# millecker/hadoop-1.0.3-gpu

Measured on AMD Instinct MI355X. Metric: K-Means job makespan + map-tasks/sec (whole node) at 1/2/4/8 MI355X, higher is better.
Workload: dtype fp32

## Files before the change

hbmr/models/kmeans.py:

```python
from __future__ import annotations

import base64
import logging
import math
import os
import threading
import time

import numpy as np
import torch

from ..gpu.splitjob import SplitJob, SplitSpec
from ..mapred import counters as C

log = logging.getLogger("hbmr.kmeans")

K_KEY = "hbmr.kmeans.k"
D_KEY = "hbmr.kmeans.dims"
INPUT_KEY = "hbmr.kmeans.input"
SPLIT_PTS_KEY = "hbmr.split.points"
CIN_KEY = "hbmr.kmeans.centroids.in"
COUT_KEY = "hbmr.kmeans.centroids.out"
INIT_KEY = "hbmr.kmeans.centroids.init"
NCENTERS_KEY = "hbmr.kmeans.synthetic.centers"
RETURN_KEY = "hbmr.kmeans.return.centroids"
CDIR_KEY = "hbmr.kmeans.centroids.dir"
EXACT_KEY = "hbmr.kmeans.exact"
EXACT_MFMA_KEY = "hbmr.kmeans.exact.mfma"
COMBINER_KEY = "hbmr.kmeans.combiner"
BOUNDS_KEY = "hbmr.kmeans.exact.bounds"

_M32 = 0xFFFFFFFF


def _mix32(x: torch.Tensor) -> torch.Tensor:
    x = x & _M32
    x = ((x ^ (x >> 16)) * 0x45D9F3B) & _M32
    x = ((x ^ (x >> 16)) * 0x45D9F3B) & _M32
    return x ^ (x >> 16)


def _uniform(c: torch.Tensor) -> torch.Tensor:
    return (_mix32(c).to(torch.float64) + 0.5) * (1.0 / 4294967296.0)


def _gauss(c1: torch.Tensor, c2: torch.Tensor) -> torch.Tensor:
    u1 = _uniform(c1)
    u2 = _uniform(c2)
    return torch.sqrt(-2.0 * torch.log(u1)) * torch.cos(2.0 * math.pi * u2)


def synthetic_points(seed: int, start: int, n: int, d: int, centers: int, device,
                     chunk: int = 1 << 18) -> torch.Tensor:
    dev = torch.device(device)
    out = torch.empty(n, d, dtype=torch.float32, device=dev)
    j = torch.arange(d, dtype=torch.int64, device=dev)
    cidx = torch.arange(centers, dtype=torch.int64, device=dev)
    s = (seed * 0x9E3779B1) & _M32
    cc = (cidx[:, None] * 131071 + j[None, :] + s * 7) & _M32
    cen = 10.0 * _gauss(cc * 2 + 1, cc * 2 + 2)
    for a in range(0, n, chunk):
        b = min(n, a + chunk)
        p = torch.arange(start + a, start + b, dtype=torch.int64, device=dev)
        lab = _mix32(p * 3 + s) % centers
        base = ((p[:, None] & 0xFFFFFF) * 1024 + j[None, :] + (s << 7)) & _M32
        noise = _gauss(base * 2 + 11, base * 2 + 12 + (p[:, None] >> 24))
        out[a:b] = (cen[lab] + noise).to(torch.float32)
    return out


def encode_centroids(c: torch.Tensor) -> str:
    a = c.detach().to("cpu", torch.float32).contiguous().numpy()
    return f"{a.shape[0]}x{a.shape[1]}:" + base64.b64encode(a.tobytes()).decode()


def decode_centroids(s: str) -> torch.Tensor:
    shp, b = s.split(":", 1)
    k, d = map(int, shp.split("x"))
    return torch.from_numpy(np.frombuffer(base64.b64decode(b), dtype=np.float32).copy()
                            ).reshape(k, d)


class CentroidStore:

    def __init__(self):
        self.lock = threading.Lock()
        self.host: dict[str, torch.Tensor] = {}
        self.images: dict[tuple, object] = {}
        self.order: list[str] = []
        self.keep = 4

    def put_host(self, key, cen):
        with self.lock:
            self.host[key] = cen
            for k in [k for k in self.images if k[0] == key]:
                self.images.pop(k)
            self._touch(key)

    def put_image(self, key, device, img):
        with self.lock:
            self.host.pop(key, None)
            self.images[(key, str(device))] = img
            self._touch(key)

    def _touch(self, key):
        if key in self.order:
            self.order.remove(key)
        self.order.append(key)
        while len(self.order) > self.keep:
            old = self.order.pop(0)
            self.host.pop(old, None)
            for k in [k for k in self.images if k[0] == old]:
                self.images.pop(k)

    def host_centroids(self, key):
        with self.lock:
            c = self.host.get(key)
            if c is not None:
                return c
            for (k, _dev), img in self.images.items():
                if k == key:
                    ready = getattr(img, "ready", None)
                    if ready is not None:
                        ready.synchronize()
                    c = img.cen.detach().to("cpu")
                    self.host[key] = c
                    return c
        return None

    def image(self, key, device):
        from ..ops import kmeans as km
        with self.lock:
            img = self.images.get((key, str(device)))
        if img is not None:
            return img
        cen = self.host_centroids(key)
        if cen is None:
            raise KeyError(f"centroids {key!r} not resident on this tracker")
        img = km.CentroidImage(cen, device)
        if img.cen.is_cuda:
            img.ready = torch.cuda.Event()
            img.ready.record()
        self.put_image(key, device, img)
        return img


STORE = CentroidStore()


def _centroid_file(cdir, key):
    return os.path.join(cdir, key.replace("/", "_").replace(":", "_") + ".npy")


def _save_centroids(cdir, key, cen):
    host = cen.detach().to("cpu", torch.float32).numpy()
    os.makedirs(cdir, exist_ok=True)
    path = _centroid_file(cdir, key)
    tmp = path + ".tmp.npy"
    np.save(tmp, host)
    os.replace(tmp, path)
    old = _SAVED.setdefault(cdir, [])
    old.append(path)
    while len(old) > 3:
        try:
            os.remove(old.pop(0))
        except OSError:
            pass


_SAVED: dict = {}
_PINNED_INFLIGHT: list = []


def _sum_slabs(outs):
    groups: dict = {}
    loose = []
    for s, c in outs:
        bs, bc = s._base, c._base
        if bs is not None and bc is not None and bs.dim() == 3 and bc.dim() == 2 and \
                tuple(s.shape) == tuple(bs.shape[1:]) and tuple(c.shape) == tuple(bc.shape[1:]):
            g = groups.setdefault(id(bs), [bs, bc, 0, []])
            g[2] += 1
            g[3].append((s, c))
        else:
            loose.append((s, c))
    parts_s, parts_c = [], []
    for bs, bc, n, members in groups.values():
        if n == bs.shape[0] and len({m[0].data_ptr() for m in members}) == n:
            parts_s.append(bs.sum(0))
            parts_c.append(bc.sum(0))
        else:
            loose.extend(members)
    if loose:
        parts_s.append(torch.stack([s for s, _ in loose]).sum(0))
        parts_c.append(torch.stack([c for _, c in loose]).sum(0))
    sums, counts = parts_s[0], parts_c[0]
    for s, c in zip(parts_s[1:], parts_c[1:]):
        sums = sums + s
        counts = counts + c
    return sums, counts


_EXACT_STATS: dict = {}
_EXACT_SKIPPED: dict = {}
_EXACT_LOCK = threading.Lock()

_BASELINES: "dict" = {}
_BASE_LOCK = threading.Lock()
_BASE_MAX = 4096


def _baseline_plan(ctxs, datas, k, dp, fx, exact, enabled):
    have, new, plain = [], [], []
    bases, keys = [], []
    seen = set()
    dev = str(ctxs[0].device)
    with _BASE_LOCK:
        for i, (c, d) in enumerate(zip(ctxs, datas)):
            sp = c.spec.split
            sk = sp.get("key") if enabled and isinstance(sp, dict) else None
            key = None if sk is None else (sk, dev, k, dp, fx, exact)
            keys.append(key)
            if key is None or key in seen:
                plain.append(i)
                bases.append(None)
                continue
            seen.add(key)
            b = _BASELINES.get(key)
            x = d.xb if exact else d
            if b is not None and b.data_ptr == x.data_ptr() and b.n == x.shape[0]:
                have.append(i)
                bases.append(b)
            else:
                new.append(i)
                bases.append(None)
    return have, new, plain, bases, keys


def _baseline_bytes(b) -> int:
    return sum(t.numel() * t.element_size() for t in (b.g, b.S0, b.N0, getattr(b, "gap", None))
               if t is not None)


def _drop_baselines(split_key, device):
    dev = f"cuda:{device}" if isinstance(device, int) else str(device)
    with _BASE_LOCK:
        for key in [kk for kk in _BASELINES if kk[0] == split_key and kk[1] == dev]:
            _BASELINES.pop(key)


def _install_baselines(entries, stream, cache=None, grown=None):
    ev = torch.cuda.Event()
    ev.record(stream)
    charge = []
    with _BASE_LOCK:
        for key, b in entries:
            b.event, b.stream = ev, stream
            old = _BASELINES.pop(key, None)
            _BASELINES[key] = b
            if old is not b:
                charge.append((key, b, _baseline_bytes(b)))
            elif grown and grown.get(id(b)):
                charge.append((key, b, grown[id(b)]))
        while len(_BASELINES) > _BASE_MAX:
            _BASELINES.pop(next(iter(_BASELINES)))
    if cache is not None and charge:
        cache.add_listener(_drop_baselines)
        idx = stream.device.index if stream is not None else 0
        for key, b, nbytes in charge:
            if not cache.charge(key[0], idx, nbytes):
                with _BASE_LOCK:
                    if _BASELINES.get(key) is b:
                        _BASELINES.pop(key)


def _exact_stats(cin, device):
    key = (cin, str(device))
    with _EXACT_LOCK:
        t = _EXACT_STATS.get(key)
        if t is None:
            t = _EXACT_STATS[key] = torch.zeros(3, dtype=torch.int64, device=device)
        return t


def _exact_skipped(cin, device):
    key = (cin, str(device))
    with _EXACT_LOCK:
        t = _EXACT_SKIPPED.get(key)
        if t is None:
            t = _EXACT_SKIPPED[key] = torch.zeros(1, dtype=torch.int64, device=device)
        return t


class KMeansSplitJob(SplitJob):
    collective_reduce = True
    needs_reduce = True

    def configure(self, conf):
        self.conf = conf
        self.k = conf.get_int(K_KEY, 64)
        self.d = conf.get_int(D_KEY, 128)
        self.input = conf.get(INPUT_KEY, "synthetic:100000:1")
        self.split_points = conf.get_int(SPLIT_PTS_KEY, 500_000)
        self.cin = conf.get(CIN_KEY)
        self.cout = conf.get(COUT_KEY)
        self.centers = conf.get_int(NCENTERS_KEY, self.k)
        self.fx_shift = conf.get_int("hbmr.kmeans.fx.shift", 24)
        self.cdir = conf.get(CDIR_KEY)
        self.exact = conf.get_boolean(EXACT_KEY, False)
        self.exact_dtype = torch.bfloat16 if (conf.get(EXACT_MFMA_KEY) or "f16").lower() in (
            "bf16", "bfloat16") else torch.float16
        self.bounds = conf.get_boolean(BOUNDS_KEY, True)
        self.combiner = (conf.get(COMBINER_KEY) or "delta").lower()
        if self.combiner not in ("delta", "sorted"):
            raise ValueError(f"{COMBINER_KEY} must be delta or sorted, not {self.combiner!r}")
        init = conf.get(INIT_KEY)
        if init and self.cin and STORE.host_centroids(self.cin) is None:
            STORE.put_host(self.cin, decode_centroids(init))
        if self.cin and self.cdir and STORE.host_centroids(self.cin) is None:
            path = _centroid_file(self.cdir, self.cin)
            if os.path.exists(path):
                STORE.put_host(self.cin, torch.from_numpy(np.load(path)))

    _split_memo: dict = {}

    def get_splits(self, conf, trackers):
        if self.input.startswith("synthetic:"):
            mk = (self.input, self.split_points, self.d, self.centers, tuple(trackers),
                  self.exact)
            got = KMeansSplitJob._split_memo.get(mk)
            if got is not None:
                return got
            if len(KMeansSplitJob._split_memo) > 16:
                KMeansSplitJob._split_memo.clear()
            out = KMeansSplitJob._split_memo[mk] = self._synthetic_splits(trackers)
            return out
        return self._file_splits(conf, trackers)

    def _synthetic_splits(self, trackers):
        _, n, seed = self.input.split(":")
        n, seed = int(n), int(seed)
        per = self.split_points
        nsplits = max(1, math.ceil(n / per))
        out = []
        for i in range(nsplits):
            a = i * per
            m = min(per, n - a)
            key = f"kmeans-syn:{seed}:{self.d}:{self.centers}:{a}:{m}" + \
                (":exact" if self.exact else "")
            loc = [trackers[i * len(trackers) // nsplits]] if trackers else []
            out.append(SplitSpec(i, key, "synthetic",
                                 {"seed": seed, "start": a, "n": m}, loc, m * self.d * 2))
        return out

    def _file_splits(self, conf, trackers):
        from ..mapred.formats import FileInputFormat, SequenceFileInputFormat
        from ..mapred.jobconf import JobConf
        jc = JobConf(conf)
        FileInputFormat.setInputPaths(jc, self.input)
        fmt = SequenceFileInputFormat()
        nmaps = max(1, conf.get_int("mapred.map.tasks", 1))
        if conf.get_long("mapred.min.split.size", 0) <= 1 and "://" not in self.input:
            total = sum(f.length for f in fmt.list_status(jc))
            jc.set_long("mapred.min.split.size", max(1, -(-total // nmaps)))
        splits = fmt.getSplits(jc, nmaps)
        out = []
        for i, s in enumerate(splits):
            key = f"kmeans-file:{s.path}:{s.start}:{s.length}" + (":exact" if self.exact else "")
            loc = [trackers[i % len(trackers)]] if trackers else []
            out.append(SplitSpec(i, key, "file", {"path": s.path, "start": s.start,
                                                  "length": s.length}, loc, s.length))
        return out

    def _load_raw(self, spec: SplitSpec, device):
        if spec.kind == "synthetic":
            p = spec.params
            return synthetic_points(p["seed"], p["start"], p["n"], self.d, self.centers, device)
        return self._load_file_split(spec.params, device)

    def _load_fp32(self, spec: SplitSpec, device):
        return self._load_raw(spec, device).to(torch.bfloat16)

    def split_nbytes(self, data) -> int:
        nb = getattr(data, "nbytes", None)
        if callable(nb):
            return int(nb())
        return super().split_nbytes(data)

    def load_split_host(self, spec: SplitSpec):
        if spec.kind != "file":
            return None
        from ..io import nativeio
        p = spec.params
        n = p["length"] // (20 + 4 * self.d) + 2
        host = torch.empty(n, self.d, dtype=torch.float32,
                           pin_memory=torch.cuda.is_available())
        got = nativeio.read_points_into(p["path"], p["start"], p["length"], host.data_ptr(),
                                        self.d, n)
        return host[:got]

    def load_split_from_host(self, spec: SplitSpec, host, device):
        from ..ops import kmeans as km
        x = host.to(device, non_blocking=True)
        ev = torch.cuda.Event()
        ev.record()
        _PINNED_INFLIGHT.append((ev, host))
        while _PINNED_INFLIGHT and _PINNED_INFLIGHT[0][0].query():
            _PINNED_INFLIGHT.pop(0)
        if self.exact:
            return km.ExactSplit(x, km.padded_dim(self.d), self.exact_dtype)
        xb = x.to(torch.bfloat16)
        dp = km.padded_dim(self.d)
        if dp == self.d:
            return xb.contiguous()
        out = torch.zeros(xb.shape[0], dp, dtype=torch.bfloat16, device=device)
        out[:, :self.d] = xb
        return out

    def _load_file_split(self, p, device):
        from ..io import nativeio
        n = p["length"] // (20 + 4 * self.d) + 2
        dev = torch.device(device)
        host = torch.empty(n, self.d, dtype=torch.float32, pin_memory=dev.type == "cuda")
        got = nativeio.read_points_into(p["path"], p["start"], p["length"], host.data_ptr(),
                                        self.d, n)
        host = host[:got]
        if dev.type != "cuda":
            return host
        x = host.to(dev, non_blocking=True)
        ev = torch.cuda.Event()
        ev.record()
        _PINNED_INFLIGHT.append((ev, host))
        while _PINNED_INFLIGHT and _PINNED_INFLIGHT[0][0].query():
            _PINNED_INFLIGHT.pop(0)
        return x

    def load_split_sample(self, spec: SplitSpec, device, fraction: float):
        if spec.kind == "synthetic":
            p = dict(spec.params)
            p["n"] = max(1, int(p["n"] * fraction))
            spec = SplitSpec(spec.index, spec.key + f":sample{fraction}", spec.kind, p,
                             spec.locations, spec.length)
            return self.load_split(spec, device)
        return super().load_split_sample(spec, device, fraction)

    def load_split(self, spec: SplitSpec, device):
        from ..ops import kmeans as km
        if self.exact:
            x = self._load_raw(spec, device)
            if str(device) == "cpu":
                return x.contiguous()
            return km.ExactSplit(x, km.padded_dim(self.d), self.exact_dtype)
        xb = self._load_fp32(spec, device)
        if str(device) == "cpu":
            return xb.to(torch.float32)
        dp = km.padded_dim(self.d)
        if dp == self.d:
            return xb.contiguous()
        out = torch.zeros(xb.shape[0], dp, dtype=torch.bfloat16, device=device)
        out[:, :self.d] = xb
        return out

    @staticmethod
    def _scratch(ctx, ns, k):
        from ..ops import kmeans as km
        key = ("kmeans-scratch", str(ctx.device), id(ctx.stream))
        store = ctx.tracker.__dict__.setdefault("_scratch", {})
        ws, labels = store.get(key, (None, None))
        need_lab, need_ws = km.batch_scratch_sizes(ns, k)
        need_ws = max(need_ws, km.delta_workspace_bytes(int(sum(ns)), len(ns), k))
        if ws is None or ws.numel() < need_ws:
            ws = torch.empty(max(need_ws, 1 << 20), dtype=torch.uint8, device=ctx.device)
        if labels is None or labels.numel() < need_lab:
            labels = torch.empty(max(need_lab, 1), dtype=torch.int32, device=ctx.device)
        store[key] = (ws, labels)
        return ws, labels

    def map_gpu(self, ctx, points):
        return self.map_gpu_batch([ctx], [points])[0]

    def map_gpu_batch(self, ctxs, datas):
        st = ctxs[0].stream
        if st is None:
            return self._map_gpu_batch(ctxs, datas)
        with torch.cuda.stream(st):
            return self._map_gpu_batch(ctxs, datas)

    def _map_gpu_batch(self, ctxs, datas):
        from ..ops import kmeans as km
        ctx = ctxs[0]
        img = STORE.image(self.cin, ctx.device)
        ready = getattr(img, "ready", None)
        if ready is not None:
            torch.cuda.current_stream().wait_event(ready)
        for t in (img.cbf, img.chalf):
            t.record_stream(torch.cuda.current_stream())
        B = len(datas)
        if self.exact:
            return self._map_exact(ctxs, datas, img)
        have, new, plain, bases, keys = _baseline_plan(
            ctxs, datas, self.k, img.dp, img.fx_shift, False, self.combiner == "delta")
        ws, labels = self._scratch(ctx, [d.shape[0] for d in datas], self.k)
        sums = torch.empty(B, self.k, img.dp, dtype=torch.int64, device=ctx.device)
        counts = torch.empty(B, self.k, dtype=torch.int64, device=ctx.device)
        order = have + new + plain
        H = len(have)
        S, N = sums.unbind(0), counts.unbind(0)
        out = [None] * B
        for j, i in enumerate(order):
            out[i] = (S[j], N[j])
        installed = []
        if have:
            hb = [bases[i] for i in have]
            km.map_batch_delta([datas[i] for i in have], img, sums[:H], counts[:H], labels, ws,
                               hb, stream=ctx.stream)
            for i, b in zip(have, hb):
                b.S0, b.N0 = out[i]
                installed.append((keys[i], b))
        rest = new + plain
        if rest:
            km.map_batch_gpu([datas[i] for i in rest], img, sums[H:], counts[H:], labels, ws,
                             stream=ctx.stream, zero_outputs=True)
            if new:
                total = sum(datas[i].shape[0] for i in rest)
                gall = labels[:total].clone()
                off = 0
                newset = set(new)
                for i in rest:
                    n = datas[i].shape[0]
                    if keys[i] is not None and i in newset:
                        installed.append((keys[i], km.Baseline(gall[off:off + n], *out[i],
                                                                datas[i].data_ptr(), n)))
                    off += n
        if installed:
            _install_baselines(installed, ctx.stream, getattr(ctx, "split_cache", None))
        for c, d in zip(ctxs, datas):
            c.reporter.incrCounter(C.TASK_GROUP, C.MAP_INPUT_RECORDS, d.shape[0])
        return out

    def _map_exact(self, ctxs, datas, img):
        from ..ops import kmeans as km
        from ..utils.trace import TRACE
        if TRACE.on:
            TRACE.instant("kmeans.map_exact", n=len(datas))
        ctx = ctxs[0]
        store = ctx.tracker.__dict__.setdefault("_scratch", {})
        scratch = store.setdefault(("kmeans-exact", str(ctx.device), id(ctx.stream)), {})
        stats = _exact_stats(self.cin, ctx.device)
        have, new, plain, bases, keys = _baseline_plan(
            ctxs, datas, self.k, img.dp, img.fx_shift, True, self.combiner == "delta")
        B = len(datas)
        sums = torch.empty(B, self.k, img.dp, dtype=torch.int64, device=ctx.device)
        counts = torch.empty(B, self.k, dtype=torch.int64, device=ctx.device)
        order = have + new + plain
        pos = {i: j for j, i in enumerate(order)}
        H = len(have)
        installed = []
        grown = None
        if have:
            ns = [datas[i].shape[0] for i in have]
            total = sum(ns)
            lab = scratch.get("labcat")
            if lab is None or lab.numel() < total:
                lab = scratch["labcat"] = torch.empty(total, dtype=torch.int32, device=ctx.device)
            need = km.delta_workspace_bytes(total, H, self.k)
            if scratch.get("dws") is None or scratch["dws"].numel() < need:
                scratch["dws"] = torch.empty(need, dtype=torch.uint8, device=ctx.device)
            hb = [bases[i] for i in have]
            bounded = self.bounds and self.combiner == "delta" and km.bounds_supported(img)
            if bounded:
                nogap = [b for b in hb if b.gap is None]
                km.assign_exact_batch([datas[i] for i in have], img, stats, lab, scratch,
                                      stream=ctx.stream, bounds=hb,
                                      skipped=_exact_skipped(self.cin, ctx.device))
                grown = {id(b): b.gap.numel() * b.gap.element_size() for b in nogap}
            else:
                km.assign_exact_batch([datas[i] for i in have], img, stats, lab, scratch,
                                      stream=ctx.stream)
            km.delta_combine([datas[i].x32 for i in have], lab, self.k, sums[:H], counts[:H],
                             scratch["dws"], hb, fx_shift=img.fx_shift, stream=ctx.stream,
                             keep_bounds=bounded)
            for i, b in zip(have, hb):
                b.S0, b.N0 = sums[pos[i]], counts[pos[i]]
                installed.append((keys[i], b))
        for i in new + plain:
            d = datas[i]
            s, c = sums[pos[i]], counts[pos[i]]
            s.zero_()
            c.zero_()
            lab = km.assign_exact(d, img, stats, scratch, stream=ctx.stream)
            need = km.workspace_bytes(d.shape[0], img.k)
            if scratch.get("ws") is None or scratch["ws"].numel() < need:
                scratch["ws"] = torch.empty(max(need, 1 << 20), dtype=torch.uint8,
                                            device=ctx.device)
            km.accumulate(d.x32, lab, img.k, s, c, fx_shift=img.fx_shift, stream=ctx.stream,
                          workspace=scratch["ws"])
            if keys[i] is not None and i in new:
                b = km.Baseline(lab.clone(), s, c, d.xb.data_ptr(), d.shape[0])
                installed.append((keys[i], b))
        if installed:
            _install_baselines(installed, ctx.stream, getattr(ctx, "split_cache", None), grown)
        for c, d in zip(ctxs, datas):
            c.reporter.incrCounter(C.TASK_GROUP, C.MAP_INPUT_RECORDS, d.shape[0])
        return [(sums[pos[i]], counts[pos[i]]) for i in range(B)]

    def map_cpu(self, ctx, points):
        from ..ops import kmeans as km
        cen = STORE.host_centroids(self.cin)
        if cen is None:
            raise KeyError(f"centroids {self.cin!r} not resident")
        sums, counts = km.new_partials(self.k, self.d, "cpu")
        st = [0]
        km.map_split_cpu(points, cen, sums, counts, nthreads=ctx.cpu_threads,
                         fx_shift=self.fx_shift, exact=self.exact, stats=st)
        if self.exact:
            ctx.reporter.incrCounter("KMEANS", "EXACT_FLAGGED_POINTS", st[0])
        ctx.reporter.incrCounter(C.TASK_GROUP, C.MAP_INPUT_RECORDS, points.shape[0])
        return sums, counts

    def map_sim(self, ctx, points):
        if points is None:
            ctx.reporter.incrCounter(C.TASK_GROUP, C.MAP_INPUT_RECORDS, 0)
            return None
        return self.map_cpu(ctx, points)

    def combine(self, ctx, outputs):
        from ..ops import kmeans as km
        dev = ctx.device if ctx.device is not None else torch.device("cpu")
        dp = km.padded_dim(self.d) if dev.type == "cuda" else self.d
        outputs = [o for o in outputs if o is not None]
        if dev.type == "cuda":
            cur = torch.cuda.current_stream()
            for s, c in outputs:
                if s.is_cuda:
                    s.record_stream(cur)
                    c.record_stream(cur)
        from ..utils.trace import TRACE
        if TRACE.on:
            TRACE.instant("kmeans.combine.recorded", n=len(outputs))
        same = [(s, c) for s, c in outputs if s.device == dev and s.shape[1] == dp]
        other = [(s, c) for s, c in outputs if not (s.device == dev and s.shape[1] == dp)]
        if same:
            sums, counts = _sum_slabs(same)
        else:
            sums = torch.zeros(self.k, dp, dtype=torch.int64, device=dev)
            counts = torch.zeros(self.k, dtype=torch.int64, device=dev)
        for s, c in other:
            sums[:, :s.shape[1]] += s.to(dev, non_blocking=True)
            counts += c.to(dev, non_blocking=True)
        return sums, counts

    def reduce(self, ctx, combined):
        from ..ops import kmeans as km
        from ..utils.trace import TRACE
        sums, counts = combined
        k, dp = sums.shape
        packed = torch.cat([sums.reshape(-1), counts])
        sim = getattr(ctx, "simulated_collective_s", None)
        with TRACE.span("kmeans.allreduce", nbytes=packed.numel() * 8):
            if sim is None:
                ctx.comm.all_reduce(packed)
            else:
                ctx.sim_ready = max(time.time(), getattr(ctx, "sim_base", 0.0)) + sim
        sums = packed[:k * dp].view(k, dp)
        counts = packed[k * dp:]
        est = _EXACT_STATS.pop((self.cin, str(sums.device)), None) \
            if self.exact and sums.device.type == "cuda" else None
        esk = _EXACT_SKIPPED.pop((self.cin, str(sums.device)), None) \
            if self.exact and sums.device.type == "cuda" else None
        killed = getattr(ctx, "killed", None)
        if killed is not None and killed():
            raise RuntimeError("reduce killed (collective restart): result not published")
        if sums.device.type == "cuda":
            old = STORE.image(self.cin, sums.device)
            ready = getattr(old, "ready", None)
            if ready is not None:
                torch.cuda.current_stream().wait_event(ready)
            img = km.CentroidImage.__new__(km.CentroidImage)
            img.__dict__.update(old.__dict__)
            img.cen = old.cen.clone()
            img.cbf = old.cbf.clone()
            img.chalf = old.chalf.clone()
            img.shift2 = torch.zeros_like(old.shift2)
            img.refresh(sums, counts)
            if self.exact:
                img.image16(self.exact_dtype)
                img.neighbors()
            img.ready = torch.cuda.Event()
            img.ready.record()
            host_cen = cen_ev = None
            if ctx.rank == 0 and (self.cdir or self.conf.get_boolean(RETURN_KEY, False)):
                host_cen = torch.empty(tuple(img.cen.shape), dtype=torch.float32,
                                       pin_memory=True)
                host_cen.copy_(img.cen, non_blocking=True)
                cen_ev = torch.cuda.Event()
                cen_ev.record()
            if TRACE.on:
                TRACE.instant("kmeans.refresh_launched")
            STORE.put_image(self.cout, sums.device, img)
            rel = getattr(ctx, "release_dependents", None)
            if rel is not None:
                rel()
            vals = [img.shift2.max().double().sqrt(), counts.sum().double()]
            if est is not None:
                vals += list(est.double().unbind(0))
            if esk is not None:
                vals.append(esk[0].double())
            got = torch.stack(vals).tolist()
            shift, npts = got[0], got[1]
            if esk is not None:
                ctx.reporter.incrCounter("KMEANS", "EXACT_BOUND_SKIPPED_POINTS", int(got[-1]))
            if est is not None:
                for name, v in zip(("EXACT_FLAGGED_POINTS", "EXACT_RELABELLED_POINTS",
                                    "EXACT_NEIGHBOUR_SCANS"), got[2:5]):
                    ctx.reporter.incrCounter("KMEANS", name, int(v))
            if TRACE.on:
                TRACE.instant("kmeans.shift_synced")
            new_cen = None
        else:
            host_cen = cen_ev = None
            old = STORE.host_centroids(self.cin)
            if sim is not None:
                new_cen, shift, npts = old, 0.0, 0
            else:
                cnt = counts.to(torch.float64)[:, None]
                s = sums[:, :self.d].to(torch.float64) / float(1 << self.fx_shift)
                new_cen = torch.where(cnt > 0, s / cnt.clamp(min=1),
                                      old.to(torch.float64)).to(torch.float32)
                shift = float((new_cen - old).norm(dim=1).max()) if self.k else 0.0
                npts = int(counts.sum().item())
            STORE.put_host(self.cout, new_cen)
            rel = getattr(ctx, "release_dependents", None)
            if rel is not None:
                rel()
            if sim is not None:
                delay = ctx.sim_ready - time.time()
                if delay > 0:
                    time.sleep(delay)
        self._write_output(ctx, counts, new_cen)
        if TRACE.on:
            TRACE.instant("kmeans.output_written")
        res = {"shift": shift, "points": int(npts), "centroids_key": self.cout}
        if host_cen is not None:
            cen_ev.synchronize()
        if ctx.rank == 0 and self.cdir:
            cen = new_cen if new_cen is not None else host_cen
            _save_centroids(self.cdir, self.cout, cen[:, :self.d])
        if ctx.rank == 0 and self.conf.get_boolean(RETURN_KEY, False):
            cen = new_cen if new_cen is not None else host_cen
            res["centroids"] = encode_centroids(cen[:, :self.d])
        if TRACE.on:
            TRACE.instant("kmeans.reduce_return")
        return res

    def poison_result(self, ctx):
        with STORE.lock:
            host = STORE.host.get(self.cout)
            if host is not None:
                STORE.host[self.cout] = host + 1.0
            for key, img in list(STORE.images.items()):
                if key[0] == self.cout:
                    STORE.images.pop(key)
                    STORE.host[self.cout] = img.cen.detach().to("cpu")[:, :self.d] + 1.0

    def _write_output(self, ctx, counts, new_cen):
        out = self.conf.get("mapred.output.dir")
        if not out:
            return
        import os

        from ..io import sequencefile as seqf
        from ..io.writable import FloatVectorWritable, IntWritable
        cen = new_cen if new_cen is not None else STORE.host_centroids(self.cout)
        W = ctx.world_size
        per = math.ceil(self.k / W)
        lo, hi = ctx.rank * per, min(self.k, (ctx.rank + 1) * per)
        os.makedirs(out, exist_ok=True)
        with seqf.Writer(os.path.join(out, f"part-{ctx.rank:05d}"), IntWritable,
                         FloatVectorWritable) as w:
            for j in range(lo, hi):
                w.append(IntWritable(j), FloatVectorWritable(cen[j].numpy()))


def make_iteration_conf(base, k, d, inp, split_points, cin, cout, init=None,
                        return_centroids=False):
    from ..mapred.jobconf import JobConf
    job = JobConf(base)
    job.set_job_name(f"kmeans {cin}->{cout}")
    job.set("hbmr.splitjob.class", "hbmr.models.kmeans:KMeansSplitJob")
    job.set("hbmr.gpu.mapper.class", "hbmr.models.kmeans:KMeansSplitJob")
    job.set_int(K_KEY, k)
    job.set_int(D_KEY, d)
    job.set(INPUT_KEY, inp)
    job.set_int(SPLIT_PTS_KEY, split_points)
    job.set(CIN_KEY, cin)
    job.set(COUT_KEY, cout)
    job.set("hbmr.job.signature", f"kmeans|{inp}|{k}|{d}|{split_points}")
    if init is not None:
        job.set(INIT_KEY, encode_centroids(init))
    if return_centroids:
        job.set_boolean(RETURN_KEY, True)
    return job


def initial_centroids(inp, k, d, centers=None, exact=False):
    def rnd(x):
        return x if exact else x.to(torch.bfloat16).to(torch.float32)
    if inp.startswith("synthetic:"):
        _, _n, seed = inp.split(":")
        x = synthetic_points(int(seed), 0, k, d, centers or k, "cpu")
        return rnd(x)
    from ..io import sequencefile as seqf
    import os
    path = inp
    if os.path.isdir(path):
        path = os.path.join(path, sorted(f for f in os.listdir(path) if not f.startswith(("_", ".")))[0])
    rows = []
    with seqf.Reader(path) as r:
        while len(rows) < k:
            raw = r.next_raw()
            if raw is None:
                break
            rows.append(np.frombuffer(raw[1][4:], dtype=">f4").astype(np.float32))
    return rnd(torch.from_numpy(np.stack(rows)))


class KMeansDriver:

    MANIFEST = "driver.json"

    def __init__(self, submit, result_of, conf=None, k=64, d=128, inp="synthetic:100000:1",
                 split_points=500_000, run_id=None, return_centroids=None, checkpoint_dir=None):
        self.submit = submit
        self.result_of = result_of
        self.base = conf
        self.k, self.d, self.inp, self.split_points = k, d, inp, split_points
        self.run_id = run_id or f"km{int(time.time() * 1e3) & 0xFFFFFF:x}"
        self.iteration = 0
        self.history = []
        self.return_centroids = (k * d <= 65536) if return_centroids is None else return_centroids
        base_dir = (conf.get("mapred.local.dir") if conf is not None else None) or "/tmp/hbmr-local"
        self.centroid_dir = checkpoint_dir or os.path.join(base_dir, "kmeans-centroids",
                                                           self.run_id)
        self._manifest_written = False
        self.prefetch_delay = 0.005
        self._ahead: list = []

    def _write_manifest(self):
        import json
        os.makedirs(self.centroid_dir, exist_ok=True)
        path = os.path.join(self.centroid_dir, self.MANIFEST)
        with open(path + ".tmp", "w") as f:
            json.dump({"run_id": self.run_id, "k": self.k, "d": self.d, "input": self.inp,
                       "split_points": self.split_points}, f)
        os.replace(path + ".tmp", path)
        self._manifest_written = True

    @classmethod
    def resume(cls, submit, result_of, checkpoint_dir, conf=None, **kw):
        import json
        import re
        with open(os.path.join(checkpoint_dir, cls.MANIFEST)) as f:
            m = json.load(f)
        drv = cls(submit, result_of, conf=conf, k=m["k"], d=m["d"], inp=m["input"],
                  split_points=m["split_points"], run_id=m["run_id"],
                  checkpoint_dir=checkpoint_dir, **kw)
        pat = re.compile(re.escape(_centroid_file("", drv.key(0))[:-len("_0.npy")]) +
                         r"_(\d+)\.npy$")
        found = sorted((int(mm.group(1)), fn) for fn in os.listdir(checkpoint_dir)
                       for mm in [pat.match(fn)] if mm)
        for i, fn in reversed(found):
            try:
                c = torch.from_numpy(np.load(os.path.join(checkpoint_dir, fn)))
            except (OSError, ValueError):
                continue
            if tuple(c.shape) != (drv.k, drv.d):
                continue
            drv.iteration = i
            STORE.put_host(drv.key(i), c.to(torch.float32))
            break
        drv._manifest_written = True
        return drv

    def key(self, i):
        return f"{self.run_id}:{i}"

    def _job_conf(self, i, depends_on=None):
        centers = self.base.get_int(NCENTERS_KEY, self.k) if self.base is not None else None
        exact = self.base.get_boolean(EXACT_KEY, False) if self.base is not None else False
        init = initial_centroids(self.inp, self.k, self.d, centers, exact=exact) if i == 0 \
            else None
        if init is not None:
            STORE.put_host(self.key(0), init)
        job = make_iteration_conf(self.base, self.k, self.d, self.inp, self.split_points,
                                  self.key(i), self.key(i + 1), init=init,
                                  return_centroids=self.return_centroids)
        job.set(CDIR_KEY, self.centroid_dir)
        if depends_on is not None:
            from ..mapred.jobtracker import DEPENDS_KEY
            job.set(DEPENDS_KEY, str(depends_on))
        return job

    def step(self, prefetch=False):
        i = self.iteration
        if not self._manifest_written:
            self._write_manifest()
        t0 = time.time()
        ahead = bool(self._ahead)
        rj = self._ahead.pop(0) if ahead else self.submit(self._job_conf(i))
        depth = int(prefetch)
        if depth > 0 and len(self._ahead) < depth and \
                (ahead or not rj.waitForCompletion(self.prefetch_delay)):
            last = self._ahead[-1] if self._ahead else rj
            while len(self._ahead) < depth:
                nxt = self.submit(self._job_conf(i + 1 + len(self._ahead),
                                                 depends_on=last.getID()))
                self._ahead.append(nxt)
                last = nxt
        rj.waitForCompletion()
        if not rj.isSuccessful():
            raise RuntimeError(f"K-Means iteration {i} failed: {rj.getFailureInfo()}")
        res = dict(self.result_of(rj) or {})
        jip = getattr(rj._impl, "jip", None)
        if jip is not None:
            res["timeline"] = jip.timeline()
            res["maps_per_tracker"] = jip.maps_per_tracker()
        res.update(iteration=i, seconds=time.time() - t0, job=str(rj.getID()),
                   counters=rj.getCounters())
        self.history.append(res)
        self.iteration += 1
        return res

    def run(self, max_iter=10, tol=0.0):
        for _ in range(max_iter):
            r = self.step()
            if r.get("shift", 1.0) <= tol:
                break
        return self.centroids()

    def cancel_prefetch(self):
        ahead, self._ahead = self._ahead, []
        for nxt in reversed(ahead):
            nxt.killJob()

    def centroids(self):
        c = STORE.host_centroids(self.key(self.iteration))
        if c is None and self.history and self.history[-1].get("centroids"):
            c = decode_centroids(self.history[-1]["centroids"])
            STORE.put_host(self.key(self.iteration), c)
        return c


def main(argv=None, cluster=None):
    import argparse
    ap = argparse.ArgumentParser(prog="hbmr kmeans")
    ap.add_argument("--input", default=None, help="SequenceFile dir (default: synthetic)")
    ap.add_argument("--points", type=int, default=1_000_000)
    ap.add_argument("--k", type=int, default=64)
    ap.add_argument("--dims", type=int, default=128)
    ap.add_argument("--iters", type=int, default=5)
    ap.add_argument("--split-points", type=int, default=500_000)
    ap.add_argument("--seed", type=int, default=7)
    a = ap.parse_args(argv)
    from ..mapred.cluster import LocalCluster
    from ..mapred.jobconf import JobConf
    own = cluster is None
    conf = JobConf()
    if own:
        gpus = [[0]] if torch.cuda.is_available() else None
        cluster = LocalCluster(conf, num_trackers=1, gpus=gpus)
    try:
        drv = KMeansDriver(cluster.submit_job, lambda rj: rj._impl.jip.result[0], conf=conf,
                           k=a.k, d=a.dims, inp=a.input or f"synthetic:{a.points}:{a.seed}",
                           split_points=a.split_points)
        for _ in range(a.iters):
            r = drv.step()
            print(f"iteration {r['iteration']}: shift {r['shift']:.6f} "
                  f"({r['seconds'] * 1e3:.1f} ms)")
        return 0
    finally:
        if own:
            cluster.shutdown()
```

hbmr/ops/_lib.py:

```python
from __future__ import annotations

import ctypes
import os
import threading
from pathlib import Path

import torch

_LIB_PATH = Path(__file__).resolve().parent.parent / "lib" / "libhbmr.so"
_lock = threading.Lock()
_lib = None

c_void_p = ctypes.c_void_p
c_long = ctypes.c_long
c_int = ctypes.c_int
c_uint = ctypes.c_uint
c_uint64 = ctypes.c_uint64
c_double_p = ctypes.POINTER(ctypes.c_double)

_SIGS = {
    "hbmr_kmeans_assign_bf16": (c_int, [c_void_p, c_long, c_int, c_void_p, c_void_p, c_int,
                                        c_void_p, c_void_p, c_void_p]),
    "hbmr_kmeans_accum_bf16": (c_int, [c_void_p, c_long, c_int, c_void_p, c_int, c_void_p,
                                       c_void_p, c_int, c_void_p, c_long, c_int, c_void_p]),
    "hbmr_kmeans_accum_f32": (c_int, [c_void_p, c_long, c_int, c_void_p, c_int, c_void_p,
                                      c_void_p, c_int, c_void_p, c_long, c_int, c_void_p]),
    "hbmr_kmeans_assign_top3_bf16": (c_int, [c_void_p, c_long, c_int, c_void_p, c_void_p, c_int,
                                             c_void_p, c_void_p, c_void_p, c_void_p, c_void_p]),
    "hbmr_kmeans_assign_top3_f16": (c_int, [c_void_p, c_long, c_int, c_void_p, c_void_p, c_int,
                                            c_void_p, c_void_p, c_void_p, c_void_p, c_void_p]),
    "hbmr_kmeans_exact_prep": (c_int, [c_void_p, c_long, c_int, c_int, c_int, c_int, c_void_p,
                                       c_void_p, c_void_p, c_void_p, c_void_p]),
    "hbmr_kmeans_assign_top3_q1_grouped": (c_int, [c_int, c_void_p, c_void_p, c_int, c_int,
                                                   c_void_p, c_void_p, c_void_p, c_int, c_void_p,
                                                   c_void_p, c_void_p, c_void_p, c_int, c_int,
                                                   c_void_p, c_void_p, c_void_p, c_void_p,
                                                   c_void_p, c_long, c_void_p, c_void_p]),
    "hbmr_kmeans_bound_workspace_bytes": (c_long, [c_long, c_int, c_int]),
    "hbmr_kmeans_assign_top3_q1_bounded": (c_int, [c_int, c_void_p, c_void_p, c_int, c_int,
                                                   c_void_p, c_void_p, c_int, c_void_p,
                                                   c_void_p, c_void_p, c_void_p, c_int, c_int,
                                                   c_void_p, c_void_p, c_void_p, c_void_p,
                                                   c_void_p, c_long, c_void_p,
                                                   c_void_p, c_void_p, c_void_p, c_void_p,
                                                   c_void_p, c_long, c_void_p, c_void_p]),
    "hbmr_kmeans_centroid_nbr": (c_int, [c_void_p, c_int, c_int, c_int, c_void_p, c_void_p,
                                         c_void_p, c_void_p]),
    "hbmr_kmeans_image16": (c_int, [c_void_p, c_int, c_int, c_int, c_int, c_int, c_void_p,
                                    c_void_p, c_void_p, c_void_p, c_void_p, c_void_p]),
    "hbmr_kmeans_image16_tiled": (c_int, [c_void_p, c_int, c_int, c_void_p, c_void_p]),
    "hbmr_kmeans_set_exact_kernel": (c_int, [c_int]),
    "hbmr_kmeans_get_exact_kernel": (c_int, []),
    "hbmr_kmeans_refine_f32": (c_int, [c_void_p, c_long, c_int, c_int, c_void_p, c_void_p,
                                       c_void_p, c_void_p, c_int, c_int, c_void_p, c_void_p,
                                       c_void_p, c_void_p, c_void_p, c_void_p, c_int, c_void_p,
                                       c_void_p, c_void_p, c_void_p, c_void_p, c_int,
                                       c_void_p]),
    "hbmr_kmeans_refine_batch_bytes": (c_long, [c_int, c_void_p]),
    "hbmr_kmeans_assign_top3_grouped": (c_int, [c_int, c_void_p, c_void_p, c_int, c_int,
                                                c_void_p, c_void_p, c_int, c_void_p, c_void_p,
                                                c_void_p, c_void_p, c_void_p]),
    "hbmr_kmeans_refine_batch_q1g": (c_int, [c_int, c_void_p, c_int, c_int, c_int, c_void_p,
                                             c_void_p, c_void_p, c_void_p, c_void_p, c_void_p,
                                             c_void_p, c_void_p, c_void_p, c_void_p, c_void_p,
                                             c_void_p, c_long, c_void_p, c_void_p]),
    "hbmr_kmeans_refine_batch_q1": (c_int, [c_int, c_void_p, c_int, c_int, c_int, c_int,
                                            c_void_p, c_void_p, c_void_p, c_void_p, c_void_p,
                                            c_void_p, c_void_p, c_void_p, c_void_p, c_void_p,
                                            c_void_p, c_void_p, c_void_p, c_long, c_int,
                                            c_void_p, c_void_p]),
    "hbmr_kmeans_refine_batch_finish": (c_int, [c_int, c_void_p, c_void_p, c_void_p, c_int,
                                                c_int, c_void_p, c_int, c_int, c_void_p,
                                                c_void_p, c_void_p, c_void_p, c_int, c_void_p,
                                                c_int, c_void_p, c_long, c_void_p]),
    "hbmr_kmeans_accum_workspace_bytes": (c_long, [c_long, c_int]),
    "hbmr_kmeans_batch_workspace_bytes": (c_long, [c_long, c_int, c_int]),
    "hbmr_kmeans_map_batch": (c_int, [c_int, c_void_p, c_void_p, c_int, c_void_p, c_void_p, c_int,
                                      c_int, c_void_p, c_void_p, c_long, c_void_p, c_void_p,
                                      c_int, c_int, c_void_p]),
    "hbmr_kmeans_delta_workspace_bytes": (c_long, [c_long, c_int, c_int]),
    "hbmr_kmeans_delta_combine": (c_int, [c_int, c_void_p, c_void_p, c_int, c_int, c_int,
                                          c_void_p, c_void_p, c_long, c_void_p, c_void_p, c_int,
                                          c_void_p, c_void_p, c_void_p, c_void_p]),
    "hbmr_kmeans_map_batch_delta": (c_int, [c_int, c_void_p, c_void_p, c_int, c_void_p, c_void_p,
                                            c_int, c_int, c_void_p, c_void_p, c_long, c_void_p,
                                            c_void_p, c_int, c_void_p, c_void_p, c_void_p,
                                            c_void_p]),
    "hbmr_kmeans_update": (c_int, [c_void_p, c_void_p, c_int, c_int, c_int, c_int, c_int,
                                   c_void_p, c_void_p, c_void_p, c_void_p, c_void_p]),
    "hbmr_kmeans_padded_k": (c_int, [c_int]),
    "hbmr_kmeans_map_cpu_f32": (c_int, [c_void_p, c_long, c_int, c_void_p, c_int, c_void_p,
                                        c_void_p, c_void_p, c_double_p, c_int, c_int]),
    "hbmr_kmeans_map_cpu_f32_ex": (c_int, [c_void_p, c_long, c_int, c_void_p, c_int, c_void_p,
                                           c_void_p, c_void_p, c_double_p, c_int, c_int, c_int,
                                           c_void_p]),
    "hbmr_kmeans_padded_dim": (c_int, [c_int]),
    "hbmr_f32_to_bf16_pad": (c_int, [c_void_p, c_long, c_int, c_int, c_void_p, c_void_p]),
    "hbmr_radix_sort_workspace_bytes": (c_long, [c_long]),
    "hbmr_radix_onesweep_workspace_bytes": (c_long, [c_long]),
    "hbmr_radix_onesweep_status_bytes": (c_long, [c_long]),
    "hbmr_radix_sort_keys_u64": (c_int, [c_void_p, c_void_p, c_long, c_int, c_int, c_void_p,
                                         c_long, c_void_p, c_long, c_void_p, c_void_p, c_int,
                                         c_void_p]),
    "hbmr_radix_sort_pairs_u64": (c_int, [c_void_p, c_void_p, c_void_p, c_void_p, c_long, c_int,
                                          c_int, c_void_p, c_long, c_void_p]),
    "hbmr_teragen": (c_int, [c_long, c_long, c_void_p, c_void_p]),
    "hbmr_tera_keys": (c_int, [c_void_p, c_long, c_int, c_void_p, c_void_p, c_void_p]),
    "hbmr_gather_u64": (c_int, [c_void_p, c_void_p, c_long, c_void_p, c_void_p]),
    "hbmr_gather_records": (c_int, [c_void_p, c_void_p, c_long, c_int, c_void_p, c_void_p]),
    "hbmr_split_offsets": (c_int, [c_void_p, c_void_p, c_long, c_void_p, c_void_p, c_int,
                                   c_void_p, c_void_p]),
    "hbmr_check_sorted": (c_int, [c_void_p, c_void_p, c_long, c_void_p, c_void_p]),
    "hbmr_tera_collect": (c_int, [c_void_p, c_void_p, c_void_p, c_void_p, c_void_p, c_int, c_long,
                                  c_void_p, c_void_p, c_void_p, c_void_p, c_void_p]),
    "hbmr_tera_collect_slots": (c_int, [c_void_p, c_void_p, c_void_p, c_int, c_int, c_long,
                                        c_void_p, c_void_p, c_void_p]),
    "hbmr_gather_records_multi": (c_int, [c_void_p, c_void_p, c_void_p, c_void_p, c_long, c_int,
                                          c_void_p, c_void_p]),
    "hbmr_tera_partition_workspace_bytes": (c_long, [c_long, c_int]),
    "hbmr_tera_collect_gid": (c_int, [c_void_p, c_void_p, c_void_p, c_void_p, c_int, c_long,
                                      c_int, c_uint64, c_uint, c_uint, c_int, c_void_p, c_void_p,
                                      c_void_p]),
    "hbmr_gather_records_gid": (c_int, [c_void_p, c_void_p, c_void_p, c_long, c_int, c_void_p,
                                        c_void_p, c_void_p, c_void_p, c_void_p]),
    "hbmr_tera_group_stats": (c_int, [c_void_p, c_void_p, c_long, c_void_p, c_void_p, c_void_p,
                                      c_void_p]),
    "hbmr_radix_set_onesweep_waves": (c_int, [c_int]),
    "hbmr_gather_set_unroll": (c_int, [c_int]),
    "hbmr_tera_tie_fix_scratch_bytes": (c_long, [c_long, c_int]),
    "hbmr_tera_tie_fix_records": (c_int, [c_void_p, c_void_p, c_void_p, c_long, c_int, c_uint64,
                                          c_uint, c_uint, c_int, c_void_p, c_void_p, c_void_p,
                                          c_long, c_void_p]),
    "hbmr_merge_path": (c_int, [c_void_p, c_void_p, c_void_p, c_long, c_void_p, c_void_p, c_void_p,
                                c_long, c_void_p, c_void_p, c_void_p, c_void_p]),
    "hbmr_tera_tie_fix": (c_int, [c_void_p, c_void_p, c_void_p, c_long, c_void_p, c_void_p]),
    "hbmr_tera_partition": (c_int, [c_void_p, c_long, c_int, c_void_p, c_void_p, c_int, c_void_p,
                                    c_void_p, c_void_p, c_void_p, c_void_p, c_void_p, c_long,
                                    c_void_p]),
    "hbmr_wc_tiles": (c_long, [c_long]),
    "hbmr_wc_tokenize_count": (c_int, [c_void_p, c_long, c_void_p, c_void_p]),
    "hbmr_wc_tokenize_write": (c_int, [c_void_p, c_long, c_void_p, c_void_p, c_void_p, c_void_p]),
    "hbmr_wc_insert": (c_int, [c_void_p, c_long, c_void_p, c_void_p, c_void_p, c_long, c_void_p,
                               c_void_p, c_long, c_void_p, c_void_p]),
    "hbmr_wc_compact": (c_int, [c_void_p, c_long, c_void_p, c_void_p, c_long, c_int, c_void_p,
                                c_void_p, c_void_p, c_void_p, c_void_p, c_void_p]),
    "hbmr_wc_pack": (c_int, [c_void_p, c_void_p, c_void_p, c_void_p, c_long, c_void_p, c_void_p,
                             c_void_p]),
    "hbmr_grep_cand_count": (c_int, [c_void_p, c_long, c_void_p, c_void_p, c_int, c_int, c_int,
                                     c_int, c_void_p, c_void_p, c_void_p]),
    "hbmr_grep_cand_write": (c_int, [c_void_p, c_long, c_void_p, c_void_p, c_int, c_int, c_int,
                                     c_int, c_void_p, c_void_p, c_void_p, c_void_p, c_void_p]),
    "hbmr_grep_select_blocks": (c_long, [c_long]),
    "hbmr_grep_block_max": (c_int, [c_void_p, c_long, c_void_p, c_void_p]),
    "hbmr_grep_prefix_max": (c_int, [c_void_p, c_long, c_void_p, c_void_p, c_void_p]),
    "hbmr_grep_select_count": (c_int, [c_void_p, c_void_p, c_void_p, c_long, c_void_p, c_void_p]),
    "hbmr_grep_select_write": (c_int, [c_void_p, c_void_p, c_void_p, c_long, c_void_p, c_void_p,
                                       c_void_p, c_void_p]),
    "hbmr_span_insert": (c_int, [c_void_p, c_long, c_void_p, c_void_p, c_void_p, c_long, c_void_p,
                                 c_void_p, c_long, c_void_p, c_void_p]),
    "hbmr_span_compact": (c_int, [c_void_p, c_void_p, c_void_p, c_void_p, c_void_p, c_long, c_int,
                                  c_void_p, c_void_p, c_void_p, c_void_p, c_void_p, c_void_p]),
    "hbmr_lines_count": (c_int, [c_void_p, c_long, c_void_p, c_void_p]),
    "hbmr_lines_write": (c_int, [c_void_p, c_long, c_void_p, c_void_p, c_void_p, c_void_p]),
    "hbmr_recsort_hash_partition": (c_int, [c_void_p, c_void_p, c_void_p, c_long, c_int, c_void_p,
                                            c_void_p]),
    "hbmr_recsort_round_keys": (c_int, [c_void_p, c_void_p, c_void_p, c_void_p, c_long, c_int,
                                        c_void_p, c_void_p, c_void_p]),
    "hbmr_recsort_round_workspace_bytes": (c_long, [c_long]),
    "hbmr_recsort_round": (c_int, [c_void_p, c_void_p, c_void_p, c_int, c_long, c_int, c_void_p,
                                   c_void_p, c_void_p, c_void_p, c_void_p, c_void_p, c_void_p,
                                   c_void_p, c_void_p, c_long, c_void_p]),
    "hbmr_recsort_cuts": (c_int, [c_void_p, c_void_p, c_void_p, c_void_p, c_long, c_void_p,
                                  c_void_p, c_void_p, c_int, c_void_p, c_void_p]),
    "hbmr_recsort_chunk_bytes": (c_int, []),
    "hbmr_recsort_set_chunk_lanes": (c_int, [c_int]),
    "hbmr_recsort_gather": (c_int, [c_void_p, c_void_p, c_void_p, c_void_p, c_void_p, c_void_p,
                                    c_void_p, c_long, c_long, c_void_p, c_void_p]),
    "hbmr_recjoin_heads": (c_int, [c_void_p, c_void_p, c_void_p, c_long, c_void_p, c_void_p,
                                   c_void_p]),
    "hbmr_recjoin_set_two_level": (c_int, [c_int]),
    "hbmr_recjoin_rank": (c_int, [c_void_p, c_void_p, c_void_p, c_void_p, c_long, c_void_p,
                                  c_void_p, c_void_p, c_void_p, c_void_p, c_long, c_void_p,
                                  c_void_p, c_void_p]),
    "hbmr_recjoin_expand": (c_int, [c_void_p, c_int, c_void_p, c_void_p, c_void_p, c_void_p,
                                    c_void_p, c_void_p, c_long, c_int, c_void_p, c_long, c_long,
                                    c_void_p, c_void_p, c_void_p, c_void_p]),
    "hbmr_recjoin_frames": (c_int, [c_void_p, c_int, c_void_p, c_void_p, c_void_p, c_int,
                                    c_void_p, c_void_p, c_void_p, c_long, c_void_p, c_void_p,
                                    c_void_p, c_void_p, c_void_p, c_void_p, c_void_p, c_void_p,
                                    c_void_p]),
    "hbmr_recjoin_copy": (c_int, [c_void_p, c_void_p, c_void_p, c_void_p, c_void_p, c_long,
                                  c_void_p, c_void_p]),
    "hbmr_pi_halton": (c_int, [ctypes.c_longlong, ctypes.c_longlong, c_void_p, c_void_p]),
    "hbmr_gemm_bf16_tn": (c_int, [c_void_p, c_void_p, c_void_p, c_long, c_long, c_long,
                                  ctypes.c_float, c_int, c_void_p]),
    "hbmr_gemm_set_kernel": (c_int, [c_int]),
    "hbmr_gemm_bf16_tn_ex": (c_int, [c_void_p, c_void_p, c_void_p, c_long, c_long, c_long,
                                     ctypes.c_float, c_int, c_void_p, c_void_p]),
}


class NativeLibraryError(RuntimeError):
    pass


def lib_path() -> Path:
    return _LIB_PATH


def available() -> bool:
    try:
        load()
        return True
    except NativeLibraryError:
        return False


def load():
    global _lib
    if _lib is not None:
        return _lib
    with _lock:
        if _lib is not None:
            return _lib
        if not _LIB_PATH.exists() and os.environ.get("HBMR_AUTOBUILD", "1") == "1":
            try:
                import importlib.util
                spec = importlib.util.spec_from_file_location(
                    "hbmr_native_build", _LIB_PATH.parent.parent.parent / "native" / "build.py")
                mod = importlib.util.module_from_spec(spec)
                spec.loader.exec_module(mod)
                mod.build()
            except Exception as e:
                raise NativeLibraryError(f"libhbmr.so missing and build failed: {e}") from e
        if not _LIB_PATH.exists():
            raise NativeLibraryError(f"native library not found at {_LIB_PATH}; run native/build.py")
        try:
            lib = ctypes.CDLL(str(_LIB_PATH), mode=ctypes.RTLD_GLOBAL)
        except OSError as e:
            raise NativeLibraryError(f"cannot load {_LIB_PATH}: {e}") from e
        for name, (res, args) in _SIGS.items():
            fn = getattr(lib, name)
            fn.restype = res
            fn.argtypes = args
        _lib = lib
        return lib


def check(rc: int, what: str) -> None:
    if rc != 0:
        raise RuntimeError(f"{what} failed with native error code {rc}")


def stream_handle(stream=None) -> int:
    if stream is None:
        stream = torch.cuda.current_stream()
    return int(stream.cuda_stream)
```

hbmr/ops/kmeans.py:

```python
from __future__ import annotations

import ctypes
import os
import threading

import torch

from . import _lib
from ..utils.trace import TRACE

SUPPORTED_DP = (64, 128, 256)


def _nullctx():
    import contextlib
    return contextlib.nullcontext()
FX_SHIFT = 24
NBR_L = 256


def padded_dim(d: int) -> int:
    for dp in SUPPORTED_DP:
        if d <= dp:
            return dp
    raise ValueError(f"feature dim {d} > {SUPPORTED_DP[-1]} not supported by the MFMA kernel")


def padded_k(k: int) -> int:
    return ((k + 63) // 64) * 64


def _ptr(t):
    return None if t is None else ctypes.c_void_p(t.data_ptr())


def new_partials(k: int, dp: int, device) -> tuple[torch.Tensor, torch.Tensor]:
    return (torch.zeros(k, dp, dtype=torch.int64, device=device),
            torch.zeros(k, dtype=torch.int64, device=device))


def partials_to_float(sums: torch.Tensor, counts: torch.Tensor, d: int | None = None,
                      fx_shift: int = FX_SHIFT):
    s = sums.to(torch.float64) / float(1 << fx_shift)
    if d is not None:
        s = s[:, :d]
    return s, counts.to(torch.float64)


class CentroidImage:

    def __init__(self, centroids: torch.Tensor, device, fx_shift: int = FX_SHIFT):
        c = centroids.detach().to(device=device, dtype=torch.float32).contiguous()
        self.k, self.d = c.shape
        self.dp = padded_dim(self.d)
        self.k_pad = padded_k(self.k)
        self.fx_shift = fx_shift
        self.device = c.device
        self.cen = c
        self.cbf = torch.zeros(self.k_pad, self.dp, dtype=torch.bfloat16, device=device)
        self.chalf = torch.empty(self.k_pad, dtype=torch.float32, device=device)
        self.shift2 = torch.zeros(self.k, dtype=torch.float32, device=device)
        self.refresh()

    def refresh(self, sums=None, counts=None, stream=None):
        lib = _lib.load()
        rc = lib.hbmr_kmeans_update(_ptr(sums), _ptr(counts), self.fx_shift, self.k, self.d,
                                    self.dp, self.k_pad, _ptr(self.cen), _ptr(self.cbf),
                                    _ptr(self.chalf), _ptr(self.shift2),
                                    _lib.stream_handle(stream))
        _lib.check(rc, "hbmr_kmeans_update")
        self._img16 = {}
        self._nbr = None
        if getattr(self, "_nbr_lock", None) is None:
            self._nbr_lock = threading.Lock()

    def set_centroids(self, centroids: torch.Tensor, stream=None):
        self.cen.copy_(centroids.to(self.cen.device, torch.float32))
        self.refresh(stream=stream)

    def image16(self, dtype=torch.float16):
        with self._nbr_lock:
            cache = self.__dict__.setdefault("_img16", {})
            ent = cache.get(dtype)
            if ent is None:
                dev = self.cen.device
                c16 = torch.empty(self.k_pad, self.dp, dtype=dtype, device=dev)
                ch = torch.empty(self.k_pad, dtype=torch.float32, device=dev)
                cn = torch.empty(self.k, dtype=torch.float32, device=dev)
                ce = torch.empty(self.k, dtype=torch.float32, device=dev)
                mx = torch.empty(2, dtype=torch.float32, device=dev)
                rc = _lib.load().hbmr_kmeans_image16(
                    _ptr(self.cen), self.k, self.d, self.dp, self.k_pad,
                    int(dtype == torch.float16), _ptr(c16), _ptr(ch), _ptr(cn), _ptr(ce),
                    _ptr(mx), _lib.stream_handle(None))
                _lib.check(rc, "hbmr_kmeans_image16")
                c16t = None
                if self.dp in (64, 128):
                    c16t = torch.empty_like(c16)
                    rc = _lib.load().hbmr_kmeans_image16_tiled(
                        _ptr(c16), self.k_pad, self.dp, _ptr(c16t), _lib.stream_handle(None))
                    _lib.check(rc, "hbmr_kmeans_image16_tiled")
                ev = torch.cuda.Event()
                ev.record()
                ent = cache[dtype] = (c16, ch, cn, mx[0:1], ce, mx[1:2], ev, c16t)
        torch.cuda.current_stream().wait_event(ent[6])
        return ent[:6]

    def image16_tiled(self, dtype=torch.float16):
        self.image16(dtype)
        return self._img16[dtype][7]

    def norms(self, dtype=torch.float16):
        _, _, cn, cm, ce, cem = self.image16(dtype)
        return cn, cm, ce, cem

    def neighbors(self, L: int | None = None):
        with self._nbr_lock:
            if self._nbr is None:
                if L is None:
                    L = int(os.environ.get("HBMR_KMEANS_NBR_L", NBR_L))
                L = max(1, min(L, self.k))
                if self.cen.is_cuda and self.k <= NBR_NATIVE_MAX_K and self.d <= 256:
                    dev = self.cen.device
                    di = torch.empty(self.k, L, dtype=torch.int32, device=dev)
                    f = torch.empty(self.k, L, dtype=torch.float32, device=dev)
                    pd = torch.empty(self.k, self.k, dtype=torch.float32, device=dev) \
                        if self.k <= PAIR_DIST_MAX_K else None
                    rc = _lib.load().hbmr_kmeans_centroid_nbr(
                        _ptr(self.cen), self.k, self.d, L, _ptr(di), _ptr(f), _ptr(pd),
                        _lib.stream_handle(None))
                    _lib.check(rc, "hbmr_kmeans_centroid_nbr")
                    ev = torch.cuda.Event()
                    ev.record()
                    self._nbr = (di, f, L, ev, pd)
                    di, f, L, ev, _ = self._nbr
                    torch.cuda.current_stream().wait_event(ev)
                    return di, f, L
                c = self.cen.double()
                n2 = (c * c).sum(1)
                nsum = n2[:, None] + n2[None, :]
                d2 = torch.addmm(nsum, c, c.T, beta=1.0, alpha=-2.0)
                err = nsum * ((self.d + 4) * 2.0 ** -53 * 1.01)
                lo = (d2 - err).clamp_(min=0.0).sqrt_()
                lo.fill_diagonal_(0.0)
                dv, di = lo.sort(dim=1, stable=True)
                dv, di = dv[:, :L].contiguous(), di[:, :L].to(torch.int32).contiguous()
                f = dv.float()
                f = torch.where(f.double() > dv, torch.nextafter(f, torch.full_like(f, -1.0)), f)
                pd = None
                if self.k <= PAIR_DIST_MAX_K:
                    hi = (d2 + err).clamp_(min=0.0).sqrt_()
                    hi.fill_diagonal_(0.0)
                    pd = hi.float()
                    pd = torch.where(pd.double() < hi, torch.nextafter(
                        pd, torch.full_like(pd, float("inf"))), pd).contiguous()
                ev = torch.cuda.Event()
                ev.record()
                self._nbr = (di, f.contiguous(), L, ev, pd)
        di, f, L, ev, _ = self._nbr
        torch.cuda.current_stream().wait_event(ev)
        return di, f, L

    def pair_dist(self):
        self.neighbors()
        return self._nbr[4]

    def max_shift(self) -> float:
        return float(self.shift2.max().sqrt().item()) if self.k else 0.0


def assign(points: torch.Tensor, img: CentroidImage, labels: torch.Tensor | None = None,
           scores: torch.Tensor | None = None, stream=None) -> torch.Tensor:
    n, dp = points.shape
    if points.dtype != torch.bfloat16 or dp != img.dp or not points.is_contiguous():
        raise ValueError("points must be contiguous bf16 [n, dp] matching the centroid image")
    if labels is None:
        labels = torch.empty(n, dtype=torch.int32, device=points.device)
    lib = _lib.load()
    rc = lib.hbmr_kmeans_assign_bf16(_ptr(points), n, dp, _ptr(img.cbf), _ptr(img.chalf),
                                     img.k_pad, _ptr(labels), _ptr(scores),
                                     _lib.stream_handle(stream))
    _lib.check(rc, "hbmr_kmeans_assign_bf16")
    return labels


ACCUM_AUTO, ACCUM_LDS, ACCUM_SORTED = 0, 1, 2
_workspaces: dict = {}


def workspace_bytes(n: int, k: int) -> int:
    return int(_lib.load().hbmr_kmeans_accum_workspace_bytes(n, k))


def batch_scratch_sizes(ns: list, k: int) -> tuple[int, int]:
    lib = _lib.load()
    total = int(sum(ns))
    ws = max(int(lib.hbmr_kmeans_batch_workspace_bytes(total, len(ns), k)),
             int(lib.hbmr_kmeans_accum_workspace_bytes(max(ns), k)))
    return total, ws


def accum_workspace(n: int, k: int, device) -> torch.Tensor:
    lib = _lib.load()
    need = int(lib.hbmr_kmeans_accum_workspace_bytes(n, k))
    key = torch.device(device)
    ws = _workspaces.get(key)
    if ws is None or ws.numel() < need:
        ws = torch.empty(max(need, 1 << 20), dtype=torch.uint8, device=key)
        _workspaces[key] = ws
    return ws


def accumulate(points: torch.Tensor, labels: torch.Tensor, k: int, sums: torch.Tensor,
               counts: torch.Tensor, fx_shift: int = FX_SHIFT, stream=None,
               workspace: torch.Tensor | None = None, mode: int = ACCUM_AUTO) -> None:
    n, dp = points.shape
    if sums.shape != (k, dp) or sums.dtype != torch.int64:
        raise ValueError(f"sums must be int64 [{k}, {dp}]")
    if counts.shape != (k,) or counts.dtype != torch.int64:
        raise ValueError(f"counts must be int64 [{k}]")
    if points.dtype not in (torch.bfloat16, torch.float32) or not points.is_contiguous() or \
            dp not in SUPPORTED_DP or labels.numel() < n:
        raise ValueError("points must be contiguous bf16/fp32 [n, dp] with n labels")
    lib = _lib.load()
    if workspace is None and mode != ACCUM_LDS:
        workspace = accum_workspace(n, k, points.device)
    fn, name = ((lib.hbmr_kmeans_accum_f32, "hbmr_kmeans_accum_f32")
                if points.dtype == torch.float32 else
                (lib.hbmr_kmeans_accum_bf16, "hbmr_kmeans_accum_bf16"))
    rc = fn(_ptr(points), n, dp, _ptr(labels), k, _ptr(sums), _ptr(counts), fx_shift,
            _ptr(workspace), 0 if workspace is None else workspace.numel(), mode,
            _lib.stream_handle(stream))
    _lib.check(rc, name)


def _f32_up(v: torch.Tensor) -> torch.Tensor:
    f = v.float()
    return torch.where(f.double() < v, torch.nextafter(f, torch.full_like(f, float("inf"))), f)


class ExactSplit:
    __slots__ = ("xb", "x32", "xnorm", "xbn2", "xerr", "d")

    def __init__(self, x32: torch.Tensor, dp: int, dtype=torch.float16):
        n, d = x32.shape
        self.d = d
        dev = x32.device
        if dp == d:
            self.x32 = x32.contiguous()
        else:
            self.x32 = torch.zeros(n, dp, dtype=torch.float32, device=dev)
            self.x32[:, :d] = x32
        if dev.type == "cuda":
            self.xb = torch.empty(n, dp, dtype=dtype, device=dev)
            self.xnorm = torch.empty(n, dtype=torch.float32, device=dev)
            self.xbn2 = torch.empty(n, dtype=torch.float32, device=dev)
            self.xerr = torch.empty(n, dtype=torch.float32, device=dev)
            rc = _lib.load().hbmr_kmeans_exact_prep(
                _ptr(self.x32), n, dp, dp, dp, int(dtype == torch.float16), _ptr(self.xb),
                _ptr(self.xnorm), _ptr(self.xbn2), _ptr(self.xerr), _lib.stream_handle(None))
            _lib.check(rc, "hbmr_kmeans_exact_prep")
            return
        x64 = self.x32.double()
        self.xnorm = x64.norm(dim=1).float()
        lim = 65504.0 if dtype == torch.float16 else float("inf")
        xb = self.x32.clamp(-lim, lim).to(dtype)
        xb64 = xb.double()
        self.xbn2 = xb64.pow(2).sum(1).float()
        self.xerr = _f32_up((x64 - xb64).norm(dim=1))
        self.xb = xb.contiguous()

    @property
    def shape(self):
        return self.xb.shape

    def nbytes(self) -> int:
        return sum(t.numel() * t.element_size() for t in (self.xb, self.x32, self.xnorm,
                                                          self.xbn2, self.xerr))


def assign_top3(points: torch.Tensor, img: CentroidImage, labels, cand, scores, margin,
                stream=None) -> None:
    n, dp = points.shape
    if points.dtype not in (torch.bfloat16, torch.float16) or dp != img.dp or \
            not points.is_contiguous():
        raise ValueError("points must be contiguous bf16/fp16 [n, dp] matching the image")
    for t, dt, m in ((labels, torch.int32, 1), (cand, torch.int32, 2), (scores, torch.float32, 1),
                     (margin, torch.float32, 2)):
        if t.numel() != m * n or t.dtype != dt or not t.is_contiguous():
            raise ValueError("top-3 outputs: labels/scores [n], cand/margin [2n]")
    f16 = points.dtype == torch.float16
    with torch.cuda.stream(stream) if stream is not None else _nullctx():
        c16, ch = img.image16(points.dtype)[:2]
    fn = "hbmr_kmeans_assign_top3_f16" if f16 else "hbmr_kmeans_assign_top3_bf16"
    rc = getattr(_lib.load(), fn)(
        _ptr(points), n, dp, _ptr(c16), _ptr(ch), img.k_pad, _ptr(labels),
        _ptr(cand), _ptr(scores), _ptr(margin), _lib.stream_handle(stream))
    _lib.check(rc, fn)


REFINE_VERSION = int(os.environ.get("HBMR_REFINE", "3"))
MAX_REFINE_BATCH = 64


def _check_refine_dim(img: "CentroidImage") -> None:
    if REFINE_VERSION >= 3 and img.d % 8:
        raise ValueError(f"refine v3 needs d % 8 == 0 (d = {img.d}): HBMR_REFINE=2 takes any d")


def _refine_ws(ns: list, device, scratch: dict | None):
    arr = (ctypes.c_long * len(ns))(*ns)
    need = int(_lib.load().hbmr_kmeans_refine_batch_bytes(len(ns), arr))
    if need < 0:
        raise ValueError("refine batch of 1..64 splits expected")
    ws = None if scratch is None else scratch.get("refine_ws")
    if ws is None or ws.numel() < need:
        ws = torch.empty(need, dtype=torch.uint8, device=device)
        if scratch is not None:
            scratch["refine_ws"] = ws
    return arr, ws


class _RefineBatch:

    def __init__(self, splits: list, img: "CentroidImage", stats, scratch, stream):
        _check_refine_dim(img)
        self.splits, self.img, self.stats, self.stream = splits, img, stats, stream
        self.dt = splits[0].xb.dtype
        self.ns, self.ws = _refine_ws([sp.shape[0] for sp in splits], splits[0].x32.device,
                                      scratch)
        with torch.cuda.stream(stream) if stream is not None else _nullctx():
            self.norms = img.norms(self.dt)
            self.nbr = img.neighbors()
            self.pd = img.pair_dist()
        self.labels = [None] * len(splits)
        self.lib = _lib.load()
        self.st = _lib.stream_handle(stream)

    def q1(self, i, labels_ptr, cand, scores, margin):
        sp, img = self.splits[i], self.img
        cn, cmax, ce, cemax = self.norms
        self.labels[i] = labels_ptr
        rc = self.lib.hbmr_kmeans_refine_batch_q1(
            len(self.splits), self.ns, i, img.d, img.k, img.k_pad, _ptr(sp.xnorm),
            _ptr(sp.xbn2), _ptr(sp.xerr), _ptr(cn), _ptr(cmax), _ptr(ce), _ptr(cemax),
            labels_ptr, _ptr(cand), _ptr(scores), _ptr(margin), _ptr(self.stats),
            _ptr(self.ws), self.ws.numel(), int(i == 0), _ptr(self.pd), self.st)
        _lib.check(rc, "hbmr_kmeans_refine_batch_q1")

    def finish(self):
        B = len(self.splits)
        img = self.img
        _, cmax, _, cemax = self.norms
        ni, nd, L = self.nbr
        xs = (ctypes.c_void_p * B)(*[sp.x32.data_ptr() for sp in self.splits])
        ls = (ctypes.c_void_p * B)(*[(lp.value if isinstance(lp, ctypes.c_void_p) else lp)
                                     for lp in self.labels])
        rc = self.lib.hbmr_kmeans_refine_batch_finish(
            B, self.ns, xs, ls, img.d, self.splits[0].x32.shape[1], _ptr(img.cen), img.k,
            img.k_pad, _ptr(cmax), _ptr(cemax), _ptr(ni), _ptr(nd), L, _ptr(self.stats),
            self.stats.numel(), _ptr(self.ws), self.ws.numel(), self.st)
        _lib.check(rc, "hbmr_kmeans_refine_batch_finish")


def refine_f32(split: ExactSplit, img: CentroidImage, labels, cand, scores, margin,
               stats: torch.Tensor, stream=None, scratch: dict | None = None) -> None:
    n = split.shape[0]
    if stats.dtype != torch.int64 or stats.numel() < 3:
        raise ValueError("stats must be int64 [3]")
    if labels.numel() != n or cand.numel() != 2 * n or margin.numel() != 2 * n:
        raise ValueError("labels [n], cand/margin [2n] from assign_top3 expected")
    if REFINE_VERSION >= 3:
        rb = _RefineBatch([split], img, stats, scratch, stream)
        rb.q1(0, labels.data_ptr(), cand, scores, margin)
        rb.finish()
        return
    with torch.cuda.stream(stream) if stream is not None else _nullctx():
        cn, cmax, ce, cemax = img.norms(split.xb.dtype)
        ni, nd, L = img.neighbors()
    rc = _lib.load().hbmr_kmeans_refine_f32(
        _ptr(split.x32), n, img.d, split.x32.shape[1], _ptr(split.xnorm), _ptr(split.xbn2),
        _ptr(split.xerr), _ptr(img.cen), img.k, img.k_pad, _ptr(cn), _ptr(cmax), _ptr(ce),
        _ptr(cemax), _ptr(ni), _ptr(nd), L,
        _ptr(labels), _ptr(cand), _ptr(scores), _ptr(margin), _ptr(stats), stats.numel(),
        _lib.stream_handle(stream))
    _lib.check(rc, "hbmr_kmeans_refine_f32")


def assign_exact(split: ExactSplit, img: CentroidImage, stats: torch.Tensor,
                 scratch: dict | None = None, stream=None) -> torch.Tensor:
    _check_refine_dim(img)
    n = split.shape[0]
    dev = split.xb.device
    scratch = {} if scratch is None else scratch
    key = ("exact", n)
    bufs = scratch.get(key)
    if bufs is None:
        bufs = scratch[key] = (torch.empty(n, dtype=torch.int32, device=dev),
                               torch.empty(2 * n, dtype=torch.int32, device=dev),
                               torch.empty(n, dtype=torch.float32, device=dev),
                               torch.empty(2 * n, dtype=torch.float32, device=dev))
    lab, cand, sc, mg = bufs
    assign_top3(split.xb, img, lab, cand, sc, mg, stream=stream)
    refine_f32(split, img, lab, cand, sc, mg, stats, stream=stream, scratch=scratch)
    return lab


def bounds_supported(img: CentroidImage) -> bool:
    return REFINE_VERSION >= 3 and img.dp <= 128 and GROUPED_EXACT and FUSED_Q1 and \
        img.cen.is_cuda and _lib.load().hbmr_kmeans_get_exact_kernel() == 3


def assign_exact_batch(splits: list, img: CentroidImage, stats: torch.Tensor, out: torch.Tensor,
                       scratch: dict | None = None, stream=None, bounds: list | None = None,
                       skipped: torch.Tensor | None = None) -> None:
    if not splits:
        return
    _check_refine_dim(img)
    if bounds is not None and (len(bounds) != len(splits) or not bounds_supported(img)):
        raise ValueError("bounds: one baseline per split, grouped fused v3 assign (dp <= 128)")
    dev = splits[0].xb.device
    total = sum(sp.shape[0] for sp in splits)
    if out.dtype != torch.int32 or out.numel() < total or not out.is_contiguous():
        raise ValueError("out must be contiguous int32 with room for every split's labels")
    if stats.dtype != torch.int64 or stats.numel() < 3:
        raise ValueError("stats must be int64 [3]")
    dt = splits[0].xb.dtype
    for sp in splits:
        if sp.xb.dtype != dt or dt not in (torch.bfloat16, torch.float16) or \
                sp.xb.shape[1] != img.dp or not sp.xb.is_contiguous() or \
                not sp.x32.is_contiguous():
            raise ValueError("exact splits must hold contiguous [n, dp] rows of one 16-bit type")
    nmax = max(sp.shape[0] for sp in splits)
    scratch = {} if scratch is None else scratch
    key = ("exact-batch", nmax)
    bufs = scratch.get(key)
    if bufs is None:
        for kk in [kk for kk in scratch if isinstance(kk, tuple) and kk[0] == "exact-batch"]:
            del scratch[kk]
        bufs = scratch[key] = (torch.empty(2 * nmax, dtype=torch.int32, device=dev),
                               torch.empty(nmax, dtype=torch.float32, device=dev),
                               torch.empty(2 * nmax, dtype=torch.float32, device=dev))
    cand, sc, mg = bufs
    grouped = REFINE_VERSION >= 3 and img.dp <= 128 and GROUPED_EXACT
    with torch.cuda.stream(stream) if stream is not None else _nullctx():
        c16, ch, cn, cmax, ce, cemax = img.image16(dt)
        ni, nd, L = (None, None, 0) if grouped else img.neighbors()
        newref = None
        if bounds is not None:
            img.cen.record_stream(torch.cuda.current_stream())
            newref = img.cen.clone()
    lib = _lib.load()
    top3 = lib.hbmr_kmeans_assign_top3_f16 if dt == torch.float16 else \
        lib.hbmr_kmeans_assign_top3_bf16
    st = _lib.stream_handle(stream)
    pc, ps, pm, pst = _ptr(cand), _ptr(sc), _ptr(mg), _ptr(stats)
    pcn, pcmax, pce, pcemax, pni, pnd = (_ptr(t) for t in (cn, cmax, ce, cemax, ni, nd))
    base, off = out.data_ptr(), 0
    for g0 in range(0, len(splits), MAX_REFINE_BATCH):
        group = splits[g0:g0 + MAX_REFINE_BATCH]
        if grouped:
            off += _exact_group(group, img, stats, base + 4 * off, c16, ch, (cn, cmax, ce, cemax),
                                dt, scratch, stream, lib, st,
                                None if bounds is None else bounds[g0:g0 + MAX_REFINE_BATCH],
                                skipped, newref)
            continue
        rb = _RefineBatch(group, img, stats, scratch, stream) if REFINE_VERSION >= 3 else None
        for i, sp in enumerate(group):
            n = sp.shape[0]
            pl = ctypes.c_void_p(base + 4 * off)
            rc = top3(_ptr(sp.xb), n, img.dp, _ptr(c16), _ptr(ch), img.k_pad, pl, pc, ps, pm, st)
            _lib.check(rc, "hbmr_kmeans_assign_top3")
            if rb is not None:
                rb.q1(i, pl, cand, sc, mg)
            else:
                rc = lib.hbmr_kmeans_refine_f32(
                    _ptr(sp.x32), n, img.d, sp.x32.shape[1], _ptr(sp.xnorm), _ptr(sp.xbn2),
                    _ptr(sp.xerr), _ptr(img.cen), img.k, img.k_pad, pcn, pcmax, pce, pcemax,
                    pni, pnd, L, pl, pc, ps, pm, pst, stats.numel(), st)
                _lib.check(rc, "hbmr_kmeans_refine_f32")
            off += n
        if rb is not None:
            rb.finish()


PAIR_DIST_MAX_K = int(os.environ.get("HBMR_PAIR_DIST_MAX_K", "8192"))
NBR_NATIVE_MAX_K = int(os.environ.get("HBMR_NBR_NATIVE_MAX_K", "8192"))
GROUPED_EXACT = os.environ.get("HBMR_EXACT_GROUPED", "1") != "0"
FUSED_Q1 = os.environ.get("HBMR_EXACT_FUSED_Q1", "1") != "0"


def _bounded_group(group, bases, img, labels_ptr, ch, norms, dt, scratch, stream, lib, st, rb,
                   skipped, newref):
    B = len(group)
    ns = [sp.shape[0] for sp in group]
    N = sum(ns)
    dev = group[0].xb.device
    cur = torch.cuda.current_stream() if stream is None else stream
    with torch.cuda.stream(cur):
        events, blocks = {}, {}
        for b in bases:
            if b.event is not None and b.stream is not None and b.stream != cur:
                events[id(b.event)] = b.event
        for ev in events.values():
            cur.wait_event(ev)
        for b in bases:
            if b.gap is None:
                b.gap, b.ref = torch.empty(b.g.numel(), dtype=torch.float32, device=dev), None
        for b, n in zip(bases, ns):
            if b.g.numel() != n or b.gap.numel() != n or \
                    (b.ref is not None and (tuple(b.ref.shape) != tuple(img.cen.shape) or
                                            not b.ref.is_contiguous())):
                raise ValueError("bounds: baseline does not match its split / the centroids")
            for t in (b.g, b.gap, b.ref):
                if t is not None:
                    base = t._base if t._base is not None else t
                    blocks[id(base)] = base
        for t in blocks.values():
            t.record_stream(cur)
        need = int(lib.hbmr_kmeans_bound_workspace_bytes(N, B, img.k))
        bws = scratch.get("bound_ws")
        if bws is None or bws.numel() < need:
            bws = scratch["bound_ws"] = torch.empty(need, dtype=torch.uint8, device=dev)
    P = ctypes.c_void_p * B
    cn, cmax, ce, cemax = norms
    refs = [b.ref for b in bases]
    for b in bases:
        b.ref = b.pending = None
    rc = lib.hbmr_kmeans_assign_top3_q1_bounded(
        B, P(*[sp.xb.data_ptr() for sp in group]), (ctypes.c_long * B)(*ns), img.dp,
        int(dt == torch.float16), _ptr(img.image16_tiled(dt)), _ptr(ch), img.k_pad, labels_ptr,
        P(*[sp.xnorm.data_ptr() for sp in group]), P(*[sp.xbn2.data_ptr() for sp in group]),
        P(*[sp.xerr.data_ptr() for sp in group]), img.d, img.k, _ptr(cn), _ptr(cmax), _ptr(ce),
        _ptr(cemax), _ptr(rb.ws), rb.ws.numel(), _ptr(rb.pd),
        P(*[b.g.data_ptr() for b in bases]), P(*[b.gap.data_ptr() for b in bases]),
        P(*[None if r is None else r.data_ptr() for r in refs]), _ptr(img.cen),
        _ptr(bws), bws.numel(), _ptr(skipped), st)
    _lib.check(rc, "hbmr_kmeans_assign_top3_q1_bounded")
    for b in bases:
        b.pending = newref


def _exact_group(group, img, stats, labels_ptr, c16, ch, norms, dt, scratch, stream, lib, st,
                 bases=None, skipped=None, newref=None):
    B = len(group)
    ns = [sp.shape[0] for sp in group]
    N = sum(ns)
    dev = group[0].xb.device
    P = ctypes.c_void_p * B
    xs = P(*[sp.xb.data_ptr() for sp in group])
    nsa = (ctypes.c_long * B)(*ns)
    if bases is not None:
        rb = _RefineBatch(group, img, stats, scratch, stream)
        if TRACE.on:
            TRACE.instant("kmeans.top3_launch", n=B)
        _bounded_group(group, bases, img, labels_ptr, ch, norms, dt, scratch, stream, lib, st, rb,
                       skipped, newref)
        o = 0
        for i in range(B):
            rb.labels[i] = labels_ptr + 4 * o
            o += ns[i]
        rb.finish()
        return N
    if FUSED_Q1 and img.dp <= 128:
        rb = _RefineBatch(group, img, stats, scratch, stream)
        if TRACE.on:
            TRACE.instant("kmeans.top3_launch", n=B)
        cn, cmax, ce, cemax = norms
        rc = lib.hbmr_kmeans_assign_top3_q1_grouped(
            B, xs, nsa, img.dp, int(dt == torch.float16), _ptr(c16),
            _ptr(img.image16_tiled(dt)), _ptr(ch), img.k_pad,
            labels_ptr, P(*[sp.xnorm.data_ptr() for sp in group]),
            P(*[sp.xbn2.data_ptr() for sp in group]), P(*[sp.xerr.data_ptr() for sp in group]),
            img.d, img.k, _ptr(cn), _ptr(cmax), _ptr(ce), _ptr(cemax), _ptr(rb.ws),
            rb.ws.numel(), _ptr(rb.pd), st)
        _lib.check(rc, "hbmr_kmeans_assign_top3_q1_grouped")
        o = 0
        for i in range(B):
            rb.labels[i] = labels_ptr + 4 * o
            o += ns[i]
        rb.finish()
        return N
    key = ("exact-group", N)
    bufs = scratch.get(key)
    if bufs is None:
        for kk in [kk for kk in scratch if isinstance(kk, tuple) and kk[0] == "exact-group"]:
            del scratch[kk]
        bufs = scratch[key] = (torch.empty(2 * N, dtype=torch.int32, device=dev),
                               torch.empty(N, dtype=torch.float32, device=dev),
                               torch.empty(2 * N, dtype=torch.float32, device=dev))
    cand, sc, mg = bufs
    rc = lib.hbmr_kmeans_assign_top3_grouped(B, xs, nsa, img.dp, int(dt == torch.float16),
                                             _ptr(c16), _ptr(ch), img.k_pad, labels_ptr,
                                             _ptr(cand), _ptr(sc), _ptr(mg), st)
    _lib.check(rc, "hbmr_kmeans_assign_top3_grouped")
    rb = _RefineBatch(group, img, stats, scratch, stream)
    cn, cmax, ce, cemax = norms
    rc = lib.hbmr_kmeans_refine_batch_q1g(
        B, nsa, img.d, img.k, img.k_pad, P(*[sp.xnorm.data_ptr() for sp in group]),
        P(*[sp.xbn2.data_ptr() for sp in group]), P(*[sp.xerr.data_ptr() for sp in group]),
        _ptr(cn), _ptr(cmax), _ptr(ce), _ptr(cemax), labels_ptr, _ptr(cand), _ptr(sc), _ptr(mg),
        _ptr(rb.ws), rb.ws.numel(), _ptr(rb.pd), st)
    _lib.check(rc, "hbmr_kmeans_refine_batch_q1g")
    o = 0
    for i in range(B):
        rb.labels[i] = labels_ptr + 4 * o
        o += ns[i]
    rb.finish()
    return N


def map_split_exact(split: ExactSplit, img: CentroidImage, sums, counts, scratch: dict,
                    stats: torch.Tensor, stream=None) -> None:
    n = split.shape[0]
    lab = assign_exact(split, img, stats, scratch, stream=stream)
    need = workspace_bytes(n, img.k)
    if scratch.get("ws") is None or scratch["ws"].numel() < need:
        scratch["ws"] = torch.empty(max(need, 1 << 20), dtype=torch.uint8, device=split.xb.device)
    accumulate(split.x32, lab, img.k, sums, counts, fx_shift=img.fx_shift, stream=stream,
               workspace=scratch["ws"])


def map_batch_gpu(splits: list, img: CentroidImage, sums: torch.Tensor, counts: torch.Tensor,
                  labels: torch.Tensor, workspace: torch.Tensor, stream=None,
                  zero_outputs: bool = True) -> None:
    B = len(splits)
    if B == 0:
        return
    for s in splits:
        if s.dtype != torch.bfloat16 or s.shape[1] != img.dp or not s.is_contiguous():
            raise ValueError("splits must be contiguous bf16 [n, dp]")
    if sums.shape != (B, img.k, img.dp) or counts.shape != (B, img.k):
        raise ValueError("batch output shape mismatch")
    need_lab, need_ws = batch_scratch_sizes([s.shape[0] for s in splits], img.k)
    if labels.numel() < need_lab:
        raise ValueError("labels scratch too small")
    lib = _lib.load()
    if workspace.numel() < need_ws:
        raise ValueError("workspace too small")
    ptrs = (ctypes.c_void_p * B)(*[s.data_ptr() for s in splits])
    ns = (ctypes.c_long * B)(*[s.shape[0] for s in splits])
    rc = lib.hbmr_kmeans_map_batch(B, ptrs, ns, img.dp, _ptr(img.cbf), _ptr(img.chalf), img.k_pad,
                                   img.k, _ptr(labels), _ptr(workspace), workspace.numel(),
                                   _ptr(sums), _ptr(counts), img.fx_shift, int(zero_outputs),
                                   _lib.stream_handle(stream))
    _lib.check(rc, "hbmr_kmeans_map_batch")


class Baseline:
    __slots__ = ("g", "S0", "N0", "event", "stream", "data_ptr", "n", "gap", "ref", "pending")

    def __init__(self, g, S0, N0, data_ptr, n):
        self.g, self.S0, self.N0 = g, S0, N0
        self.gap = self.ref = self.pending = None
        self.event = None
        self.stream = None
        self.data_ptr, self.n = data_ptr, n

    def labels_advanced(self, bounded: bool = False) -> None:
        self.ref = self.pending if bounded else None
        self.pending = None


def delta_workspace_bytes(total: int, ntasks: int, k: int) -> int:
    return int(_lib.load().hbmr_kmeans_delta_workspace_bytes(total, ntasks, k))


def _delta_args(xs, bases, stream):
    B = len(xs)
    st = torch.cuda.current_stream() if stream is None else stream
    events, blocks = {}, {}
    for b in bases:
        if b.event is not None and b.stream is not None and b.stream != st:
            events[id(b.event)] = b.event
        for t in (b.g, b.S0, b.N0):
            base = t._base if t._base is not None else t
            blocks[id(base)] = base
    for ev in events.values():
        st.wait_event(ev)
    for t in blocks.values():
        t.record_stream(st)
    ptrs = (ctypes.c_void_p * B)(*[x.data_ptr() for x in xs])
    ns = (ctypes.c_long * B)(*[x.shape[0] for x in xs])
    gs = (ctypes.c_void_p * B)(*[b.g.data_ptr() for b in bases])
    s0 = (ctypes.c_void_p * B)(*[b.S0.data_ptr() for b in bases])
    n0 = (ctypes.c_void_p * B)(*[b.N0.data_ptr() for b in bases])
    return ptrs, ns, gs, s0, n0


def map_batch_delta(splits: list, img: CentroidImage, sums: torch.Tensor, counts: torch.Tensor,
                    labels: torch.Tensor, workspace: torch.Tensor, bases: list,
                    stream=None) -> None:
    B = len(splits)
    if B == 0:
        return
    if B > 64 or len(bases) != B:
        raise ValueError("at most 64 splits per delta batch, one baseline each")
    for s, b in zip(splits, bases):
        if s.dtype != torch.bfloat16 or s.shape[1] != img.dp or not s.is_contiguous():
            raise ValueError("splits must be contiguous bf16 [n, dp]")
        if b.g.numel() != s.shape[0] or tuple(b.S0.shape) != (img.k, img.dp) or \
                b.N0.numel() != img.k:
            raise ValueError("baseline does not match its split")
    if sums.shape != (B, img.k, img.dp) or counts.shape != (B, img.k) or \
            not sums.is_contiguous() or not counts.is_contiguous():
        raise ValueError("batch output shape mismatch")
    total = sum(s.shape[0] for s in splits)
    if labels.numel() < total:
        raise ValueError("labels scratch too small")
    need = delta_workspace_bytes(total, B, img.k)
    if workspace.numel() < need:
        raise ValueError("workspace too small")
    ptrs, ns, gs, s0, n0 = _delta_args(splits, bases, stream)
    for b in bases:
        b.labels_advanced()
    rc = _lib.load().hbmr_kmeans_map_batch_delta(
        B, ptrs, ns, img.dp, _ptr(img.cbf), _ptr(img.chalf), img.k_pad, img.k, _ptr(labels),
        _ptr(workspace), workspace.numel(), _ptr(sums), _ptr(counts), img.fx_shift, gs, s0, n0,
        _lib.stream_handle(stream))
    _lib.check(rc, "hbmr_kmeans_map_batch_delta")


def delta_combine(xs: list, labels: torch.Tensor, k: int, sums: torch.Tensor,
                  counts: torch.Tensor, workspace: torch.Tensor, bases: list,
                  fx_shift: int = FX_SHIFT, stream=None, keep_bounds: bool = False) -> None:
    B = len(xs)
    if B == 0:
        return
    pend = [b.pending for b in bases]
    for b in bases:
        b.labels_advanced()
    dp = xs[0].shape[1]
    f32 = xs[0].dtype == torch.float32
    for x, b in zip(xs, bases):
        if x.dtype != xs[0].dtype or x.shape[1] != dp or not x.is_contiguous() or \
                b.g.numel() != x.shape[0]:
            raise ValueError("delta_combine: rows/baselines mismatch")
    if B > 64 or dp not in SUPPORTED_DP or sums.shape != (B, k, dp) or counts.shape != (B, k):
        raise ValueError("delta_combine: shape mismatch")
    total = sum(x.shape[0] for x in xs)
    need = delta_workspace_bytes(total, B, k)
    if workspace.numel() < need or labels.numel() < total:
        raise ValueError("delta_combine: scratch too small")
    ptrs, ns, gs, s0, n0 = _delta_args(xs, bases, stream)
    rc = _lib.load().hbmr_kmeans_delta_combine(
        B, ptrs, ns, dp, int(f32), k, _ptr(labels), _ptr(workspace), workspace.numel(),
        _ptr(sums), _ptr(counts), fx_shift, gs, s0, n0, _lib.stream_handle(stream))
    _lib.check(rc, "hbmr_kmeans_delta_combine")
    if keep_bounds:
        for b, p in zip(bases, pend):
            b.ref = p


def map_split_gpu(points, img: CentroidImage, sums, counts, labels=None, stream=None):
    labels = assign(points, img, labels=labels, stream=stream)
    accumulate(points, labels, img.k, sums, counts, fx_shift=img.fx_shift, stream=stream)
    return labels


def map_split_cpu(points: torch.Tensor, centroids: torch.Tensor, sums: torch.Tensor,
                  counts: torch.Tensor, nthreads: int = 1, labels: torch.Tensor | None = None,
                  fx_shift: int = FX_SHIFT, exact: bool = False, stats: list | None = None):
    x = points.detach().to(torch.float32).contiguous()
    c = centroids.detach().to(torch.float32).contiguous()
    n, d = x.shape
    k = c.shape[0]
    if counts.shape != (k,) or counts.dtype != torch.int64 or sums.dtype != torch.int64:
        raise ValueError("sums/counts must be int64")
    target = sums
    if sums.shape != (k, d):
        target = torch.zeros(k, d, dtype=torch.int64)
    cost = ctypes.c_double(0.0)
    lib = _lib.load()
    res = ctypes.c_long(0)
    rc = lib.hbmr_kmeans_map_cpu_f32_ex(_ptr(x), n, d, _ptr(c), k, _ptr(labels), _ptr(target),
                                        _ptr(counts), ctypes.byref(cost), fx_shift, int(nthreads),
                                        int(exact), ctypes.byref(res))
    _lib.check(rc, "hbmr_kmeans_map_cpu_f32_ex")
    if stats is not None:
        stats[0] += res.value
    if target is not sums:
        sums[:, :d] += target
    return cost.value
```

native/include/hbmr/hbmr.h:

```cpp
#pragma once
#include <stddef.h>
#include <stdint.h>

#ifdef __cplusplus
extern "C" {
#endif

typedef struct ihipStream_t* hbmr_stream_t;

#ifndef HBMR_NO_HIP_DECLS
#include <hip/hip_runtime_api.h>
int hbmr_kmeans_assign_bf16(const void* X, long n, int dp, const void* C, const float* chalf,
                            int k_pad, int32_t* labels, float* scores, hipStream_t st);
int hbmr_kmeans_accum_bf16(const void* X, long n, int dp, const int32_t* labels, int k,
                           long long* sums, long long* counts, int fx_shift, void* ws,
                           long ws_bytes, int mode, hipStream_t st);
int hbmr_kmeans_accum_f32(const float* X, long n, int dp, const int32_t* labels, int k,
                          long long* sums, long long* counts, int fx_shift, void* ws,
                          long ws_bytes, int mode, hipStream_t st);
int hbmr_kmeans_assign_top3_bf16(const void* X, long n, int dp, const void* C, const float* chalf,
                                 int k_pad, int32_t* labels, int32_t* cand, float* scores,
                                 float* margin, hipStream_t st);
int hbmr_kmeans_assign_top3_f16(const void* X, long n, int dp, const void* C, const float* chalf,
                                int k_pad, int32_t* labels, int32_t* cand, float* scores,
                                float* margin, hipStream_t st);
int hbmr_kmeans_exact_prep(const float* x, long n, int d, int ldx, int dp, int f16, void* x16,
                           float* xnorm, float* xn2, float* xerr, hipStream_t st);
int hbmr_kmeans_centroid_nbr(const float* cen, int k, int d, int L, int32_t* di, float* dv,
                             float* pd, hipStream_t st);
int hbmr_kmeans_image16(const float* cen, int k, int d, int dp, int k_pad, int f16, void* c16,
                        float* chalf, float* cnorm, float* cerr, float* maxima, hipStream_t st);
int hbmr_kmeans_image16_tiled(const void* c16, int k_pad, int dp, void* c16t, hipStream_t st);
int hbmr_kmeans_set_stamps(void* p);
int hbmr_kmeans_refine_f32(const float* X32, long n, int d, int ldx, const float* xnorm,
                           const float* xbn2, const float* xerr, const float* C32, int k,
                           int k_pad, const float* cnorm, const float* cmax, const float* cerr,
                           const float* cerrmax, const int32_t* nbr_idx,
                           const float* nbr_dist, int L, int32_t* labels, const int32_t* cand,
                           const float* scores, const float* margin, unsigned long long* stats,
                           int nstats, hipStream_t st);
int hbmr_kmeans_assign_top3_q1_grouped(int nsplit, const void* const* X, const long* n, int dp,
                                       int f16, const void* C, const void* Ct,
                                       const float* chalf, int k_pad,
                                       int32_t* labels, const float* const* xnorm,
                                       const float* const* xbn2, const float* const* xerr,
                                       int d, int k, const float* cnorm, const float* cmax,
                                       const float* cerr, const float* cerrmax, void* ws,
                                       long ws_bytes, const float* dcc, hipStream_t st);
long hbmr_kmeans_bound_workspace_bytes(long total, int nsplit, int k);
int hbmr_kmeans_assign_top3_q1_bounded(int nsplit, const void* const* X, const long* n, int dp,
                                       int f16, const void* Ct, const float* chalf, int k_pad,
                                       int32_t* labels, const float* const* xnorm,
                                       const float* const* xbn2, const float* const* xerr,
                                       int d, int k, const float* cnorm, const float* cmax,
                                       const float* cerr, const float* cerrmax, void* ws,
                                       long ws_bytes, const float* dcc,
                                       const int32_t* const* g, float* const* gap,
                                       const float* const* ref, const float* cen, void* bws,
                                       long bws_bytes, unsigned long long* skipped,
                                       hipStream_t st);
int hbmr_kmeans_assign_top3_grouped(int nsplit, const void* const* X, const long* n, int dp,
                                    int f16, const void* C, const float* chalf, int k_pad,
                                    int32_t* labels, int32_t* cand, float* scores, float* margin,
                                    hipStream_t st);
int hbmr_kmeans_refine_batch_q1g(int nsplit, const long* ns, int d, int k, int k_pad,
                                 const float* const* xnorm, const float* const* xbn2,
                                 const float* const* xerr, const float* cnorm, const float* cmax,
                                 const float* cerr, const float* cerrmax, const int32_t* labels,
                                 const int32_t* cand, const float* scores, const float* margin,
                                 void* ws, long ws_bytes, const float* dcc, hipStream_t st);
long hbmr_kmeans_refine_batch_bytes(int nsplit, const long* ns);
int hbmr_kmeans_refine_batch_q1(int nsplit, const long* ns, int s, int d, int k, int k_pad,
                                const float* xnorm, const float* xbn2, const float* xerr,
                                const float* cnorm, const float* cmax, const float* cerr,
                                const float* cerrmax, const int32_t* labels, const int32_t* cand,
                                const float* scores, const float* margin,
                                unsigned long long* stats, void* ws, long ws_bytes, int reset,
                                const float* dcc, hipStream_t st);
int hbmr_kmeans_refine_batch_finish(int nsplit, const long* ns, const float* const* x32,
                                    int32_t* const* labels, int d, int ldx, const float* C32,
                                    int k, int k_pad, const float* cmax, const float* cerrmax,
                                    const int32_t* nbr_idx, const float* nbr_dist, int L,
                                    unsigned long long* stats, int nstats, void* ws,
                                    long ws_bytes, hipStream_t st);
int hbmr_kmeans_update(const long long* sums, const long long* counts, int fx_shift, int k, int d,
                       int dp, int k_pad, float* cen, void* cbf, float* chalf, float* shift2,
                       hipStream_t st);
int hbmr_kmeans_map_batch(int ntasks, const void* const* X, const long* n, int dp,
                          const void* C, const float* chalf, int k_pad, int k, int32_t* labels,
                          void* ws, long ws_bytes, long long* sums, long long* counts,
                          int fx_shift, int zero_outputs, hipStream_t st);
int hbmr_f32_to_bf16_pad(const float* src, long n, int d, int dp, void* dst, hipStream_t st);
#endif
int hbmr_kmeans_padded_dim(int d);

#ifndef HBMR_NO_HIP_DECLS
int hbmr_radix_sort_pairs_u64(uint64_t* keys, uint32_t* vals, uint64_t* tkeys, uint32_t* tvals,
                              long n, int begin_bit, int end_bit, void* ws, long ws_bytes,
                              hipStream_t st);
int hbmr_teragen(long first_row, long nrows, void* out, hipStream_t st);
int hbmr_tera_keys(const void* records, long n, int stride, uint64_t* hi, uint64_t* lo,
                   hipStream_t st);
int hbmr_gather_u64(const uint64_t* src, const uint32_t* perm, long n, uint64_t* dst,
                    hipStream_t st);
int hbmr_gather_records(const void* src, const uint32_t* perm, long n, int record_bytes, void* dst,
                        hipStream_t st);
int hbmr_split_offsets(const uint64_t* hi, const uint64_t* lo, long n, const uint64_t* shi,
                       const uint64_t* slo, int nparts, long* offsets, hipStream_t st);
int hbmr_check_sorted(const uint64_t* hi, const uint64_t* lo, long n, unsigned long long* bad,
                      hipStream_t st);
int hbmr_tera_collect(const uint64_t* const* his, const uint64_t* const* los,
                      const uint32_t* const* rows, const long* starts, const long* prefix, int S,
                      long n, uint64_t* ohi, uint64_t* olo, uint32_t* osplit, uint32_t* orow,
                      hipStream_t st);
int hbmr_tera_collect_slots(const uint32_t* const* rows, const long* starts, const long* pre,
                            int S, int W, long C, uint32_t* osplit, uint32_t* orow,
                            hipStream_t st);
int hbmr_gather_records_multi(const void* const* bases, const uint32_t* split, const uint32_t* row,
                              const uint32_t* perm, long n, int record_bytes, void* dst,
                              hipStream_t st);
int hbmr_tera_collect_gid(const uint64_t* const* his, const uint32_t* const* rows,
                          const long* starts, const long* prefix, int S, long n, int pack,
                          uint64_t vlo, unsigned int m, unsigned int R, int sh, uint64_t* ohi,
                          uint32_t* ogid, hipStream_t st);
int hbmr_gather_records_gid(const void* const* bases, const uint32_t* gid, const uint64_t* packed,
                            long n, int record_bytes, void* dst, uint64_t* hi, uint64_t* lo,
                            uint32_t* win, hipStream_t st);
long hbmr_radix_onesweep_workspace_bytes(long n);
long hbmr_radix_onesweep_status_bytes(long n);
int hbmr_radix_sort_keys_u64(uint64_t* keys, uint64_t* tkeys, long n, int begin_bit, int end_bit,
                             void* ws, long ws_bytes, void* status, long status_bytes,
                             unsigned int* epoch, uint32_t* err, int copy_back, hipStream_t st);
long hbmr_tera_tie_fix_scratch_bytes(long cap, int record_bytes);
int hbmr_tera_group_stats(const uint64_t* hi, const uint64_t* lo, long n, const uint64_t* ph,
                          const uint64_t* pl, unsigned long long* acc, hipStream_t st);
int hbmr_tera_tie_fix_records(uint64_t* hi, uint64_t* lo, void* rec, long n, int record_bytes,
                              uint64_t vlo, unsigned int m, unsigned int R, int sh,
                              const uint32_t* win, unsigned int* flag, void* scratch, long cap,
                              hipStream_t st);
int hbmr_merge_path(const uint64_t* ahi, const uint64_t* alo, const uint32_t* av, long na,
                    const uint64_t* bhi, const uint64_t* blo, const uint32_t* bv, long nb,
                    uint64_t* ohi, uint64_t* olo, uint32_t* ov, hipStream_t st);
int hbmr_tera_tie_fix(const uint64_t* hi, uint64_t* lo, uint32_t* perm, long n,
                      unsigned int* flag, hipStream_t st);
int hbmr_tera_partition(const void* records, long n, int stride, const uint64_t* shi,
                        const uint64_t* slo, int nsplit, uint64_t* ohi, uint64_t* olo,
                        uint32_t* orow, long* offsets, unsigned long long* kmm, void* ws,
                        long ws_bytes, hipStream_t st);
#endif
long hbmr_radix_sort_workspace_bytes(long n);
long hbmr_tera_partition_workspace_bytes(long n, int nparts);

#ifndef HBMR_NO_HIP_DECLS
int hbmr_gemm_bf16_tn(const void* A, const void* Bt, void* C, long M, long N, long K, float alpha,
                      int out_bf16, hipStream_t st);
int hbmr_gemm_bf16_tn_ex(const void* A, const void* Bt, void* C, long M, long N, long K,
                         float alpha, int out_bf16, double* partials, hipStream_t st);
#endif
#ifndef HBMR_NO_HIP_DECLS
long hbmr_wc_tiles(long n);
int hbmr_wc_tokenize_count(const uint8_t* buf, long n, uint32_t* tile_counts, hipStream_t st);
int hbmr_wc_tokenize_write(const uint8_t* buf, long n, const long* tile_base, uint32_t* starts,
                           uint32_t* lens, hipStream_t st);
int hbmr_wc_insert(const uint8_t* buf, long n, const uint32_t* starts, const uint32_t* lens,
                   const int64_t* weights, long nwords, uint64_t* tkeys, uint64_t* tcounts,
                   long cap, int* overflow, hipStream_t st);
int hbmr_wc_compact(const uint8_t* buf, long n, const uint64_t* tkeys, const uint64_t* tcounts,
                    long cap, int R, uint32_t* ustart, uint32_t* ulen, int64_t* ucount,
                    int32_t* upart, unsigned int* counter, hipStream_t st);
int hbmr_wc_pack(const uint8_t* buf, const uint32_t* ustart, const uint32_t* ulen,
                 const int64_t* order, long nu, const int64_t* out_off, uint8_t* out,
                 hipStream_t st);
#endif
#ifndef HBMR_NO_HIP_DECLS
int hbmr_grep_cand_count(const uint8_t* buf, long n, const uint16_t* table,
                         const uint8_t* byteclass, int nstates, int nclasses, int start_bol,
                         int start_mid, uint32_t* tile_counts, int* non_ascii, hipStream_t st);
int hbmr_grep_cand_write(const uint8_t* buf, long n, const uint16_t* table,
                         const uint8_t* byteclass, int nstates, int nclasses, int start_bol,
                         int start_mid, const long* tile_base, uint32_t* pos, uint32_t* len,
                         int64_t* end, hipStream_t st);
long hbmr_grep_select_blocks(long nc);
int hbmr_grep_block_max(const int64_t* end, long nc, int64_t* block_max, hipStream_t st);
int hbmr_grep_prefix_max(const int64_t* end, long nc, const int64_t* block_prefix, int64_t* pmax,
                         hipStream_t st);
int hbmr_grep_select_count(const uint32_t* pos, const uint32_t* len, const int64_t* pmax, long nc,
                           uint32_t* block_counts, hipStream_t st);
int hbmr_grep_select_write(const uint32_t* pos, const uint32_t* len, const int64_t* pmax, long nc,
                           const long* block_base, uint32_t* spos, uint32_t* slen,
                           hipStream_t st);
int hbmr_span_insert(const uint8_t* buf, long n, const uint32_t* starts, const uint32_t* lens,
                     const int64_t* weights, long nspans, uint64_t* tkeys, uint64_t* tcounts,
                     long cap, int* overflow, hipStream_t st);
int hbmr_span_compact(const uint8_t* buf, const uint32_t* starts, const uint32_t* lens,
                      const uint64_t* tkeys, const uint64_t* tcounts, long cap, int R,
                      uint32_t* ustart, uint32_t* ulen, int64_t* ucount, int32_t* upart,
                      unsigned int* counter, hipStream_t st);
int hbmr_lines_count(const uint8_t* buf, long n, uint32_t* tile_counts, hipStream_t st);
int hbmr_lines_write(const uint8_t* buf, long n, const long* tile_base, uint32_t* starts,
                     uint32_t* lens, hipStream_t st);
int hbmr_recsort_hash_partition(const uint8_t* data, const int64_t* koff, const int64_t* klen,
                                long n, int nparts, uint32_t* part, hipStream_t st);
int hbmr_recsort_round_keys(const uint8_t* data, const int64_t* koff, const int64_t* klen,
                            const uint32_t* rec, long m, int d, uint64_t* keys, uint32_t* vals,
                            hipStream_t st);
long hbmr_recsort_round_workspace_bytes(long m);
int hbmr_recsort_round(const uint8_t* data, const int64_t* koff, const int64_t* klen, int d,
                       long m, int seg_bits, const uint32_t* act_pos, const uint32_t* act_rec,
                       const uint32_t* act_seg, uint32_t* perm, uint32_t* new_pos,
                       uint32_t* new_rec, uint32_t* new_seg, uint32_t* count, void* ws,
                       long ws_bytes, hipStream_t st);
int hbmr_recsort_cuts(const uint8_t* data, const int64_t* koff, const int64_t* klen,
                      const uint32_t* perm, long n, const uint8_t* sp, const int64_t* sp_off,
                      const int64_t* sp_len, int nsplit, int64_t* cuts, hipStream_t st);
int hbmr_recsort_chunk_bytes(void);
int hbmr_recsort_set_chunk_lanes(int lanes);
int hbmr_recsort_gather(const uint8_t* src, const uint32_t* perm, const int64_t* foff,
                        const int64_t* flen, const int64_t* dst_off, const int64_t* chunk_base,
                        const uint32_t* chunk_entry, long n, long nchunks, uint8_t* dst,
                        hipStream_t st);
int hbmr_recjoin_heads(const uint8_t* data, const int64_t* koff, const int64_t* klen, long n,
                       int32_t* head, uint32_t* bad, hipStream_t st);
int hbmr_recjoin_set_two_level(int on);
int hbmr_recjoin_rank(const uint8_t* pdata, const int64_t* pkoff, const int64_t* pklen,
                      const int32_t* prec, long np, const uint8_t* tdata, const int64_t* tkoff,
                      const int64_t* tklen, const int32_t* trec, const uint64_t* thk, long nt,
                      int32_t* lb, int32_t* eq, hipStream_t st);
int hbmr_recjoin_expand(const int64_t* tab, int S, const int64_t* base, const int32_t* mask,
                        const int32_t* first, const int32_t* cnt, const int32_t* osrc,
                        const int32_t* orec, long K, int override_op, const int32_t* hdr_len,
                        long lo, long T, int32_t* tkey, int32_t* trec, int64_t* tlen,
                        hipStream_t st);
int hbmr_recjoin_frames(const int64_t* tab, int S, const int32_t* mask, const int32_t* osrc,
                        const int32_t* orec, int override_op, const int32_t* hdr_len,
                        const int32_t* hdr_off, const uint8_t* hdr_bytes, long T,
                        const int32_t* tkey, const int32_t* trec, const int64_t* tlen,
                        const int64_t* dst_off, uint8_t* dst, int64_t* psrc, int64_t* plen,
                        int64_t* pdst, hipStream_t st);
int hbmr_recjoin_copy(const int64_t* psrc, const int64_t* plen, const int64_t* pdst,
                      const int64_t* chunk_base, const uint32_t* chunk_entry, long nchunks,
                      uint8_t* dst, hipStream_t st);
#endif
int hbmr_kmeans_padded_k(int k);
long hbmr_kmeans_accum_workspace_bytes(long n, int k);
long hbmr_kmeans_batch_workspace_bytes(long total_n, int ntasks, int k);

int hbmr_kmeans_map_cpu_f32(const float* X, long n, int d, const float* C, int k,
                            int32_t* labels, long long* sums, long long* counts, double* cost,
                            int fx_shift, int nthreads);
int hbmr_kmeans_map_cpu_f32_ex(const float* X, long n, int d, const float* C, int k,
                               int32_t* labels, long long* sums, long long* counts, double* cost,
                               int fx_shift, int nthreads, int exact, long* rescored);

#ifdef __cplusplus
}
#endif
```

native/kernels/kmeans.hip:

```cpp
#include "common.h"
#include "../include/hbmr/hbmr.h"
#include <algorithm>
#include <cstdlib>
#include <cstring>
#include <type_traits>
#include "kmeans/assign.h"
#include "kmeans/grouped.h"
#include "kmeans/combine.h"
#include "kmeans/refine.h"
#include "kmeans/image.h"
#include "kmeans/refine_queue.h"
#include "kmeans/fused.h"
#include "kmeans/bounded.h"
#include "kmeans/launch.h"

extern "C" {

int hbmr_kmeans_assign_bf16(const void* X, long n, int dp, const void* C, const float* chalf,
                            int k_pad, int32_t* labels, float* scores, hipStream_t st) {
  return dispatch_dp(dp, [&](auto D) {
    return launch_assign<D()>(X, n, C, chalf, k_pad, labels, scores, st);
  });
}

long hbmr_kmeans_accum_workspace_bytes(long n, int k) {
  return (long)(3 * ws_align(((size_t)k + 1) * 4) + ws_align((size_t)n * 4));
}

int hbmr_kmeans_accum_bf16(const void* X, long n, int dp, const int32_t* labels, int k,
                           long long* sums, long long* counts, int fx_shift, void* ws,
                           long ws_bytes, int mode, hipStream_t st) {
  return accum_impl<__bf16>(X, n, dp, labels, k, sums, counts, fx_shift, ws, ws_bytes, mode, st);
}

int hbmr_kmeans_accum_f32(const float* X, long n, int dp, const int32_t* labels, int k,
                          long long* sums, long long* counts, int fx_shift, void* ws,
                          long ws_bytes, int mode, hipStream_t st) {
  return accum_impl<float>(X, n, dp, labels, k, sums, counts, fx_shift, ws, ws_bytes, mode, st);
}

int hbmr_kmeans_update(const long long* sums, const long long* counts, int fx_shift, int k, int d,
                       int dp, int k_pad, float* cen, void* cbf, float* chalf, float* shift2,
                       hipStream_t st) {
  if (k <= 0) return 0;
  hipLaunchKernelGGL(kmeans_update_kernel, dim3(k), dim3(128), 0, st, sums, counts, k, d, dp,
                     ldexpf(1.0f, -fx_shift), cen, reinterpret_cast<__bf16*>(cbf), chalf, shift2);
  if (k_pad > k)
    hipLaunchKernelGGL(kmeans_pad_clusters_kernel, dim3(k_pad - k), dim3(64), 0, st,
                       reinterpret_cast<__bf16*>(cbf), chalf, k, k_pad, dp);
  return (int)hipGetLastError();
}

int hbmr_kmeans_padded_k(int k) { return ((k + kCK - 1) / kCK) * kCK; }

int hbmr_kmeans_padded_dim(int d) {
  for (int dp : {64, 128, 256})
    if (d <= dp) return dp;
  return -1;
}

int hbmr_f32_to_bf16_pad(const float* src, long n, int d, int dp, void* dst, hipStream_t st) {
  if (n <= 0) return 0;
  if (d > dp) return (int)hipErrorInvalidValue;
  const long total = n * dp;
  const long grid = std::min<long>((total + 255) / 256, 1L << 20);
  hipLaunchKernelGGL(f32_to_bf16_pad_kernel, dim3((unsigned)grid), dim3(256), 0, st, src, n, d,
                     dp, reinterpret_cast<uint16_t*>(dst));
  return (int)hipGetLastError();
}

long hbmr_kmeans_batch_workspace_bytes(long total_n, int ntasks, int k) {
  return (long)(ws_align((size_t)ntasks * k * 4) * 2 + ws_align((size_t)ntasks * (k + 1) * 4) +
                ws_align((size_t)total_n * 4));
}

int hbmr_kmeans_map_batch(int ntasks, const void* const* X, const long* n, int dp,
                          const void* C, const float* chalf, int k_pad, int k, int32_t* labels,
                          void* ws, long ws_bytes, long long* sums, long long* counts,
                          int fx_shift, int zero_outputs, hipStream_t st) {
  if (ntasks <= 0) return 0;
  if (zero_outputs) {
    HBMR_RETURN_IF_ERROR(hipMemsetAsync(sums, 0, (size_t)ntasks * k * dp * 8, st));
    HBMR_RETURN_IF_ERROR(hipMemsetAsync(counts, 0, (size_t)ntasks * k * 8, st));
  }
  long total = 0;
  for (int t = 0; t < ntasks; ++t) total += n[t];
  const bool small = ((size_t)k * AccCfg<128>::RS * 8 + (size_t)k * 4) <= 76 * 1024 && dp <= 128;
  if (!small && ntasks <= kMaxGroup && k <= 8192 &&
      ws_bytes >= hbmr_kmeans_batch_workspace_bytes(total, ntasks, k)) {
    set_lds_limits();
    return map_batch_grouped(ntasks, X, n, dp, C, chalf, k_pad, k, labels, ws, sums, counts,
                             fx_shift, st, cu_count());
  }
  long off = 0;
  for (int t = 0; t < ntasks; ++t) {
    int rc = hbmr_kmeans_assign_bf16(X[t], n[t], dp, C, chalf, k_pad, labels + off, nullptr, st);
    if (rc) return rc;
    rc = hbmr_kmeans_accum_bf16(X[t], n[t], dp, labels + off, k, sums + (size_t)t * k * dp,
                                counts + (size_t)t * k, fx_shift, ws, ws_bytes, 0, st);
    if (rc) return rc;
    off += n[t];
  }
  return 0;
}

long hbmr_kmeans_delta_workspace_bytes(long total_n, int ntasks, int k) {
  return (long)(2 * ws_align((size_t)ntasks * k * 4) + ws_align((size_t)ntasks * (k + 1) * 4) +
                ws_align((size_t)ntasks * 4) + 2 * ws_align((size_t)total_n * 8));
}

int hbmr_kmeans_delta_combine(int ntasks, const void* const* X, const long* n, int dp, int x_f32,
                              int k, const int32_t* labels, void* ws, long ws_bytes,
                              long long* sums, long long* counts, int fx_shift,
                              int32_t* const* g, const long long* const* S0,
                              const long long* const* N0, hipStream_t st) {
  if (ntasks <= 0) return 0;
  if (ntasks > kMaxGroup || k <= 0 || k > 8192 || (dp != 64 && dp != 128 && dp != 256))
    return (int)hipErrorInvalidValue;
  long total = 0;
  for (int i = 0; i < ntasks; ++i) {
    if (n[i] < 0 || n[i] >= (1L << 31)) return (int)hipErrorInvalidValue;
    total += n[i];
  }
  if (ws == nullptr || ws_bytes < hbmr_kmeans_delta_workspace_bytes(total, ntasks, k))
    return (int)hipErrorInvalidValue;
  set_lds_limits();
  return x_f32 ? delta_combine_impl<float>(ntasks, X, n, dp, k, labels, ws, sums, counts,
                                           fx_shift, g, S0, N0, st)
               : delta_combine_impl<__bf16>(ntasks, X, n, dp, k, labels, ws, sums, counts,
                                            fx_shift, g, S0, N0, st);
}

int hbmr_kmeans_map_batch_delta(int ntasks, const void* const* X, const long* n, int dp,
                                const void* C, const float* chalf, int k_pad, int k,
                                int32_t* labels, void* ws, long ws_bytes, long long* sums,
                                long long* counts, int fx_shift, int32_t* const* g,
                                const long long* const* S0, const long long* const* N0,
                                hipStream_t st) {
  if (ntasks <= 0) return 0;
  if (ntasks > kMaxGroup || k_pad % kCK) return (int)hipErrorInvalidValue;
  const int pts = assign_pts_of(dp);
  if (!pts) return (int)hipErrorInvalidValue;
  SplitTable t;
  make_split_table(t, ntasks, k, X, n);
  const long nb = split_blocks(t, [&](long m) { return (m + pts - 1) / pts; });
  if (nb > 0x7fffffffL) return (int)hipErrorInvalidValue;
  if (nb > 0) {
    launch_grouped_assign(dp, nb, t, C, chalf, k_pad, labels, st);
    HBMR_RETURN_IF_ERROR(hipGetLastError());
  }
  return hbmr_kmeans_delta_combine(ntasks, X, n, dp, 0, k, labels, ws, ws_bytes, sums, counts,
                                   fx_shift, g, S0, N0, st);
}

int hbmr_kmeans_assign_top3_bf16(const void* X, long n, int dp, const void* C, const float* chalf,
                                 int k_pad, int32_t* labels, int32_t* cand, float* scores,
                                 float* margin, hipStream_t st) {
  if (!labels || !cand || !scores || !margin) return (int)hipErrorInvalidValue;
  return dispatch_dp(dp, [&](auto D) {
    return launch_assign_top3<D(), false>(X, n, C, chalf, k_pad, labels, cand, scores, margin, st);
  });
}

int hbmr_kmeans_assign_top3_f16(const void* X, long n, int dp, const void* C, const float* chalf,
                                int k_pad, int32_t* labels, int32_t* cand, float* scores,
                                float* margin, hipStream_t st) {
  if (!labels || !cand || !scores || !margin) return (int)hipErrorInvalidValue;
  return dispatch_dp(dp, [&](auto D) {
    return launch_assign_top3<D(), true>(X, n, C, chalf, k_pad, labels, cand, scores, margin, st);
  });
}

int hbmr_kmeans_assign_top3_grouped(int nsplit, const void* const* X, const long* n, int dp,
                                    int f16, const void* C, const float* chalf, int k_pad,
                                    int32_t* labels, int32_t* cand, float* scores, float* margin,
                                    hipStream_t st) {
  if (!labels || !cand || !scores || !margin) return (int)hipErrorInvalidValue;
  return dispatch_dp(dp, [&](auto D) {
    return f16 ? launch_assign_top3_grouped<D(), true>(nsplit, X, n, C, chalf, k_pad, labels,
                                                       cand, scores, margin, st)
               : launch_assign_top3_grouped<D(), false>(nsplit, X, n, C, chalf, k_pad, labels,
                                                        cand, scores, margin, st);
  });
}

int hbmr_kmeans_assign_top3_q1_grouped(int nsplit, const void* const* X, const long* n, int dp,
                                       int f16, const void* C, const void* Ct,
                                       const float* chalf, int k_pad,
                                       int32_t* labels, const float* const* xnorm,
                                       const float* const* xbn2, const float* const* xerr,
                                       int d, int k, const float* cnorm, const float* cmax,
                                       const float* cerr, const float* cerrmax, void* ws,
                                       long ws_bytes, const float* dcc, hipStream_t st) {
  if (nsplit <= 0 || nsplit > kMaxGroup || k_pad % 32 || k <= 0 || k_pad < k ||
      d > kRefineMaxDp || !labels || ((uintptr_t)ws & 255) || (dp != 64 && dp != 128))
    return (int)hipErrorInvalidValue;
  TopQ1Table t;
  memset(&t, 0, sizeof(t));
  t.nsplit = nsplit;
  long total = 0, nb = 0;
  for (int i = 0; i < nsplit; ++i) {
    if (n[i] < 0 || n[i] > 0x7fffffffL) return (int)hipErrorInvalidValue;
    fill_topq1(t, i, X, xnorm, xbn2, xerr, total, nb);
    total += n[i];
    nb += ceil_div(n[i], kFusedPts);
  }
  t.off[nsplit] = total;
  t.blk[nsplit] = nb;
  const RefineLayout Ly = refine_layout(nsplit, n);
  if (ws_bytes < (long)Ly.bytes) return (int)hipErrorInvalidValue;
  char* w = static_cast<char*>(ws);
  HBMR_RETURN_IF_ERROR(hipMemsetAsync(w, 0, kHdrClear, st));
  if (nb == 0) return 0;
  if (nb > 0x7fffffffL) return (int)hipErrorInvalidValue;
  const FusedQ1Fin fin = make_fused_fin(k, d, k_pad, cnorm, cerr, dcc, cmax, cerrmax, w, Ly);
  if (exact_kernel() == 3) {
    if (!Ct) return (int)hipErrorInvalidValue;
    const auto [kern, lds] = fused_kernel(dp, f16, [](auto D, auto F) {
      return &kmeans_assign_top3_q1_v3_kernel<D(), F()>;
    });
    hipLaunchKernelGGL(kern, dim3((unsigned)nb), dim3(256), lds, st, t,
                       reinterpret_cast<const __bf16*>(Ct), chalf, k_pad / 32, labels, fin);
    return (int)hipGetLastError();
  }
  const auto [kern, lds] = fused_kernel(dp, f16, [](auto D, auto F) {
    return &kmeans_assign_top3_q1_grouped_kernel<D(), F()>;
  });
  hipLaunchKernelGGL(kern, dim3((unsigned)nb), dim3(AssignV2<64>::THREADS), lds, st, t,
                     reinterpret_cast<const __bf16*>(C), chalf, k_pad / 32, labels, fin);
  return (int)hipGetLastError();
}

long hbmr_kmeans_bound_workspace_bytes(long total, int nsplit, int k) {
  if (total < 0 || nsplit <= 0 || nsplit > kMaxGroup || k <= 0) return -1;
  const size_t sh = ((size_t)nsplit * k * sizeof(float) + 255) & ~(size_t)255;
  return (long)(kBoundHdr + sh + (size_t)total * sizeof(uint32_t));
}

int hbmr_kmeans_assign_top3_q1_bounded(int nsplit, const void* const* X, const long* n, int dp,
                                       int f16, const void* Ct, const float* chalf, int k_pad,
                                       int32_t* labels, const float* const* xnorm,
                                       const float* const* xbn2, const float* const* xerr,
                                       int d, int k, const float* cnorm, const float* cmax,
                                       const float* cerr, const float* cerrmax, void* ws,
                                       long ws_bytes, const float* dcc,
                                       const int32_t* const* g, float* const* gap,
                                       const float* const* ref, const float* cen, void* bws,
                                       long bws_bytes, unsigned long long* skipped,
                                       hipStream_t st) {
  if (nsplit <= 0 || nsplit > kMaxGroup || k_pad % 32 || k <= 0 || k_pad < k || d <= 0 ||
      d > kRefineMaxDp || !labels || ((uintptr_t)ws & 255) || (dp != 64 && dp != 128) || !Ct ||
      !g || !gap || !ref || !cen || !bws || ((uintptr_t)bws & 255))
    return (int)hipErrorInvalidValue;
  TopQ1Table t;
  SweepTable sw;
  GapTable gt;
  ShiftTable sh;
  memset(&t, 0, sizeof(t));
  memset(&sw, 0, sizeof(sw));
  memset(&gt, 0, sizeof(gt));
  memset(&sh, 0, sizeof(sh));
  t.nsplit = sw.nsplit = nsplit;
  long total = 0, nb = 0, nsb = 0;
  int nref = 0;
  for (int i = 0; i < nsplit; ++i) {
    if (n[i] < 0 || n[i] > 0x7fffffffL || (n[i] > 0 && (!gap[i] || (ref[i] && !g[i]))))
      return (int)hipErrorInvalidValue;
    fill_topq1(t, i, X, xnorm, xbn2, xerr, total, nb);
    sw.off[i] = total;
    sw.blk[i] = nsb;
    sw.n[i] = n[i];
    sw.g[i] = g[i];
    gt.gap[i] = gap[i];
    if (ref[i]) {
      int r = 0;
      while (r < nref && sh.ref[r] != ref[i]) ++r;
      if (r == nref) sh.ref[nref++] = ref[i];
      sw.rid[i] = r;
      sw.gap[i] = gap[i];
    }
    total += n[i];
    nb += ceil_div(n[i], kFusedPts);
    nsb += ceil_div(n[i], 256 * kSweepPer);
  }
  t.off[nsplit] = total;
  t.blk[nsplit] = nb;
  sw.blk[nsplit] = nsb;
  const RefineLayout Ly = refine_layout(nsplit, n);
  if (ws_bytes < (long)Ly.bytes ||
      bws_bytes < hbmr_kmeans_bound_workspace_bytes(total, nsplit, k))
    return (int)hipErrorInvalidValue;
  char* w = static_cast<char*>(ws);
  char* bw = static_cast<char*>(bws);
  HBMR_RETURN_IF_ERROR(hipMemsetAsync(w, 0, kHdrClear, st));
  if (nb == 0) return 0;
  if (nb > 0x7fffffffL) return (int)hipErrorInvalidValue;
  HBMR_RETURN_IF_ERROR(hipMemsetAsync(bw, 0, kBoundHdr, st));
  uint32_t* cnt = reinterpret_cast<uint32_t*>(bw);
  uint32_t* smax = cnt + kMaxGroup;
  float* shift = reinterpret_cast<float*>(bw + kBoundHdr);
  uint32_t* idx = reinterpret_cast<uint32_t*>(
      bw + kBoundHdr + (((size_t)nsplit * k * sizeof(float) + 255) & ~(size_t)255));
  if (nref > 0) {
    hipLaunchKernelGGL(kmeans_bound_shift_kernel, dim3((unsigned)k, (unsigned)nref), dim3(64), 0,
                       st, sh, cen, k, d, shift, smax);
    HBMR_RETURN_IF_ERROR(hipGetLastError());
  }
  hipLaunchKernelGGL(kmeans_bound_sweep_kernel, dim3((unsigned)nsb), dim3(256), 0, st, sw, k,
                     shift, reinterpret_cast<const float*>(smax), labels, cnt, idx);
  HBMR_RETURN_IF_ERROR(hipGetLastError());
  const FusedQ1Fin fin = make_fused_fin(k, d, k_pad, cnorm, cerr, dcc, cmax, cerrmax, w, Ly);
  const auto [kern, lds] = fused_kernel(dp, f16, [](auto D, auto F) {
    return &kmeans_assign_top3_q1_bounded_kernel<D(), F()>;
  });
  hipLaunchKernelGGL(kern, dim3((unsigned)nb), dim3(256), lds, st, t, gt,
                     reinterpret_cast<const __bf16*>(Ct), chalf, k_pad / 32, labels, fin,
                     (const uint32_t*)cnt, (const uint32_t*)idx, skipped);
  return (int)hipGetLastError();
}

int hbmr_kmeans_refine_f32(const float* X32, long n, int d, int ldx, const float* xnorm,
                           const float* xbn2, const float* xerr, const float* C32, int k,
                           int k_pad, const float* cnorm, const float* cmax, const float* cerr,
                           const float* cerrmax, const int32_t* nbr_idx,
                           const float* nbr_dist, int L, int32_t* labels, const int32_t* cand,
                           const float* scores, const float* margin, unsigned long long* stats,
                           int nstats, hipStream_t st) {
  if (n <= 0) return 0;
  if (d > ldx || d > kRefineMaxDp || k <= 0 || k_pad < k || L < 1 || L > k)
    return (int)hipErrorInvalidValue;
  const double pack_rel = pack_rel_of(k_pad);
  const long blocks = (n + 255) / 256;
  const bool v2_ok = d % 8 == 0 && ldx % 4 == 0 && ((uintptr_t)X32 & 15) == 0 &&
                     ((uintptr_t)C32 & 15) == 0;
  if (v2_ok) {
    auto kern = d <= 128 ? kmeans_refine_v2_kernel<1> : kmeans_refine_v2_kernel<2>;
    hipLaunchKernelGGL(kern, dim3((unsigned)blocks), dim3(256), 0, st, X32, n, d, ldx, xnorm,
                       xbn2, xerr, C32, k, cnorm, cmax, cerr, cerrmax, pack_rel, nbr_idx,
                       nbr_dist, L, labels, cand, scores, margin, stats, nstats);
    return (int)hipGetLastError();
  }
  hipLaunchKernelGGL(kmeans_refine_kernel, dim3((unsigned)blocks), dim3(256), 0, st, X32, n, d,
                     ldx, xnorm, xbn2, xerr, C32, k, cnorm, cmax, cerr, cerrmax, pack_rel,
                     nbr_idx, nbr_dist, L,
                     labels, cand, scores, margin, stats, nstats);
  return (int)hipGetLastError();
}


int hbmr_kmeans_exact_prep(const float* x, long n, int d, int ldx, int dp, int f16, void* x16,
                           float* xnorm, float* xn2, float* xerr, hipStream_t st) {
  if (n <= 0) return 0;
  if (d > ldx || d > dp || dp % 8 || !x16 || !xnorm || !xn2 || !xerr)
    return (int)hipErrorInvalidValue;
  const long blocks = (n + 15) / 16;
  if (blocks > 0x7fffffffL) return (int)hipErrorInvalidValue;
  hipLaunchKernelGGL(kmeans_exact_prep_kernel, dim3((unsigned)blocks), dim3(256), 0, st, x, n, d,
                     ldx, dp, f16, reinterpret_cast<uint16_t*>(x16), xnorm, xn2, xerr);
  return (int)hipGetLastError();
}

int hbmr_kmeans_set_exact_kernel(int v) {
  const int old = g_exact_kernel;
  g_exact_kernel = v == 2 || v == 3 ? v : -1;
  return old;
}

int hbmr_kmeans_get_exact_kernel(void) { return exact_kernel(); }

int hbmr_kmeans_image16_tiled(const void* c16, int k_pad, int dp, void* c16t, hipStream_t st) {
  if (k_pad <= 0 || k_pad % 32 || (dp != 64 && dp != 128) || !c16 || !c16t)
    return (int)hipErrorInvalidValue;
  const long pieces = (long)k_pad * dp / 8;
  hipLaunchKernelGGL(kmeans_image16_tiled_kernel, dim3((unsigned)((pieces + 255) / 256)),
                     dim3(256), 0, st, reinterpret_cast<const uint4*>(c16), k_pad, dp,
                     reinterpret_cast<uint4*>(c16t));
  return (int)hipGetLastError();
}

int hbmr_kmeans_image16(const float* cen, int k, int d, int dp, int k_pad, int f16, void* c16,
                        float* chalf, float* cnorm, float* cerr, float* maxima, hipStream_t st) {
  if (k <= 0 || k_pad < k || d > dp) return (int)hipErrorInvalidValue;
  HBMR_RETURN_IF_ERROR(hipMemsetAsync(maxima, 0, 2 * sizeof(float), st));
  hipLaunchKernelGGL(kmeans_image16_kernel, dim3((unsigned)k_pad), dim3(128), 0, st, cen, k, d,
                     dp, f16, reinterpret_cast<uint16_t*>(c16), chalf, cnorm, cerr,
                     reinterpret_cast<unsigned*>(maxima));
  return (int)hipGetLastError();
}

int hbmr_kmeans_centroid_nbr(const float* cen, int k, int d, int L, int32_t* di, float* dv,
                             float* pd, hipStream_t st) {
  if (k <= 0 || k > kNbrMaxK || d <= 0 || d > kNbrMaxD || L <= 0 || L > k)
    return (int)hipErrorInvalidValue;
  if (((uintptr_t)cen & 15) != 0) return (int)hipErrorInvalidValue;
  int kp2 = 1;
  while (kp2 < k) kp2 <<= 1;
  const size_t lds = (size_t)kp2 * sizeof(unsigned long long);
  static bool lds_set = false;
  if (!lds_set) {
    HBMR_RETURN_IF_ERROR(hipFuncSetAttribute((const void*)kmeans_centroid_nbr_kernel,
                                             hipFuncAttributeMaxDynamicSharedMemorySize,
                                             (int)(kNbrMaxK * sizeof(unsigned long long))));
    lds_set = true;
  }
  const double rel = (double)(d + 4) * 0x1p-53 * 1.01;
  hipLaunchKernelGGL(kmeans_centroid_nbr_kernel, dim3((unsigned)k), dim3(kNbrThreads), lds, st,
                     cen, k, d, L, kp2, rel, di, dv, pd);
  return (int)hipGetLastError();
}


long hbmr_kmeans_refine_batch_bytes(int nsplit, const long* ns) {
  if (nsplit <= 0 || nsplit > kMaxGroup) return -1;
  return (long)refine_layout(nsplit, ns).bytes;
}

int hbmr_kmeans_refine_batch_q1(int nsplit, const long* ns, int s, int d, int k, int k_pad,
                                const float* xnorm, const float* xbn2, const float* xerr,
                                const float* cnorm, const float* cmax, const float* cerr,
                                const float* cerrmax, const int32_t* labels, const int32_t* cand,
                                const float* scores, const float* margin,
                                unsigned long long* stats, void* ws, long ws_bytes, int reset,
                                const float* dcc, hipStream_t st) {
  if (nsplit <= 0 || nsplit > kMaxGroup || s < 0 || s >= nsplit || k <= 0 || k_pad < k ||
      d > kRefineMaxDp || ((uintptr_t)ws & 255))
    return (int)hipErrorInvalidValue;
  for (int i = 0; i < nsplit; ++i)
    if (ns[i] < 0 || ns[i] > 0x7fffffffL) return (int)hipErrorInvalidValue;
  const RefineLayout Ly = refine_layout(nsplit, ns);
  if (ws_bytes < (long)Ly.bytes) return (int)hipErrorInvalidValue;
  char* w = static_cast<char*>(ws);
  uint32_t* c1 = reinterpret_cast<uint32_t*>(w);
  if (reset) HBMR_RETURN_IF_ERROR(hipMemsetAsync(c1, 0, kHdrClear, st));
  const long n = ns[s];
  if (n == 0) return 0;
  const double pack_rel = pack_rel_of(k_pad);
  const long b1 = ceil_div(n, 256 * kQ1Per);
  hipLaunchKernelGGL(kmeans_refine_q1_kernel, dim3((unsigned)b1), dim3(256), 0, st, n, s, d, k,
                     xnorm, xbn2, xerr, cnorm, cmax, cerr, cerrmax, pack_rel, labels, cand,
                     scores, margin, c1, reinterpret_cast<ExactQ1*>(w + Ly.off1), Ly.cap1,
                     reinterpret_cast<unsigned long long*>(w + kStatsOff), dcc);
  return (int)hipGetLastError();
}

int hbmr_kmeans_refine_batch_q1g(int nsplit, const long* ns, int d, int k, int k_pad,
                                 const float* const* xnorm, const float* const* xbn2,
                                 const float* const* xerr, const float* cnorm, const float* cmax,
                                 const float* cerr, const float* cerrmax, const int32_t* labels,
                                 const int32_t* cand, const float* scores, const float* margin,
                                 void* ws, long ws_bytes, const float* dcc, hipStream_t st) {
  if (nsplit <= 0 || nsplit > kMaxGroup || k <= 0 || k_pad < k || d > kRefineMaxDp ||
      ((uintptr_t)ws & 255))
    return (int)hipErrorInvalidValue;
  Q1Table t;
  memset(&t, 0, sizeof(t));
  t.nsplit = nsplit;
  long total = 0, nb = 0;
  for (int i = 0; i < nsplit; ++i) {
    if (ns[i] < 0 || ns[i] > 0x7fffffffL) return (int)hipErrorInvalidValue;
    t.n[i] = ns[i];
    fill_topq1(t, i, nullptr, xnorm, xbn2, xerr, total, nb);
    total += ns[i];
    nb += ceil_div(ns[i], 256 * kQ1Per);
  }
  t.blk[nsplit] = nb;
  t.total = total;
  const RefineLayout Ly = refine_layout(nsplit, ns);
  if (ws_bytes < (long)Ly.bytes) return (int)hipErrorInvalidValue;
  char* w = static_cast<char*>(ws);
  uint32_t* c1 = reinterpret_cast<uint32_t*>(w);
  HBMR_RETURN_IF_ERROR(hipMemsetAsync(c1, 0, kHdrClear, st));
  if (nb == 0) return 0;
  const double pack_rel = pack_rel_of(k_pad);
  hipLaunchKernelGGL(kmeans_refine_q1_grouped_kernel, dim3((unsigned)nb), dim3(256), 0, st, t, d,
                     k, cnorm, cmax, cerr, cerrmax, pack_rel, labels, cand, scores, margin, c1,
                     reinterpret_cast<ExactQ1*>(w + Ly.off1), Ly.cap1,
                     reinterpret_cast<unsigned long long*>(w + kStatsOff), dcc);
  return (int)hipGetLastError();
}

int hbmr_kmeans_refine_batch_finish(int nsplit, const long* ns, const float* const* x32,
                                    int32_t* const* labels, int d, int ldx, const float* C32,
                                    int k, int k_pad, const float* cmax, const float* cerrmax,
                                    const int32_t* nbr_idx, const float* nbr_dist, int L,
                                    unsigned long long* stats, int nstats, void* ws,
                                    long ws_bytes, hipStream_t st) {
  if (nsplit <= 0 || nsplit > kMaxGroup || d > ldx || d > kRefineMaxDp || d % 8 || ldx % 4 ||
      k <= 0 || k_pad < k || L < 1 || L > k || nstats < 3 || ((uintptr_t)C32 & 15) ||
      ((uintptr_t)ws & 255))
    return (int)hipErrorInvalidValue;
  const RefineLayout Ly = refine_layout(nsplit, ns);
  if (ws_bytes < (long)Ly.bytes) return (int)hipErrorInvalidValue;
  RefineTable tbl;
  std::memset(&tbl, 0, sizeof(tbl));
  tbl.nsplit = nsplit;
  for (int i = 0; i < nsplit; ++i) {
    if ((uintptr_t)x32[i] & 15) return (int)hipErrorInvalidValue;
    tbl.x32[i] = x32[i];
    tbl.labels[i] = labels[i];
  }
  const double pack_rel = pack_rel_of(k_pad);
  char* w = static_cast<char*>(ws);
  uint32_t* c1 = reinterpret_cast<uint32_t*>(w);
  uint32_t* c2 = c1 + kQShards;
  const ExactQ1* q1 = reinterpret_cast<const ExactQ1*>(w + Ly.off1);
  ExactQ2* q2 = reinterpret_cast<ExactQ2*>(w + Ly.off2);
  unsigned long long* ss = reinterpret_cast<unsigned long long*>(w + kStatsOff);
  const unsigned g3 = std::max(1u, Ly.g2);
  if (d <= 128) {
    hipLaunchKernelGGL(kmeans_refine_q2_kernel<1>, dim3(Ly.g2), dim3(256), 0, st, tbl, d, ldx,
                       C32, k, cmax, cerrmax, pack_rel, c1, q1, Ly.cap1, c2, q2, Ly.cap2, ss);
    HBMR_RETURN_IF_ERROR(hipGetLastError());
    hipLaunchKernelGGL(kmeans_refine_q3_kernel<1>, dim3(g3), dim3(256), 0, st, tbl, d, ldx, C32,
                       k, nbr_idx, nbr_dist, L, c2, q2, Ly.cap2, ss, nstats);
  } else {
    hipLaunchKernelGGL(kmeans_refine_q2_kernel<2>, dim3(Ly.g2), dim3(256), 0, st, tbl, d, ldx,
                       C32, k, cmax, cerrmax, pack_rel, c1, q1, Ly.cap1, c2, q2, Ly.cap2, ss);
    HBMR_RETURN_IF_ERROR(hipGetLastError());
    hipLaunchKernelGGL(kmeans_refine_q3_kernel<2>, dim3(g3), dim3(256), 0, st, tbl, d, ldx, C32,
                       k, nbr_idx, nbr_dist, L, c2, q2, Ly.cap2, ss, nstats);
  }
  HBMR_RETURN_IF_ERROR(hipGetLastError());
  hipLaunchKernelGGL(kmeans_refine_stats_kernel, dim3(1), dim3(64), 0, st, ss, stats, nstats);
  return (int)hipGetLastError();
}

}
```

native/kernels/kmeans/bounded.h:

```cpp
#pragma once
#include "../common.h"
#include "fused.h"

namespace {

constexpr int kSweepPer = 8;
constexpr int kBoundHdr = 512;

struct ShiftTable {
  const float* ref[kMaxGroup];
};

__global__ __launch_bounds__(64) void kmeans_bound_shift_kernel(
    const ShiftTable tbl, const float* __restrict__ cen, int k, int d, float* __restrict__ shift,
    uint32_t* __restrict__ smax) {
  const int j = blockIdx.x, r = blockIdx.y;
  const float* a = cen + (size_t)j * d;
  const float* b = tbl.ref[r] + (size_t)j * d;
  double acc = 0.0;
  for (int i = threadIdx.x; i < d; i += 64) {
    const double e = (double)a[i] - (double)b[i];
    acc = fma(e, e, acc);
  }
#pragma unroll
  for (int off = 1; off < 64; off <<= 1) acc += __shfl_xor(acc, off);
  if (threadIdx.x == 0) {
    const float s = __double2float_ru(sqrt(acc) * (1.0 + 0x1p-40));
    shift[(size_t)r * k + j] = s;
    atomicMax(smax + r, __float_as_uint(s));
  }
}

__device__ __forceinline__ float sub_rd_pos(float a, float b) {
  const float t = a - b;
  if (!(t > 0x1p-100f)) return 0.f;
  const float bb = t - a;
  const float err = (a - (t - bb)) - (b + bb);
  return err < 0.f ? __uint_as_float(__float_as_uint(t) - 1u) : t;
}

struct SweepTable {
  int nsplit;
  const int32_t* g[kMaxGroup];
  float* gap[kMaxGroup];
  int rid[kMaxGroup];
  long n[kMaxGroup];
  long off[kMaxGroup];
  long blk[kMaxGroup + 1];
};

__global__ __launch_bounds__(256) void kmeans_bound_sweep_kernel(
    const SweepTable tbl, int k, const float* __restrict__ shift,
    const float* __restrict__ smax, int32_t* __restrict__ labels, uint32_t* __restrict__ cnt,
    uint32_t* __restrict__ idx) {
  const long b = blockIdx.x;
  int lo = 0, hi = tbl.nsplit;
  while (hi - lo > 1) {
    const int mid = (lo + hi) >> 1;
    if (tbl.blk[mid] <= b) lo = mid; else hi = mid;
  }
  const int s = __builtin_amdgcn_readfirstlane(lo);
  const int tid = threadIdx.x, lane = tid & 63, wave = tid >> 6;
  const long n = tbl.n[s], o = tbl.off[s];
  const int32_t* __restrict__ g = tbl.g[s];
  float* __restrict__ gap = tbl.gap[s];
  const float* __restrict__ sh = shift + (size_t)tbl.rid[s] * k;
  const float sm = gap ? smax[tbl.rid[s]] : 0.f;
  const long p0 = (b - tbl.blk[s]) * (256 * kSweepPer);
  __shared__ uint32_t wcnt[4][kSweepPer];
  __shared__ uint32_t base_s;
  bool list[kSweepPer];
  uint32_t rank[kSweepPer];
#pragma unroll
  for (int i = 0; i < kSweepPer; ++i) {
    const long p = p0 + i * 256 + tid;
    list[i] = false;
    if (p < n) {
      list[i] = true;
      if (gap) {
        const int32_t c = g[p];
        const float v =
            (uint32_t)c < (uint32_t)k ? sub_rd_pos(sub_rd_pos(gap[p], sh[c]), sm) : 0.f;
        if (v > 0.f) {
          list[i] = false;
          labels[o + p] = c;
          gap[p] = v;
        }
      }
    }
    const unsigned long long m = __ballot(list[i]);
    rank[i] = lane_rank(m);
    if (lane == 0) wcnt[wave][i] = (uint32_t)__popcll(m);
  }
  __syncthreads();
  if (tid == 0) {
    uint32_t tot = 0;
#pragma unroll
    for (int w = 0; w < 4; ++w)
#pragma unroll
      for (int i = 0; i < kSweepPer; ++i) {
        const uint32_t c = wcnt[w][i];
        wcnt[w][i] = tot;
        tot += c;
      }
    base_s = tot ? atomicAdd(cnt + s, tot) : 0u;
  }
  __syncthreads();
  uint32_t* out = idx + o + base_s;
#pragma unroll
  for (int i = 0; i < kSweepPer; ++i)
    if (list[i]) out[wcnt[wave][i] + rank[i]] = (uint32_t)(p0 + i * 256 + tid);
}

struct GapTable {
  float* gap[kMaxGroup];
};

template <int D, bool F16>
__global__ __launch_bounds__(256, kExactMinB) void kmeans_assign_top3_q1_bounded_kernel(
    const TopQ1Table tbl, const GapTable gt, const __bf16* __restrict__ Ct,
    const float* __restrict__ chalf, int ntiles, int32_t* __restrict__ labels, FusedQ1Fin fin,
    const uint32_t* __restrict__ cnt, const uint32_t* __restrict__ idx,
    unsigned long long* __restrict__ skipped) {
  extern __shared__ __attribute__((aligned(16))) char smem[];
  if (blockIdx.x == 0 && threadIdx.x == 0 && skipped != nullptr) {
    unsigned long long sk = 0;
    for (int i = 0; i < tbl.nsplit; ++i)
      sk += (unsigned long long)(tbl.off[i + 1] - tbl.off[i]) - cnt[i];
    if (sk) atomicAdd(skipped, sk);
  }
  const long b = hbmr_xcd_remap(blockIdx.x, gridDim.x);
  int lo = 0, hi = tbl.nsplit;
  while (hi - lo > 1) {
    const int mid = (lo + hi) >> 1;
    if (tbl.blk[mid] <= b) lo = mid; else hi = mid;
  }
  const int s = __builtin_amdgcn_readfirstlane(lo);
  const long nl = (long)__builtin_amdgcn_readfirstlane(cnt[s]);
  const long lb = b - tbl.blk[s];
  if (lb * 256 >= nl) return;
  const long o = tbl.off[s];
  fin.xnorm = tbl.xnorm[s];
  fin.xbn2 = tbl.xbn2[s];
  fin.xerr = tbl.xerr[s];
  fin.sidx = s;
  fin.idx = idx + o;
  fin.gap = gt.gap[s];
  assign_tile_v3<D, F16, true>(tbl.X[s], nl, Ct, chalf, ntiles, labels + o, lb, smem, fin);
}


}
```

native/kernels/kmeans/fused.h:

```cpp
#pragma once
#include "../common.h"
#include "assign.h"
#include "grouped.h"
#include "refine_queue.h"

namespace {

struct FusedQ1Fin {
  const float* xnorm;
  const float* xbn2;
  const float* xerr;
  int sidx;
  int k;
  double gam, pack_rel;
  const float* cmax_p;
  const float* cerrmax_p;
  const float* cnorm;
  const float* cerr;
  const float* dcc;
  uint32_t* qcount;
  ExactQ1* q1;
  long cap1;
  unsigned long long* stats;
  const uint32_t* idx;
  float* gap;

  template <class AM, int PB, bool BND = false>
  __device__ __forceinline__ void operator()(const AM (&am)[PB], int h, long p0, int col, long n,
                                             int32_t* __restrict__ labels) const {
    const int tid = threadIdx.x, lane = tid & 63, wave = tid >> 6;
    __shared__ uint32_t fq_cnt[4 * PB];
    __shared__ uint32_t fq_base;
    const int shard = blockIdx.x % kQShards;
    const double inflate = 1.0 + 0x1p-20;
    const double cem = (double)cerrmax_p[0] * inflate;
    const double cm = (double)cmax_p[0] * inflate + cem;
    ExactQ1 e[PB];
    bool flag[PB];
    uint32_t rank[PB];
#pragma unroll
    for (int pb = 0; pb < PB; ++pb) {
      float v[3];
      int c[3];
      am[pb].top3(v[0], v[1], v[2]);
#pragma unroll
      for (int i = 0; i < 3; ++i) c[i] = am[pb].cluster(v[i], h);
      float ov[3];
      int oc[3];
#pragma unroll
      for (int i = 0; i < 3; ++i) {
        ov[i] = __shfl_xor(v[i], 32);
        oc[i] = __shfl_xor(c[i], 32);
      }
#pragma unroll
      for (int i = 0; i < 3; ++i) insert3(v, c, ov[i], oc[i]);
      if (((c[0] ^ c[1]) & AM::TMASK) == 0) {
        v[2] = v[0];
        c[2] = c[0];
      }
      const long p = p0 + pb * 32 + col;
      flag[pb] = false;
      if (h == 0 && p < n) {
        long row = p;
        if constexpr (BND) row = idx[p];
        labels[row] = c[0];
        const float bs = am[pb].score(v[0]);
        const float m2 = bs - am[pb].score(v[1]);
        ExactQ1& q = e[pb];
        q.row = (uint32_t)row;
        q.split = (uint32_t)sidx;
        q.b = c[0];
        q.s = c[1];
        q.t = c[2];
        q.sb = bs;
        q.m3 = bs - am[pb].score(v[2]);
        q.x2 = xbn2[row];
        q.xn = xnorm[row];
        q.xe = xerr[row];
        q.pad0 = q.pad1 = 0.f;
        if constexpr (BND) {
          float gp = 0.f;
          flag[pb] = q.s < k && q1_certify<true>(q, m2, cnorm[q.b], cerr[q.b], k, gam, cm, cem,
                                                 pack_rel, cnorm, cerr, dcc, gp);
          gap[row] = gp;
        } else {
          flag[pb] = q.s < k && q1_flagged(q, m2, cnorm[q.b], cerr[q.b], k, gam, cm, cem,
                                           pack_rel, cnorm, cerr, dcc);
        }
      }
      const unsigned long long m = __ballot(flag[pb]);
      rank[pb] = lane_rank(m);
      if (lane == 0) fq_cnt[wave * PB + pb] = (uint32_t)__popcll(m);
    }
    __syncthreads();
    if (tid == 0) {
      uint32_t tot = 0;
#pragma unroll
      for (int i = 0; i < 4 * PB; ++i) {
        const uint32_t c = fq_cnt[i];
        fq_cnt[i] = tot;
        tot += c;
      }
      fq_base = tot ? atomicAdd(qcount + shard, tot) : 0u;
      if (tot) atomicAdd(stats + 4 * shard, (unsigned long long)tot);
    }
    __syncthreads();
    ExactQ1* out = q1 + (long)shard * cap1 + fq_base;
#pragma unroll
    for (int pb = 0; pb < PB; ++pb)
      if (flag[pb]) out[fq_cnt[wave * PB + pb] + rank[pb]] = e[pb];
  }
};

template <int D>
__device__ __forceinline__ void stage_tile32t(char* buf, const __bf16* __restrict__ Ct,
                                              const float* __restrict__ chalf, int tile, int wave,
                                              int lane) {
  using V = AssignV2<D>;
  const uint32_t loff = (uint32_t)lane * 16u;
#pragma unroll
  for (int i = 0; i < V::P; ++i) {
    const int base = (i * V::WAVES + wave) * HBMR_WAVE;
    const char* g = reinterpret_cast<const char*>(Ct) + (size_t)tile * V::TILE_BYTES +
                    (size_t)base * 16;
    __builtin_amdgcn_global_load_lds((const void*)(g + loff), (void*)(buf + base * 16), 16, 0, 0);
  }
  if (wave == 0 && lane < 32) {
    const char* g = reinterpret_cast<const char*>(chalf + (size_t)tile * 32);
    __builtin_amdgcn_global_load_lds((const void*)(g + loff / 4u), (void*)(buf + V::TILE_BYTES),
                                     4, 0, 0);
  }
}

__device__ __forceinline__ void tile_codes(uint32_t top, int t, uint32_t (&code)[16]) {
  const uint32_t base = top - ((uint32_t)t << 4);
#pragma unroll
  for (int r = 0; r < 16; ++r) {
    code[r] = base | (15u - r);
    asm("" : "+s"(code[r]));
  }
}

__device__ __forceinline__ void top2_insert(PackedTop2x8& am, const f32x16& acc,
                                            const uint32_t (&code)[16], uint32_t vmask) {
  constexpr int NT = PackedTop2x8::NT;
#pragma unroll
  for (int r = 0; r < 16; ++r) {
    if ((r / NT) % 2) continue;
    const float u = __uint_as_float((__float_as_uint(acc[r]) & vmask) | code[r]);
    const float v = __uint_as_float((__float_as_uint(acc[r + NT]) & vmask) | code[r + NT]);
    const float m = vmed3(am.tb[r % NT], u, v);
    am.ts[r % NT] = vmax3(m, am.ts[r % NT], am.ts[r % NT]);
    am.tb[r % NT] = vmax3(am.tb[r % NT], u, v);
  }
}

template <int D, bool F16, bool BND = false>
__device__ __forceinline__ void assign_tile_v3(const __bf16* __restrict__ X, long n,
                                               const __bf16* __restrict__ Ct,
                                               const float* __restrict__ chalf, int ntiles,
                                               int32_t* __restrict__ labels, long blk, char* smem,
                                               const FusedQ1Fin& fin) {
  static_assert(D <= 128, "v3 keeps two 32-point blocks of D <= 128 in registers");
  constexpr int PB = 2, NS = 4;
  using V = AssignV2<D, NS>;
  static_assert(V::WAVES == 4, "v3: 4 waves per workgroup");
  constexpr int KS = V::KS;
  static_assert(V::TILE_BYTES == 32 * D * 2, "tile layout");
  const int tid = threadIdx.x;
  const int wave = __builtin_amdgcn_readfirstlane(tid / HBMR_WAVE);
  const int lane = tid & (HBMR_WAVE - 1);
  const int h = lane >> 5;
  const int col = lane & 31;
  const long p0 = blk * (V::WAVES * PB * 32) + (long)wave * PB * 32;
  const int rowoff = h * 512 + col * 16;
  auto frag = [&](const char* row, int s) __attribute__((always_inline)) {
    return *reinterpret_cast<const bf16x8*>(row + s * 1024);
  };
  auto bias = [&](const char* buf, f32x16& acc) __attribute__((always_inline)) {
    const float* ch = reinterpret_cast<const float*>(buf + V::TILE_BYTES);
#pragma unroll
    for (int g = 0; g < 4; ++g) {
      const f32x4 v = *reinterpret_cast<const f32x4*>(ch + 8 * g + 4 * h);
      acc[4 * g + 0] = v[0];
      acc[4 * g + 1] = v[1];
      acc[4 * g + 2] = v[2];
      acc[4 * g + 3] = v[3];
    }
  };

#pragma unroll
  for (int i = 0; i < NS; ++i)
    if (i < ntiles) stage_tile32t<D>(smem + i * V::BUF, Ct, chalf, i, wave, lane);

  bf16x8 bfrag[PB][KS];
#pragma unroll
  for (int pb = 0; pb < PB; ++pb) {
    long p = p0 + pb * 32 + col;
    if (p >= n) p = n - 1;
    if constexpr (BND) p = fin.idx[p];
    const uint4* row = reinterpret_cast<const uint4*>(X + p * D);
#pragma unroll
    for (int s = 0; s < KS; ++s) bfrag[pb][s] = __builtin_bit_cast(bf16x8, row[2 * s + h]);
  }
  PackedTop2x8 am[PB];
#pragma unroll
  for (int pb = 0; pb < PB; ++pb) am[pb].init(ntiles);
  asm volatile("s_waitcnt vmcnt(0)" ::: "memory");
#pragma unroll
  for (int pb = 0; pb < PB; ++pb)
#pragma unroll
    for (int s = 0; s < KS; ++s) asm volatile("" : "+v"(bfrag[pb][s]));
  __syncthreads();
  const bool w0 = wave == 0;
  const uint32_t top = am[0].top;
  const uint32_t vmask = am[0].vmask;

  bf16x8 a[KS];
  f32x16 bz;
  {
    const char* row = smem + rowoff;
#pragma unroll
    for (int s = 0; s < KS; ++s) a[s] = frag(row, s);
    bias(smem, bz);
  }
  int slot = 0;
  for (int t = 0; t < ntiles; ++t) {
    wait_tile_dmas<V::P, NS - 2>(max(0, min(NS - 2, ntiles - 2 - t)), w0);
    asm volatile("s_waitcnt lgkmcnt(0)" ::: "memory");
    __syncthreads();
    char* rbuf = smem + slot * V::BUF;
    if (t + NS < ntiles) stage_tile32t<D>(rbuf, Ct, chalf, t + NS, wave, lane);
    slot = slot + 1 == NS ? 0 : slot + 1;
    const char* nbuf = smem + slot * V::BUF;
    const char* nrow = nbuf + rowoff;
    f32x16 acc[PB];
#pragma unroll
    for (int s = 0; s < KS; ++s) {
#pragma unroll
      for (int pb = 0; pb < PB; ++pb)
        acc[pb] = mfma32x32x16<F16>(a[s], bfrag[pb][s], s == 0 ? bz : acc[pb]);
      a[s] = frag(nrow, s);
    }
    uint32_t code[16];
    tile_codes(top, t, code);
#pragma unroll
    for (int pb = 0; pb < PB; ++pb) top2_insert(am[pb], acc[pb], code, vmask);
    bias(nbuf, bz);
  }
  fin.template operator()<PackedTop2x8, PB, BND>(am, h, p0, col, n, labels);
}

struct TopQ1Table {
  int nsplit;
  const __bf16* X[kMaxGroup];
  const float* xnorm[kMaxGroup];
  const float* xbn2[kMaxGroup];
  const float* xerr[kMaxGroup];
  long off[kMaxGroup + 1];
  long blk[kMaxGroup + 1];
};

template <int D, bool F16>
__global__ __launch_bounds__(AssignV2<D>::THREADS, kExactMinB) void
kmeans_assign_top3_q1_grouped_kernel(const TopQ1Table tbl, const __bf16* __restrict__ C,
                                     const float* __restrict__ chalf, int ntiles,
                                     int32_t* __restrict__ labels, FusedQ1Fin fin) {
  extern __shared__ __attribute__((aligned(16))) char smem[];
  const long b = hbmr_xcd_remap(blockIdx.x, gridDim.x);
  int lo = 0, hi = tbl.nsplit;
  while (hi - lo > 1) {
    const int mid = (lo + hi) >> 1;
    if (tbl.blk[mid] <= b) lo = mid; else hi = mid;
  }
  const int s = __builtin_amdgcn_readfirstlane(lo);
  const long o = tbl.off[s];
  fin.xnorm = tbl.xnorm[s];
  fin.xbn2 = tbl.xbn2[s];
  fin.xerr = tbl.xerr[s];
  fin.sidx = s;
  assign_tile_v2<D, 2, true, F16, FusedQ1Fin>(tbl.X[s], tbl.off[s + 1] - o, C, chalf, ntiles,
                                              labels + o, nullptr, b - tbl.blk[s], smem, nullptr,
                                              nullptr, -1, &fin);
}

template <int D, bool F16>
__global__ __launch_bounds__(256, kExactMinB) void kmeans_assign_top3_q1_v3_kernel(
    const TopQ1Table tbl, const __bf16* __restrict__ Ct, const float* __restrict__ chalf,
    int ntiles, int32_t* __restrict__ labels, FusedQ1Fin fin) {
  extern __shared__ __attribute__((aligned(16))) char smem[];
  const long b = hbmr_xcd_remap(blockIdx.x, gridDim.x);
  int lo = 0, hi = tbl.nsplit;
  while (hi - lo > 1) {
    const int mid = (lo + hi) >> 1;
    if (tbl.blk[mid] <= b) lo = mid; else hi = mid;
  }
  const int s = __builtin_amdgcn_readfirstlane(lo);
  const long o = tbl.off[s];
  fin.xnorm = tbl.xnorm[s];
  fin.xbn2 = tbl.xbn2[s];
  fin.xerr = tbl.xerr[s];
  fin.sidx = s;
  assign_tile_v3<D, F16>(tbl.X[s], tbl.off[s + 1] - o, Ct, chalf, ntiles, labels + o,
                         b - tbl.blk[s], smem, fin);
}

}
```

native/kernels/kmeans/refine_queue.h:

```cpp
#pragma once
#include "../common.h"
#include <algorithm>
#include "grouped.h"
#include "refine.h"

namespace {

struct ExactQ1 {
  uint32_t row, split;
  int32_t b, s, t;
  float sb, m3, x2, xn, xe, pad0, pad1;
};
struct ExactQ2 {
  uint32_t row, split;
  int32_t w, pad;
  double dw;
};
static_assert(sizeof(ExactQ1) == 48 && sizeof(ExactQ2) == 24, "queue entry layout");

constexpr int kQShards = 8;
constexpr int kQ1Per = 4;
constexpr int kQ2Lanes = 8;
constexpr int kQ2Per = HBMR_WAVE / kQ2Lanes;
constexpr int kRefineGrid = 2048;
constexpr int kStatsOff = 64;
constexpr int kRefineHdr = 512;
constexpr int kHdrClear = kStatsOff + kQShards * 4 * 8;

struct RefineTable {
  int nsplit;
  const float* x32[kMaxGroup];
  int32_t* labels[kMaxGroup];
};

__host__ __device__ inline long ceil_div(long a, long b) { return (a + b - 1) / b; }

struct RefineLayout {
  long cap1, cap2;
  unsigned g2;
  size_t off1, off2, bytes;
};
inline RefineLayout refine_layout(int nsplit, const long* ns) {
  RefineLayout L;
  long total = 0, cap1 = 0, nb_fused = 0;
  for (int i = 0; i < nsplit; ++i) {
    total += ns[i];
    cap1 += ceil_div(ceil_div(ns[i], 256 * kQ1Per), kQShards) * 256 * kQ1Per;
    nb_fused += ceil_div(ns[i], 256);
  }
  L.cap1 = std::max<long>(cap1, ceil_div(nb_fused, kQShards) * 256);
  L.g2 = (unsigned)std::max<long>(1, std::min<long>(kRefineGrid, ceil_div(total, 4 * kQ2Per)));
  const long per_iter = (long)L.g2 * 4 * kQ2Per;
  L.cap2 = ceil_div(L.g2, kQShards) * 4 * kQ2Per * std::max<long>(1, ceil_div(total, per_iter));
  L.off1 = kRefineHdr;
  L.off2 = L.off1 + ((kQShards * (size_t)L.cap1 * sizeof(ExactQ1) + 255) & ~(size_t)255);
  L.bytes = L.off2 + kQShards * (size_t)L.cap2 * sizeof(ExactQ2);
  return L;
}

__device__ __forceinline__ long shard_slot(const uint32_t (&c)[kQShards], long cap, uint32_t i) {
  uint32_t acc = 0;
  long slot = 0;
#pragma unroll
  for (int j = 0; j < kQShards; ++j) {
    if (i >= acc && i < acc + c[j]) slot = (long)j * cap + (i - acc);
    acc += c[j];
  }
  return slot;
}

__device__ __forceinline__ uint32_t lane_rank(unsigned long long m) {
  return __builtin_amdgcn_mbcnt_hi((uint32_t)(m >> 32), __builtin_amdgcn_mbcnt_lo((uint32_t)m, 0u));
}

template <bool GAP>
__device__ __forceinline__ bool q1_certify(const ExactQ1& e, float m2, float cnb, float ceb, int k,
                                           double gam, double cm, double cem, double pack_rel,
                                           const float* __restrict__ cnorm,
                                           const float* __restrict__ cerr,
                                           const float* __restrict__ dcc, float& gap) {
  const double inflate = 1.0 + 0x1p-20;
  const double xn = ((double)e.xn + (double)e.xe) * inflate;
  const double x2 = (double)e.x2;
  const double sb = e.sb;
  const double mm = m2;
  const double amax = ((double)e.xe + cem) * inflate;
  double eb, es, dl_b, dl_s;
  exact_bound(sb, ((double)cnb + (double)ceb) * inflate, xn, x2,
              ((double)e.xe + (double)ceb) * inflate, gam, pack_rel, eb, dl_b);
  exact_bound(sb - mm, cm, xn, x2, amax, gam, pack_rel, es, dl_s);
  bool flag = !(mm > eb + es && dl_s >= 2.0 * amax);
  double marg = mm - (eb + es);
  const int b = e.b, sc = e.s, t = e.t;
  if (flag && dcc != nullptr && t < k && t != b) {
    const double ex = (double)e.xe * inflate;
    const double ebb = (double)ceb * inflate;
    const double ess = (double)cerr[sc] * inflate;
    const double dbs = ((double)dcc[(size_t)b * k + sc] + (double)ceb + (double)cerr[sc]) *
                       inflate;
    double eap_b, rb, eap_s, rs;
    score_err(sb, ((double)cnb + (double)ceb) * inflate, xn, x2, gam, pack_rel, eap_b, rb);
    score_err(sb - mm, ((double)cnorm[sc] + (double)cerr[sc]) * inflate, xn, x2, gam,
              pack_rel, eap_s, rs);
    const double ep = dbs * ex + rs * ess + rb * ebb + 0.5 * (ex + ebb) * (ex + ebb) +
                      eap_b + eap_s;
    double et, dl_t;
    const double m3 = e.m3;
    exact_bound(sb - m3, cm, xn, x2, amax, gam, pack_rel, et, dl_t);
    if (mm > ep && m3 > eb + et && dl_t >= 2.0 * amax) {
      flag = false;
      if constexpr (GAP) marg = fmin(mm - ep, m3 - (eb + et));
    }
  }
  if constexpr (GAP) {
    gap = 0.f;
    if (!flag && marg > 0.0) {
      const double ctb = ((double)cnb + (double)ceb) * inflate;
      const double eacc = gam * (xn * ctb + 0.5 * ctb * ctb);
      const double slack = 2.0 * (eacc + fabs(sb) * pack_rel) + x2 * 0x1p-22;
      const double r = sqrt(fmax(0.0, x2 - 2.0 * sb) + slack) * (1.0 + 0x1p-40) +
                       ((double)e.xe + (double)ceb) * inflate;
      const double delta = 2.0 * marg * (1.0 - 0x1p-30);
      const double g = delta / (sqrt(r * r + delta) * (1.0 + 0x1p-40) + r) * (1.0 - 0x1p-30);
      gap = fmaxf(0.f, __double2float_rd(g));
    }
  }
  return flag;
}

__device__ __forceinline__ bool q1_flagged(const ExactQ1& e, float m2, float cnb, float ceb, int k,
                                           double gam, double cm, double cem, double pack_rel,
                                           const float* __restrict__ cnorm,
                                           const float* __restrict__ cerr,
                                           const float* __restrict__ dcc) {
  float unused;
  return q1_certify<false>(e, m2, cnb, ceb, k, gam, cm, cem, pack_rel, cnorm, cerr, dcc, unused);
}

__device__ __forceinline__ void refine_q1_block(
    long n, int sidx, long blk, int d, int k, const float* __restrict__ xnorm,
    const float* __restrict__ xbn2, const float* __restrict__ xerr,
    const float* __restrict__ cnorm, const float* __restrict__ cmax,
    const float* __restrict__ cerr, const float* __restrict__ cerrmax, double pack_rel,
    const int32_t* __restrict__ labels, const int32_t* __restrict__ cand,
    const float* __restrict__ score, const float* __restrict__ margin, long cs,
    uint32_t* __restrict__ qcount, ExactQ1* __restrict__ q1, long cap1,
    unsigned long long* __restrict__ stats, const float* __restrict__ dcc) {
  const int tid = threadIdx.x, lane = tid & 63, wave = tid >> 6;
  const int shard = blockIdx.x % kQShards;
  __shared__ uint32_t wcnt[4][kQ1Per];
  __shared__ uint32_t base_s;
  const double inflate = 1.0 + 0x1p-20;
  const double gam = (double)(d + 2) * 0x1p-23 * 1.01;
  const double cem = (double)cerrmax[0] * inflate;
  const double cm = (double)cmax[0] * inflate + cem;
  ExactQ1 e[kQ1Per];
  bool in[kQ1Per];
  float m2[kQ1Per];
#pragma unroll
  for (int i = 0; i < kQ1Per; ++i) {
    const long p = blk * (256 * kQ1Per) + i * 256 + tid;
    in[i] = p < n;
    const long q = in[i] ? p : n - 1;
    e[i].row = (uint32_t)q;
    e[i].split = (uint32_t)sidx;
    e[i].b = labels[q];
    e[i].s = cand[q];
    e[i].t = cand[cs + q];
    e[i].sb = score[q];
    m2[i] = margin[q];
    e[i].m3 = margin[cs + q];
    e[i].x2 = xbn2[q];
    e[i].xn = xnorm[q];
    e[i].xe = xerr[q];
  }
  float cnb[kQ1Per], ceb[kQ1Per];
#pragma unroll
  for (int i = 0; i < kQ1Per; ++i) {
    cnb[i] = cnorm[e[i].b];
    ceb[i] = cerr[e[i].b];
  }
  bool flag[kQ1Per];
  uint32_t rank[kQ1Per];
#pragma unroll
  for (int i = 0; i < kQ1Per; ++i) {
    flag[i] = in[i] && e[i].s < k &&
              q1_flagged(e[i], m2[i], cnb[i], ceb[i], k, gam, cm, cem, pack_rel, cnorm, cerr, dcc);
    const unsigned long long m = __ballot(flag[i]);
    rank[i] = lane_rank(m);
    if (lane == 0) wcnt[wave][i] = (uint32_t)__popcll(m);
  }
  __syncthreads();
  if (tid == 0) {
    uint32_t tot = 0;
#pragma unroll
    for (int w = 0; w < 4; ++w)
#pragma unroll
      for (int i = 0; i < kQ1Per; ++i) {
        const uint32_t c = wcnt[w][i];
        wcnt[w][i] = tot;
        tot += c;
      }
    base_s = tot ? atomicAdd(qcount + shard, tot) : 0u;
    if (tot) atomicAdd(stats + 4 * shard, (unsigned long long)tot);
  }
  __syncthreads();
  ExactQ1* out = q1 + (long)shard * cap1 + base_s;
#pragma unroll
  for (int i = 0; i < kQ1Per; ++i)
    if (flag[i]) out[wcnt[wave][i] + rank[i]] = e[i];
}

__global__ __launch_bounds__(256) void kmeans_refine_q1_kernel(
    long n, int sidx, int d, int k, const float* __restrict__ xnorm,
    const float* __restrict__ xbn2, const float* __restrict__ xerr,
    const float* __restrict__ cnorm, const float* __restrict__ cmax,
    const float* __restrict__ cerr, const float* __restrict__ cerrmax, double pack_rel,
    const int32_t* __restrict__ labels, const int32_t* __restrict__ cand,
    const float* __restrict__ score, const float* __restrict__ margin,
    uint32_t* __restrict__ qcount, ExactQ1* __restrict__ q1, long cap1,
    unsigned long long* __restrict__ stats, const float* __restrict__ dcc) {
  refine_q1_block(n, sidx, blockIdx.x, d, k, xnorm, xbn2, xerr, cnorm, cmax, cerr, cerrmax,
                  pack_rel, labels, cand, score, margin, n, qcount, q1, cap1, stats, dcc);
}

struct Q1Table {
  int nsplit;
  long total;
  long n[kMaxGroup];
  long off[kMaxGroup];
  long blk[kMaxGroup + 1];
  const float* xnorm[kMaxGroup];
  const float* xbn2[kMaxGroup];
  const float* xerr[kMaxGroup];
};

__global__ __launch_bounds__(256) void kmeans_refine_q1_grouped_kernel(
    const Q1Table tbl, int d, int k, const float* __restrict__ cnorm,
    const float* __restrict__ cmax, const float* __restrict__ cerr,
    const float* __restrict__ cerrmax, double pack_rel, const int32_t* __restrict__ labels,
    const int32_t* __restrict__ cand, const float* __restrict__ score,
    const float* __restrict__ margin, uint32_t* __restrict__ qcount, ExactQ1* __restrict__ q1,
    long cap1, unsigned long long* __restrict__ stats, const float* __restrict__ dcc) {
  const long b = blockIdx.x;
  int lo = 0, hi = tbl.nsplit;
  while (hi - lo > 1) {
    const int mid = (lo + hi) >> 1;
    if (tbl.blk[mid] <= b) lo = mid; else hi = mid;
  }
  const int s = __builtin_amdgcn_readfirstlane(lo);
  const long o = tbl.off[s];
  refine_q1_block(tbl.n[s], s, b - tbl.blk[s], d, k, tbl.xnorm[s], tbl.xbn2[s], tbl.xerr[s],
                  cnorm, cmax, cerr, cerrmax, pack_rel, labels + o, cand + o, score + o,
                  margin + o, tbl.total, qcount, q1, cap1, stats, dcc);
}

template <int NM>
__device__ __forceinline__ void load_row16(const float* __restrict__ r, int d, int sub,
                                           float (&v)[16 * NM]) {
#pragma unroll
  for (int m = 0; m < NM; ++m) {
#pragma unroll
    for (int h = 0; h < 4; ++h) {
      const int b = 128 * m + 32 * h + 4 * sub;
      const bool ok = b < d;
      const float4 a = *reinterpret_cast<const float4*>(r + (ok ? b : 0));
      float* o = v + 16 * m + 4 * h;
      o[0] = ok ? a.x : 0.f; o[1] = ok ? a.y : 0.f; o[2] = ok ? a.z : 0.f; o[3] = ok ? a.w : 0.f;
    }
  }
}

__device__ __forceinline__ float row_sum8f(float v) {
  v += __shfl_xor(v, 1);
  v += __shfl_xor(v, 2);
  v += __shfl_xor(v, 4);
  return v;
}

__device__ __forceinline__ double row_sum8(double v) {
  v += dpp_f64<0xB1>(v);
  v += dpp_f64<0x4E>(v);
  v += dpp_f64<0x141>(v);
  return v;
}

template <int NM>
__global__ __launch_bounds__(256) void kmeans_refine_q2_kernel(
    const RefineTable tbl, int d, int ldx, const float* __restrict__ C32, int k,
    const float* __restrict__ cmax, const float* __restrict__ cerrmax, double pack_rel,
    const uint32_t* __restrict__ qcount, const ExactQ1* __restrict__ q1, long cap1,
    uint32_t* __restrict__ q2count, ExactQ2* __restrict__ q2, long cap2,
    unsigned long long* __restrict__ sstats) {
  constexpr uint32_t kPerBlk = 4 * kQ2Per;
  constexpr uint32_t kBuf = 256;
  const int tid = threadIdx.x, lane = tid & 63, wave = tid >> 6;
  const int grp = lane / kQ2Lanes, sub = lane % kQ2Lanes;
  __shared__ ExactQ2 sbuf[kBuf];
  __shared__ uint32_t sn, sbase;
  __shared__ unsigned long long cnt[2];
  if (tid < 2) cnt[tid] = 0;
  if (tid == 0) sn = 0;
  __syncthreads();
  const double inflate = 1.0 + 0x1p-20;
  const double gam = (double)(d + 2) * 0x1p-23 * 1.01;
  const double cem = (double)cerrmax[0] * inflate;
  const double cm = (double)cmax[0] * inflate + cem;
  uint32_t c1[kQShards];
  uint32_t total = 0;
#pragma unroll
  for (int j = 0; j < kQShards; ++j) {
    c1[j] = qcount[j];
    total += c1[j];
  }
  const int shard = blockIdx.x % kQShards;
  const uint32_t stride = gridDim.x * kPerBlk;
  const uint32_t off = wave * kQ2Per + grp;
  auto flush = [&]() {
    if (tid == 0) {
      sbase = atomicAdd(q2count + shard, sn);
      cnt[1] += sn;
    }
    __syncthreads();
    const uint32_t m = sn;
    for (uint32_t i = tid; i < m; i += 256) q2[(long)shard * cap2 + sbase + i] = sbuf[i];
    __syncthreads();
    if (tid == 0) sn = 0;
    __syncthreads();
  };
  uint32_t bb = blockIdx.x * kPerBlk;
  ExactQ1 e;
  if (bb < total) e = q1[shard_slot(c1, cap1, min(bb + off, total - 1))];
  for (; bb < total; bb += stride) {
    const ExactQ1 q = e;
    const bool have = bb + off < total;
    const uint32_t nb = bb + stride;
    if (nb < total) e = q1[shard_slot(c1, cap1, min(nb + off, total - 1))];
    const bool t_real = q.t < k;
    const float* xr = tbl.x32[q.split] + (size_t)q.row * ldx;
    float xf[16 * NM], c0[16 * NM], c1r[16 * NM], c2[16 * NM];
    load_row16<NM>(xr, d, sub, xf);
    load_row16<NM>(C32 + (size_t)q.b * d, d, sub, c0);
    load_row16<NM>(C32 + (size_t)q.s * d, d, sub, c1r);
    load_row16<NM>(C32 + (size_t)(t_real ? q.t : q.b) * d, d, sub, c2);
    float f0 = 0.f, f1 = 0.f, f2 = 0.f;
#pragma unroll
    for (int i = 0; i < 16 * NM; ++i) {
      const float e0 = xf[i] - c0[i], e1 = xf[i] - c1r[i], e2 = xf[i] - c2[i];
      f0 = fmaf(e0, e0, f0);
      f1 = fmaf(e1, e1, f1);
      f2 = fmaf(e2, e2, f2);
    }
    f0 = row_sum8f(f0);
    f1 = row_sum8f(f1);
    f2 = row_sum8f(f2);
    const double rel = (double)(16 * NM + 8) * 0x1p-24 * 1.01, aeps = 0x1p-120;
    int w = q.b;
    double dw = f0;
    if ((double)f1 < dw || ((double)f1 == dw && q.s < w)) { w = q.s; dw = f1; }
    if (t_real && ((double)f2 < dw || ((double)f2 == dw && q.t < w))) { w = q.t; dw = f2; }
    const double whi = dw * (1.0 + rel) + aeps;
    auto beats = [&](double dj) { return dj * (1.0 - rel) - aeps > whi; };
    bool separated = isfinite(whi) &&
                     (w == q.b || beats(f0)) && (w == q.s || beats(f1)) &&
                     (!t_real || w == q.t || beats(f2));
    dw = whi;
    bool certified = !t_real && separated;
    if (t_real && separated) {
      const double xn = ((double)q.xn + (double)q.xe) * inflate;
      const double x2 = (double)q.x2;
      const double amax = ((double)q.xe + cem) * inflate;
      const double st = (double)q.sb - (double)q.m3;
      double et, dl_t;
      exact_bound(st, cm, xn, x2, amax, gam, pack_rel, et, dl_t);
      certified = 0.5 * (x2 - dw) - x2 * 0x1p-23 > st + et && dl_t >= 2.0 * amax;
    }
    if (have && sub == 0 && certified && w != q.b) {
      tbl.labels[q.split][q.row] = w;
      atomicAdd(&cnt[0], 1ull);
    }
    const bool spill = have && sub == 0 && !certified;
    const unsigned long long m = __ballot(spill);
    if (m) {
      uint32_t b2 = 0;
      if (lane == 0) b2 = atomicAdd(&sn, (uint32_t)__popcll(m));
      b2 = __shfl(b2, 0);
      if (spill) {
        ExactQ2 o;
        o.row = q.row;
        o.split = q.split;
        o.w = w;
        o.pad = 0;
        o.dw = dw;
        sbuf[b2 + lane_rank(m)] = o;
      }
    }
    __syncthreads();
    if (sn > kBuf - kPerBlk) flush();
  }
  __syncthreads();
  if (sn) flush();
  if (tid < 2 && cnt[tid]) atomicAdd(sstats + 4 * shard + 1 + tid, cnt[tid]);
}

template <int NM>
__global__ __launch_bounds__(256) void kmeans_refine_q3_kernel(
    const RefineTable tbl, int d, int ldx, const float* __restrict__ C32, int k,
    const int32_t* __restrict__ nbr_idx, const float* __restrict__ nbr_dist, int L,
    const uint32_t* __restrict__ q2count, const ExactQ2* __restrict__ q2, long cap2,
    unsigned long long* __restrict__ sstats, int nstats) {
  const int tid = threadIdx.x, lane = tid & 63;
  const int grp = lane / kRefineGroup, sub = lane % kRefineGroup;
  __shared__ unsigned long long cnt[3];
  if (tid < 3) cnt[tid] = 0;
  __syncthreads();
  uint32_t c2[kQShards];
  uint32_t total = 0;
#pragma unroll
  for (int j = 0; j < kQShards; ++j) {
    c2[j] = q2count[j];
    total += c2[j];
  }
  const uint32_t nwaves = gridDim.x * 4;
  const uint32_t gw = blockIdx.x * 4 + (tid >> 6);
  for (uint32_t base = gw * 4; base < total; base += nwaves * 4) {
    const uint32_t idx = base + grp;
    const bool have = idx < total;
    const ExactQ2 q = q2[shard_slot(c2, cap2, have ? idx : base)];
    int32_t* lab = tbl.labels[q.split];
    const int b0 = lab[q.row];
    double xv[8 * NM];
    {
      float xf[8 * NM];
      load_row8<NM>(tbl.x32[q.split] + (size_t)q.row * ldx, d, sub, xf);
#pragma unroll
      for (int i = 0; i < 8 * NM; ++i) xv[i] = (double)xf[i];
    }
    const int w0 = q.w;
    int w = w0;
    double dw;
    {
      const float* c0p[1] = {C32 + (size_t)w0 * d};
      double d0[1];
      rows_dist2<NM, 1>(xv, c0p, d, sub, d0);
      dw = d0[0];
    }
    const double r0 = sqrt(dw);
    bool done = false;
    const int32_t* ni = nbr_idx + (size_t)w0 * L;
    const float* nd = nbr_dist + (size_t)w0 * L;
    const float* cw0 = C32 + (size_t)w0 * d;
    int evals = 0;
    for (int jj = 0; jj < L; jj += kElkanStep) {
      const double lim = (r0 + sqrt(dw)) * (1.0 + 0x1p-40);
      if ((double)nd[jj] > lim) {
        done = true;
        break;
      }
      int jv[kElkanStep];
      const float* cp[kElkanStep];
#pragma unroll
      for (int v = 0; v < kElkanStep; ++v) {
        const bool ok = jj + v < L && (double)nd[jj + v] <= lim;
        jv[v] = ok ? ni[jj + v] : -1;
        cp[v] = ok ? C32 + (size_t)jv[v] * d : cw0;
      }
      double dj[kElkanStep];
      rows_dist2<NM, kElkanStep>(xv, cp, d, sub, dj);
      evals += kElkanStep;
#pragma unroll
      for (int v = 0; v < kElkanStep; ++v)
        if (jv[v] >= 0 && (dj[v] < dw || (dj[v] == dw && jv[v] < w))) { w = jv[v]; dw = dj[v]; }
    }
    const bool full = !done && L < k;
    if (full) {
      for (int j = 0; j < k; j += 4) {
        const float* cp[4];
#pragma unroll
        for (int v = 0; v < 4; ++v) cp[v] = C32 + (size_t)(j + v < k ? j + v : j) * d;
        double dj[4];
        rows_dist2<NM, 4>(xv, cp, d, sub, dj);
#pragma unroll
        for (int v = 0; v < 4; ++v)
          if (j + v < k && (dj[v] < dw || (dj[v] == dw && j + v < w))) { w = j + v; dw = dj[v]; }
      }
    }
    if (have && sub == 0) {
      atomicAdd(&cnt[1], (unsigned long long)evals);
      if (full) atomicAdd(&cnt[2], 1ull);
      if (w != b0) atomicAdd(&cnt[0], 1ull);
      lab[q.row] = w;
    }
  }
  __syncthreads();
  const int sh = blockIdx.x % (kQShards / 2);
  if (tid == 0 && cnt[0]) atomicAdd(sstats + 4 * sh + 1, cnt[0]);
  if (tid == 1 && cnt[1]) atomicAdd(sstats + 4 * sh + 3, cnt[1]);
  if (tid == 2 && cnt[2]) atomicAdd(sstats + 4 * (sh + kQShards / 2) + 3, cnt[2]);
}

__global__ void kmeans_refine_stats_kernel(const unsigned long long* __restrict__ ss,
                                           unsigned long long* __restrict__ stats, int nstats) {
  const int t = threadIdx.x;
  if (t >= 5 || (t >= 3 && nstats < 5)) return;
  unsigned long long v = 0;
  if (t < 3) {
    for (int j = 0; j < kQShards; ++j) v += ss[4 * j + t];
  } else {
    for (int j = 0; j < kQShards / 2; ++j) v += ss[4 * (j + (t - 3) * (kQShards / 2)) + 3];
  }
  if (v) stats[t] += v;
}

}
```

Measured before the change: 10730.

## Record refined second-best gap bounds from exact refine passes to skip more points

```diff
diff --git a/hbmr/models/kmeans.py b/hbmr/models/kmeans.py
--- a/hbmr/models/kmeans.py
+++ b/hbmr/models/kmeans.py
@@ -29,6 +29,7 @@
 EXACT_MFMA_KEY = "hbmr.kmeans.exact.mfma"
 COMBINER_KEY = "hbmr.kmeans.combiner"
 BOUNDS_KEY = "hbmr.kmeans.exact.bounds"
+BOUNDS_REFINE_KEY = "hbmr.kmeans.exact.bounds.refine"
 
 _M32 = 0xFFFFFFFF
 
@@ -238,7 +239,8 @@
 
 
 def _baseline_bytes(b) -> int:
-    return sum(t.numel() * t.element_size() for t in (b.g, b.S0, b.N0, getattr(b, "gap", None))
+    return sum(t.numel() * t.element_size() for t in (b.g, b.S0, b.N0, getattr(b, "gap", None),
+                                                          getattr(b, "gap2", None))
                if t is not None)
 
 
@@ -288,7 +290,7 @@
     with _EXACT_LOCK:
         t = _EXACT_SKIPPED.get(key)
         if t is None:
-            t = _EXACT_SKIPPED[key] = torch.zeros(1, dtype=torch.int64, device=device)
+            t = _EXACT_SKIPPED[key] = torch.zeros(2, dtype=torch.int64, device=device)
         return t
 
 
@@ -311,6 +313,7 @@
         self.exact_dtype = torch.bfloat16 if (conf.get(EXACT_MFMA_KEY) or "f16").lower() in (
             "bf16", "bfloat16") else torch.float16
         self.bounds = conf.get_boolean(BOUNDS_KEY, True)
+        self.bounds_refine = conf.get_boolean(BOUNDS_REFINE_KEY, True)
         self.combiner = (conf.get(COMBINER_KEY) or "delta").lower()
         if self.combiner not in ("delta", "sorted"):
             raise ValueError(f"{COMBINER_KEY} must be delta or sorted, not {self.combiner!r}")
@@ -569,11 +572,12 @@
             hb = [bases[i] for i in have]
             bounded = self.bounds and self.combiner == "delta" and km.bounds_supported(img)
             if bounded:
-                nogap = [b for b in hb if b.gap is None]
+                before = {id(b): _baseline_bytes(b) for b in hb}
+                esk = _exact_skipped(self.cin, ctx.device)
                 km.assign_exact_batch([datas[i] for i in have], img, stats, lab, scratch,
-                                      stream=ctx.stream, bounds=hb,
-                                      skipped=_exact_skipped(self.cin, ctx.device))
-                grown = {id(b): b.gap.numel() * b.gap.element_size() for b in nogap}
+                                      stream=ctx.stream, bounds=hb, skipped=esk[0:1],
+                                      refine_bounds=self.bounds_refine, held=esk[1:2])
+                grown = {id(b): max(0, _baseline_bytes(b) - before[id(b)]) for b in hb}
             else:
                 km.assign_exact_batch([datas[i] for i in have], img, stats, lab, scratch,
                                       stream=ctx.stream)
@@ -705,11 +709,12 @@
             if est is not None:
                 vals += list(est.double().unbind(0))
             if esk is not None:
-                vals.append(esk[0].double())
+                vals += list(esk.double().unbind(0))
             got = torch.stack(vals).tolist()
             shift, npts = got[0], got[1]
             if esk is not None:
-                ctx.reporter.incrCounter("KMEANS", "EXACT_BOUND_SKIPPED_POINTS", int(got[-1]))
+                ctx.reporter.incrCounter("KMEANS", "EXACT_BOUND_SKIPPED_POINTS", int(got[-2]))
+                ctx.reporter.incrCounter("KMEANS", "EXACT_BOUND_HELD_POINTS", int(got[-1]))
             if est is not None:
                 for name, v in zip(("EXACT_FLAGGED_POINTS", "EXACT_RELABELLED_POINTS",
                                     "EXACT_NEIGHBOUR_SCANS"), got[2:5]):
diff --git a/hbmr/ops/_lib.py b/hbmr/ops/_lib.py
--- a/hbmr/ops/_lib.py
+++ b/hbmr/ops/_lib.py
@@ -44,6 +44,14 @@
                                                    c_void_p, c_long, c_void_p,
                                                    c_void_p, c_void_p, c_void_p, c_void_p,
                                                    c_void_p, c_long, c_void_p, c_void_p]),
+    "hbmr_kmeans_assign_top3_q1_bounded2": (c_int, [c_int, c_void_p, c_void_p, c_int, c_int,
+                                                    c_void_p, c_void_p, c_int, c_void_p,
+                                                    c_void_p, c_void_p, c_void_p, c_int, c_int,
+                                                    c_void_p, c_void_p, c_void_p, c_void_p,
+                                                    c_void_p, c_long, c_void_p,
+                                                    c_void_p, c_void_p, c_void_p, c_void_p,
+                                                    c_void_p, c_long, c_void_p, c_void_p,
+                                                    c_void_p, c_void_p]),
     "hbmr_kmeans_centroid_nbr": (c_int, [c_void_p, c_int, c_int, c_int, c_void_p, c_void_p,
                                          c_void_p, c_void_p]),
     "hbmr_kmeans_image16": (c_int, [c_void_p, c_int, c_int, c_int, c_int, c_int, c_void_p,
@@ -73,6 +81,11 @@
                                                 c_int, c_void_p, c_int, c_int, c_void_p,
                                                 c_void_p, c_void_p, c_void_p, c_int, c_void_p,
                                                 c_int, c_void_p, c_long, c_void_p]),
+    "hbmr_kmeans_refine_batch_finish_gap2": (c_int, [c_int, c_void_p, c_void_p, c_void_p, c_int,
+                                                     c_int, c_void_p, c_int, c_int, c_void_p,
+                                                     c_void_p, c_void_p, c_void_p, c_int,
+                                                     c_void_p, c_int, c_void_p, c_long, c_void_p,
+                                                     c_void_p]),
     "hbmr_kmeans_accum_workspace_bytes": (c_long, [c_long, c_int]),
     "hbmr_kmeans_batch_workspace_bytes": (c_long, [c_long, c_int, c_int]),
     "hbmr_kmeans_map_batch": (c_int, [c_int, c_void_p, c_void_p, c_int, c_void_p, c_void_p, c_int,
diff --git a/hbmr/ops/kmeans.py b/hbmr/ops/kmeans.py
--- a/hbmr/ops/kmeans.py
+++ b/hbmr/ops/kmeans.py
@@ -334,6 +334,7 @@
             self.nbr = img.neighbors()
             self.pd = img.pair_dist()
         self.labels = [None] * len(splits)
+        self.gap2 = None
         self.lib = _lib.load()
         self.st = _lib.stream_handle(stream)
 
@@ -356,6 +357,14 @@
         xs = (ctypes.c_void_p * B)(*[sp.x32.data_ptr() for sp in self.splits])
         ls = (ctypes.c_void_p * B)(*[(lp.value if isinstance(lp, ctypes.c_void_p) else lp)
                                      for lp in self.labels])
+        if self.gap2 is not None:
+            g2 = (ctypes.c_void_p * B)(*[None if t is None else t.data_ptr() for t in self.gap2])
+            rc = self.lib.hbmr_kmeans_refine_batch_finish_gap2(
+                B, self.ns, xs, ls, img.d, self.splits[0].x32.shape[1], _ptr(img.cen), img.k,
+                img.k_pad, _ptr(cmax), _ptr(cemax), _ptr(ni), _ptr(nd), L, _ptr(self.stats),
+                self.stats.numel(), _ptr(self.ws), self.ws.numel(), g2, self.st)
+            _lib.check(rc, "hbmr_kmeans_refine_batch_finish_gap2")
+            return
         rc = self.lib.hbmr_kmeans_refine_batch_finish(
             B, self.ns, xs, ls, img.d, self.splits[0].x32.shape[1], _ptr(img.cen), img.k,
             img.k_pad, _ptr(cmax), _ptr(cemax), _ptr(ni), _ptr(nd), L, _ptr(self.stats),
@@ -413,7 +422,8 @@
 
 def assign_exact_batch(splits: list, img: CentroidImage, stats: torch.Tensor, out: torch.Tensor,
                        scratch: dict | None = None, stream=None, bounds: list | None = None,
-                       skipped: torch.Tensor | None = None) -> None:
+                       skipped: torch.Tensor | None = None, refine_bounds: bool = True,
+                       held: torch.Tensor | None = None) -> None:
     if not splits:
         return
     _check_refine_dim(img)
@@ -463,7 +473,7 @@
             off += _exact_group(group, img, stats, base + 4 * off, c16, ch, (cn, cmax, ce, cemax),
                                 dt, scratch, stream, lib, st,
                                 None if bounds is None else bounds[g0:g0 + MAX_REFINE_BATCH],
-                                skipped, newref)
+                                skipped, newref, refine_bounds, held)
             continue
         rb = _RefineBatch(group, img, stats, scratch, stream) if REFINE_VERSION >= 3 else None
         for i, sp in enumerate(group):
@@ -491,7 +501,7 @@
 
 
 def _bounded_group(group, bases, img, labels_ptr, ch, norms, dt, scratch, stream, lib, st, rb,
-                   skipped, newref):
+                   skipped, newref, refine_bounds=True, held=None):
     B = len(group)
     ns = [sp.shape[0] for sp in group]
     N = sum(ns)
@@ -507,12 +517,18 @@
         for b in bases:
             if b.gap is None:
                 b.gap, b.ref = torch.empty(b.g.numel(), dtype=torch.float32, device=dev), None
+            if not refine_bounds:
+                b.gap2 = None
+            elif b.gap2 is None:
+                b.gap2 = torch.zeros(b.g.numel(), dtype=torch.float32, device=dev)
         for b, n in zip(bases, ns):
             if b.g.numel() != n or b.gap.numel() != n or \
+                    (b.gap2 is not None and (b.gap2.numel() != n or b.gap2.dtype != torch.float32
+                                             or not b.gap2.is_contiguous())) or \
                     (b.ref is not None and (tuple(b.ref.shape) != tuple(img.cen.shape) or
                                             not b.ref.is_contiguous())):
                 raise ValueError("bounds: baseline does not match its split / the centroids")
-            for t in (b.g, b.gap, b.ref):
+            for t in (b.g, b.gap, b.gap2, b.ref):
                 if t is not None:
                     base = t._base if t._base is not None else t
                     blocks[id(base)] = base
@@ -527,7 +543,8 @@
     refs = [b.ref for b in bases]
     for b in bases:
         b.ref = b.pending = None
-    rc = lib.hbmr_kmeans_assign_top3_q1_bounded(
+    rb.gap2 = [b.gap2 for b in bases] if refine_bounds else None
+    rc = lib.hbmr_kmeans_assign_top3_q1_bounded2(
         B, P(*[sp.xb.data_ptr() for sp in group]), (ctypes.c_long * B)(*ns), img.dp,
         int(dt == torch.float16), _ptr(img.image16_tiled(dt)), _ptr(ch), img.k_pad, labels_ptr,
         P(*[sp.xnorm.data_ptr() for sp in group]), P(*[sp.xbn2.data_ptr() for sp in group]),
@@ -535,14 +552,15 @@
         _ptr(cemax), _ptr(rb.ws), rb.ws.numel(), _ptr(rb.pd),
         P(*[b.g.data_ptr() for b in bases]), P(*[b.gap.data_ptr() for b in bases]),
         P(*[None if r is None else r.data_ptr() for r in refs]), _ptr(img.cen),
-        _ptr(bws), bws.numel(), _ptr(skipped), st)
-    _lib.check(rc, "hbmr_kmeans_assign_top3_q1_bounded")
+        _ptr(bws), bws.numel(), _ptr(skipped),
+        P(*[b.gap2.data_ptr() for b in bases]) if refine_bounds else None, _ptr(held), st)
+    _lib.check(rc, "hbmr_kmeans_assign_top3_q1_bounded2")
     for b in bases:
         b.pending = newref
 
 
 def _exact_group(group, img, stats, labels_ptr, c16, ch, norms, dt, scratch, stream, lib, st,
-                 bases=None, skipped=None, newref=None):
+                 bases=None, skipped=None, newref=None, refine_bounds=True, held=None):
     B = len(group)
     ns = [sp.shape[0] for sp in group]
     N = sum(ns)
@@ -555,7 +573,7 @@
         if TRACE.on:
             TRACE.instant("kmeans.top3_launch", n=B)
         _bounded_group(group, bases, img, labels_ptr, ch, norms, dt, scratch, stream, lib, st, rb,
-                       skipped, newref)
+                       skipped, newref, refine_bounds, held)
         o = 0
         for i in range(B):
             rb.labels[i] = labels_ptr + 4 * o
@@ -648,11 +666,12 @@
 
 
 class Baseline:
-    __slots__ = ("g", "S0", "N0", "event", "stream", "data_ptr", "n", "gap", "ref", "pending")
+    __slots__ = ("g", "S0", "N0", "event", "stream", "data_ptr", "n", "gap", "gap2", "ref",
+                 "pending")
 
     def __init__(self, g, S0, N0, data_ptr, n):
         self.g, self.S0, self.N0 = g, S0, N0
-        self.gap = self.ref = self.pending = None
+        self.gap = self.gap2 = self.ref = self.pending = None
         self.event = None
         self.stream = None
         self.data_ptr, self.n = data_ptr, n
diff --git a/native/include/hbmr/hbmr.h b/native/include/hbmr/hbmr.h
--- a/native/include/hbmr/hbmr.h
+++ b/native/include/hbmr/hbmr.h
@@ -59,6 +59,18 @@
                                        const float* const* ref, const float* cen, void* bws,
                                        long bws_bytes, unsigned long long* skipped,
                                        hipStream_t st);
+int hbmr_kmeans_assign_top3_q1_bounded2(int nsplit, const void* const* X, const long* n, int dp,
+                                        int f16, const void* Ct, const float* chalf, int k_pad,
+                                        int32_t* labels, const float* const* xnorm,
+                                        const float* const* xbn2, const float* const* xerr,
+                                        int d, int k, const float* cnorm, const float* cmax,
+                                        const float* cerr, const float* cerrmax, void* ws,
+                                        long ws_bytes, const float* dcc,
+                                        const int32_t* const* g, float* const* gap,
+                                        const float* const* ref, const float* cen, void* bws,
+                                        long bws_bytes, unsigned long long* skipped,
+                                        float* const* gap2, unsigned long long* held,
+                                        hipStream_t st);
 int hbmr_kmeans_assign_top3_grouped(int nsplit, const void* const* X, const long* n, int dp,
                                     int f16, const void* C, const float* chalf, int k_pad,
                                     int32_t* labels, int32_t* cand, float* scores, float* margin,
@@ -83,6 +95,13 @@
                                     const int32_t* nbr_idx, const float* nbr_dist, int L,
                                     unsigned long long* stats, int nstats, void* ws,
                                     long ws_bytes, hipStream_t st);
+int hbmr_kmeans_refine_batch_finish_gap2(int nsplit, const long* ns, const float* const* x32,
+                                         int32_t* const* labels, int d, int ldx,
+                                         const float* C32, int k, int k_pad, const float* cmax,
+                                         const float* cerrmax, const int32_t* nbr_idx,
+                                         const float* nbr_dist, int L, unsigned long long* stats,
+                                         int nstats, void* ws, long ws_bytes,
+                                         float* const* gap2, hipStream_t st);
 int hbmr_kmeans_update(const long long* sums, const long long* counts, int fx_shift, int k, int d,
                        int dp, int k_pad, float* cen, void* cbf, float* chalf, float* shift2,
                        hipStream_t st);
diff --git a/native/kernels/kmeans.hip b/native/kernels/kmeans.hip
--- a/native/kernels/kmeans.hip
+++ b/native/kernels/kmeans.hip
@@ -248,6 +248,24 @@
                                        const float* const* ref, const float* cen, void* bws,
                                        long bws_bytes, unsigned long long* skipped,
                                        hipStream_t st) {
+  return hbmr_kmeans_assign_top3_q1_bounded2(nsplit, X, n, dp, f16, Ct, chalf, k_pad, labels,
+                                             xnorm, xbn2, xerr, d, k, cnorm, cmax, cerr, cerrmax,
+                                             ws, ws_bytes, dcc, g, gap, ref, cen, bws, bws_bytes,
+                                             skipped, nullptr, nullptr, st);
+}
+
+int hbmr_kmeans_assign_top3_q1_bounded2(int nsplit, const void* const* X, const long* n, int dp,
+                                        int f16, const void* Ct, const float* chalf, int k_pad,
+                                        int32_t* labels, const float* const* xnorm,
+                                        const float* const* xbn2, const float* const* xerr,
+                                        int d, int k, const float* cnorm, const float* cmax,
+                                        const float* cerr, const float* cerrmax, void* ws,
+                                        long ws_bytes, const float* dcc,
+                                        const int32_t* const* g, float* const* gap,
+                                        const float* const* ref, const float* cen, void* bws,
+                                        long bws_bytes, unsigned long long* skipped,
+                                        float* const* gap2, unsigned long long* held,
+                                        hipStream_t st) {
   if (nsplit <= 0 || nsplit > kMaxGroup || k_pad % 32 || k <= 0 || k_pad < k || d <= 0 ||
       d > kRefineMaxDp || !labels || ((uintptr_t)ws & 255) || (dp != 64 && dp != 128) || !Ct ||
       !g || !gap || !ref || !cen || !bws || ((uintptr_t)bws & 255))
@@ -272,12 +290,14 @@
     sw.n[i] = n[i];
     sw.g[i] = g[i];
     gt.gap[i] = gap[i];
+    gt.gap2[i] = gap2 ? gap2[i] : nullptr;
     if (ref[i]) {
       int r = 0;
       while (r < nref && sh.ref[r] != ref[i]) ++r;
       if (r == nref) sh.ref[nref++] = ref[i];
       sw.rid[i] = r;
       sw.gap[i] = gap[i];
+      sw.gap2[i] = gt.gap2[i];
     }
     total += n[i];
     nb += ceil_div(n[i], kFusedPts);
@@ -298,6 +318,7 @@
   HBMR_RETURN_IF_ERROR(hipMemsetAsync(bw, 0, kBoundHdr, st));
   uint32_t* cnt = reinterpret_cast<uint32_t*>(bw);
   uint32_t* smax = cnt + kMaxGroup;
+  uint32_t* cnt2 = smax + kMaxGroup;
   float* shift = reinterpret_cast<float*>(bw + kBoundHdr);
   uint32_t* idx = reinterpret_cast<uint32_t*>(
       bw + kBoundHdr + (((size_t)nsplit * k * sizeof(float) + 255) & ~(size_t)255));
@@ -307,7 +328,8 @@
     HBMR_RETURN_IF_ERROR(hipGetLastError());
   }
   hipLaunchKernelGGL(kmeans_bound_sweep_kernel, dim3((unsigned)nsb), dim3(256), 0, st, sw, k,
-                     shift, reinterpret_cast<const float*>(smax), labels, cnt, idx);
+                     shift, reinterpret_cast<const float*>(smax), labels, cnt, cnt2, idx, held,
+                     reinterpret_cast<unsigned long long*>(w + kStatsOff));
   HBMR_RETURN_IF_ERROR(hipGetLastError());
   const FusedQ1Fin fin = make_fused_fin(k, d, k_pad, cnorm, cerr, dcc, cmax, cerrmax, w, Ly);
   const auto [kern, lds] = fused_kernel(dp, f16, [](auto D, auto F) {
@@ -315,7 +337,7 @@
   });
   hipLaunchKernelGGL(kern, dim3((unsigned)nb), dim3(256), lds, st, t, gt,
                      reinterpret_cast<const __bf16*>(Ct), chalf, k_pad / 32, labels, fin,
-                     (const uint32_t*)cnt, (const uint32_t*)idx, skipped);
+                     (const uint32_t*)cnt, (const uint32_t*)cnt2, (const uint32_t*)idx, skipped);
   return (int)hipGetLastError();
 }
 
@@ -485,6 +507,18 @@
                                     const int32_t* nbr_idx, const float* nbr_dist, int L,
                                     unsigned long long* stats, int nstats, void* ws,
                                     long ws_bytes, hipStream_t st) {
+  return hbmr_kmeans_refine_batch_finish_gap2(nsplit, ns, x32, labels, d, ldx, C32, k, k_pad,
+                                              cmax, cerrmax, nbr_idx, nbr_dist, L, stats, nstats,
+                                              ws, ws_bytes, nullptr, st);
+}
+
+int hbmr_kmeans_refine_batch_finish_gap2(int nsplit, const long* ns, const float* const* x32,
+                                         int32_t* const* labels, int d, int ldx,
+                                         const float* C32, int k, int k_pad, const float* cmax,
+                                         const float* cerrmax, const int32_t* nbr_idx,
+                                         const float* nbr_dist, int L, unsigned long long* stats,
+                                         int nstats, void* ws, long ws_bytes,
+                                         float* const* gap2, hipStream_t st) {
   if (nsplit <= 0 || nsplit > kMaxGroup || d > ldx || d > kRefineMaxDp || d % 8 || ldx % 4 ||
       k <= 0 || k_pad < k || L < 1 || L > k || nstats < 3 || ((uintptr_t)C32 & 15) ||
       ((uintptr_t)ws & 255))
@@ -499,6 +533,9 @@
     tbl.x32[i] = x32[i];
     tbl.labels[i] = labels[i];
   }
+  Gap2Table gt;
+  std::memset(&gt, 0, sizeof(gt));
+  for (int i = 0; gap2 && i < nsplit; ++i) gt.gap2[i] = gap2[i];
   const double pack_rel = pack_rel_of(k_pad);
   char* w = static_cast<char*>(ws);
   uint32_t* c1 = reinterpret_cast<uint32_t*>(w);
@@ -507,7 +544,17 @@
   ExactQ2* q2 = reinterpret_cast<ExactQ2*>(w + Ly.off2);
   unsigned long long* ss = reinterpret_cast<unsigned long long*>(w + kStatsOff);
   const unsigned g3 = std::max(1u, Ly.g2);
-  if (d <= 128) {
+  if (gap2) {
+    auto k2 = d <= 128 ? kmeans_refine_q2_kernel<1, Gap2Table>
+                       : kmeans_refine_q2_kernel<2, Gap2Table>;
+    auto k3 = d <= 128 ? kmeans_refine_q3_kernel<1, Gap2Table>
+                       : kmeans_refine_q3_kernel<2, Gap2Table>;
+    hipLaunchKernelGGL(k2, dim3(Ly.g2), dim3(256), 0, st, tbl, d, ldx, C32, k, cmax, cerrmax,
+                       pack_rel, c1, q1, Ly.cap1, c2, q2, Ly.cap2, ss, gt);
+    HBMR_RETURN_IF_ERROR(hipGetLastError());
+    hipLaunchKernelGGL(k3, dim3(g3), dim3(256), 0, st, tbl, d, ldx, C32, k, nbr_idx, nbr_dist, L,
+                       c2, q2, Ly.cap2, ss, nstats, gt);
+  } else if (d <= 128) {
     hipLaunchKernelGGL(kmeans_refine_q2_kernel<1>, dim3(Ly.g2), dim3(256), 0, st, tbl, d, ldx,
                        C32, k, cmax, cerrmax, pack_rel, c1, q1, Ly.cap1, c2, q2, Ly.cap2, ss);
     HBMR_RETURN_IF_ERROR(hipGetLastError());
diff --git a/native/kernels/kmeans/bounded.h b/native/kernels/kmeans/bounded.h
--- a/native/kernels/kmeans/bounded.h
+++ b/native/kernels/kmeans/bounded.h
@@ -5,7 +5,7 @@
 namespace {
 
 constexpr int kSweepPer = 8;
-constexpr int kBoundHdr = 512;
+constexpr int kBoundHdr = 768;
 
 struct ShiftTable {
   const float* ref[kMaxGroup];
@@ -43,6 +43,7 @@
   int nsplit;
   const int32_t* g[kMaxGroup];
   float* gap[kMaxGroup];
+  float* gap2[kMaxGroup];
   int rid[kMaxGroup];
   long n[kMaxGroup];
   long off[kMaxGroup];
@@ -52,7 +53,8 @@
 __global__ __launch_bounds__(256) void kmeans_bound_sweep_kernel(
     const SweepTable tbl, int k, const float* __restrict__ shift,
     const float* __restrict__ smax, int32_t* __restrict__ labels, uint32_t* __restrict__ cnt,
-    uint32_t* __restrict__ idx) {
+    uint32_t* __restrict__ cnt2, uint32_t* __restrict__ idx,
+    unsigned long long* __restrict__ held, unsigned long long* __restrict__ sstats) {
   const long b = blockIdx.x;
   int lo = 0, hi = tbl.nsplit;
   while (hi - lo > 1) {
@@ -64,34 +66,50 @@
   const long n = tbl.n[s], o = tbl.off[s];
   const int32_t* __restrict__ g = tbl.g[s];
   float* __restrict__ gap = tbl.gap[s];
+  float* __restrict__ gap2 = gap ? tbl.gap2[s] : nullptr;
   const float* __restrict__ sh = shift + (size_t)tbl.rid[s] * k;
   const float sm = gap ? smax[tbl.rid[s]] : 0.f;
   const long p0 = (b - tbl.blk[s]) * (256 * kSweepPer);
   __shared__ uint32_t wcnt[4][kSweepPer];
+  __shared__ uint32_t whold[4];
   __shared__ uint32_t base_s;
   bool list[kSweepPer];
   uint32_t rank[kSweepPer];
+  uint32_t nheld = 0;
 #pragma unroll
   for (int i = 0; i < kSweepPer; ++i) {
     const long p = p0 + i * 256 + tid;
     list[i] = false;
+    bool hold = false;
     if (p < n) {
       list[i] = true;
       if (gap) {
         const int32_t c = g[p];
-        const float v =
-            (uint32_t)c < (uint32_t)k ? sub_rd_pos(sub_rd_pos(gap[p], sh[c]), sm) : 0.f;
+        const bool in = (uint32_t)c < (uint32_t)k;
+        const float g1 = gap[p];
+        const float v = in ? sub_rd_pos(sub_rd_pos(g1, sh[c]), sm) : 0.f;
         if (v > 0.f) {
           list[i] = false;
           labels[o + p] = c;
           gap[p] = v;
+        } else if (gap2) {
+          const float v2 = in ? sub_rd_pos(sub_rd_pos(gap2[p], sh[c]), sm) : 0.f;
+          if (v2 > 0.f) {
+            list[i] = false;
+            hold = true;
+            labels[o + p] = c;
+            gap2[p] = v2;
+            if (g1 != 0.f) gap[p] = 0.f;
+          }
         }
       }
     }
     const unsigned long long m = __ballot(list[i]);
     rank[i] = lane_rank(m);
     if (lane == 0) wcnt[wave][i] = (uint32_t)__popcll(m);
+    nheld += (uint32_t)__popcll(__ballot(hold));
   }
+  if (lane == 0) whold[wave] = nheld;
   __syncthreads();
   if (tid == 0) {
     uint32_t tot = 0;
@@ -103,7 +121,11 @@
         wcnt[w][i] = tot;
         tot += c;
       }
-    base_s = tot ? atomicAdd(cnt + s, tot) : 0u;
+    const uint32_t h = whold[0] + whold[1] + whold[2] + whold[3];
+    base_s = tot ? atomicAdd(cnt2 + s, tot) : 0u;
+    if (tot + h) atomicAdd(cnt + s, tot + h);
+    if (h && held != nullptr) atomicAdd(held, (unsigned long long)h);
+    if (h) atomicAdd(sstats + 4 * (blockIdx.x % kQShards), (unsigned long long)h);
   }
   __syncthreads();
   uint32_t* out = idx + o + base_s;
@@ -114,14 +136,15 @@
 
 struct GapTable {
   float* gap[kMaxGroup];
+  float* gap2[kMaxGroup];
 };
 
 template <int D, bool F16>
 __global__ __launch_bounds__(256, kExactMinB) void kmeans_assign_top3_q1_bounded_kernel(
     const TopQ1Table tbl, const GapTable gt, const __bf16* __restrict__ Ct,
     const float* __restrict__ chalf, int ntiles, int32_t* __restrict__ labels, FusedQ1Fin fin,
-    const uint32_t* __restrict__ cnt, const uint32_t* __restrict__ idx,
-    unsigned long long* __restrict__ skipped) {
+    const uint32_t* __restrict__ cnt, const uint32_t* __restrict__ cnt2,
+    const uint32_t* __restrict__ idx, unsigned long long* __restrict__ skipped) {
   extern __shared__ __attribute__((aligned(16))) char smem[];
   if (blockIdx.x == 0 && threadIdx.x == 0 && skipped != nullptr) {
     unsigned long long sk = 0;
@@ -136,7 +159,7 @@
     if (tbl.blk[mid] <= b) lo = mid; else hi = mid;
   }
   const int s = __builtin_amdgcn_readfirstlane(lo);
-  const long nl = (long)__builtin_amdgcn_readfirstlane(cnt[s]);
+  const long nl = (long)__builtin_amdgcn_readfirstlane(cnt2[s]);
   const long lb = b - tbl.blk[s];
   if (lb * 256 >= nl) return;
   const long o = tbl.off[s];
@@ -146,7 +169,8 @@
   fin.sidx = s;
   fin.idx = idx + o;
   fin.gap = gt.gap[s];
-  assign_tile_v3<D, F16, true>(tbl.X[s], nl, Ct, chalf, ntiles, labels + o, lb, smem, fin);
+  assign_tile_v3<D, F16, true>(tbl.X[s], nl, Ct, chalf, ntiles, labels + o, lb, smem, fin,
+                               gt.gap2[s]);
 }
 
 
diff --git a/native/kernels/kmeans/fused.h b/native/kernels/kmeans/fused.h
--- a/native/kernels/kmeans/fused.h
+++ b/native/kernels/kmeans/fused.h
@@ -27,7 +27,8 @@
 
   template <class AM, int PB, bool BND = false>
   __device__ __forceinline__ void operator()(const AM (&am)[PB], int h, long p0, int col, long n,
-                                             int32_t* __restrict__ labels) const {
+                                             int32_t* __restrict__ labels,
+                                             float* __restrict__ gap2 = nullptr) const {
     const int tid = threadIdx.x, lane = tid & 63, wave = tid >> 6;
     __shared__ uint32_t fq_cnt[4 * PB];
     __shared__ uint32_t fq_base;
@@ -83,6 +84,7 @@
           flag[pb] = q.s < k && q1_certify<true>(q, m2, cnorm[q.b], cerr[q.b], k, gam, cm, cem,
                                                  pack_rel, cnorm, cerr, dcc, gp);
           gap[row] = gp;
+          if (gap2 != nullptr) gap2[row] = 0.f;
         } else {
           flag[pb] = q.s < k && q1_flagged(q, m2, cnorm[q.b], cerr[q.b], k, gam, cm, cem,
                                            pack_rel, cnorm, cerr, dcc);
@@ -160,7 +162,8 @@
                                                const __bf16* __restrict__ Ct,
                                                const float* __restrict__ chalf, int ntiles,
                                                int32_t* __restrict__ labels, long blk, char* smem,
-                                               const FusedQ1Fin& fin) {
+                                               const FusedQ1Fin& fin,
+                                               float* __restrict__ gap2 = nullptr) {
   static_assert(D <= 128, "v3 keeps two 32-point blocks of D <= 128 in registers");
   constexpr int PB = 2, NS = 4;
   using V = AssignV2<D, NS>;
@@ -248,7 +251,7 @@
     for (int pb = 0; pb < PB; ++pb) top2_insert(am[pb], acc[pb], code, vmask);
     bias(nbuf, bz);
   }
-  fin.template operator()<PackedTop2x8, PB, BND>(am, h, p0, col, n, labels);
+  fin.template operator()<PackedTop2x8, PB, BND>(am, h, p0, col, n, labels, gap2);
 }
 
 struct TopQ1Table {
diff --git a/native/kernels/kmeans/refine_queue.h b/native/kernels/kmeans/refine_queue.h
--- a/native/kernels/kmeans/refine_queue.h
+++ b/native/kernels/kmeans/refine_queue.h
@@ -32,6 +32,17 @@
   const float* x32[kMaxGroup];
   int32_t* labels[kMaxGroup];
 };
+struct Gap2Table {
+  float* gap2[kMaxGroup];
+};
+__device__ __forceinline__ float* const* gap2_of() { return nullptr; }
+__device__ __forceinline__ float* const* gap2_of(const Gap2Table& t) { return t.gap2; }
+
+__device__ __forceinline__ float refine_gap2(double lo2, double rest, double whi2) {
+  const double a = fmin(sqrt(fmax(0.0, lo2)) * (1.0 - 0x1p-36), rest);
+  const double g = (a - sqrt(whi2) * (1.0 + 0x1p-36)) * (1.0 - 0x1p-30);
+  return g > 0.0 && g < 0x1p126 ? fmaxf(0.f, __double2float_rd(g)) : 0.f;
+}
 
 __host__ __device__ inline long ceil_div(long a, long b) { return (a + b - 1) / b; }
 
@@ -285,13 +296,15 @@
   return v;
 }
 
-template <int NM>
+template <int NM, class... Gap>
 __global__ __launch_bounds__(256) void kmeans_refine_q2_kernel(
     const RefineTable tbl, int d, int ldx, const float* __restrict__ C32, int k,
     const float* __restrict__ cmax, const float* __restrict__ cerrmax, double pack_rel,
     const uint32_t* __restrict__ qcount, const ExactQ1* __restrict__ q1, long cap1,
     uint32_t* __restrict__ q2count, ExactQ2* __restrict__ q2, long cap2,
-    unsigned long long* __restrict__ sstats) {
+    unsigned long long* __restrict__ sstats, const Gap... gt) {
+  static_assert(sizeof...(Gap) <= 1, "nothing or one Gap2Table");
+  constexpr bool GAP = sizeof...(Gap) == 1;
   constexpr uint32_t kPerBlk = 4 * kQ2Per;
   constexpr uint32_t kBuf = 256;
   const int tid = threadIdx.x, lane = tid & 63, wave = tid >> 6;
@@ -366,6 +379,7 @@
                      (!t_real || w == q.t || beats(f2));
     dw = whi;
     bool certified = !t_real && separated;
+    double lrest = __builtin_inf();
     if (t_real && separated) {
       const double xn = ((double)q.xn + (double)q.xe) * inflate;
       const double x2 = (double)q.x2;
@@ -374,10 +388,24 @@
       double et, dl_t;
       exact_bound(st, cm, xn, x2, amax, gam, pack_rel, et, dl_t);
       certified = 0.5 * (x2 - dw) - x2 * 0x1p-23 > st + et && dl_t >= 2.0 * amax;
+      if constexpr (GAP)
+        lrest = 2.0 * (0.5 * x2 - x2 * 0x1p-23 - (st + et)) -
+                (x2 + 2.0 * (fabs(st) + et)) * 0x1p-40;
     }
     if (have && sub == 0 && certified && w != q.b) {
       tbl.labels[q.split][q.row] = w;
       atomicAdd(&cnt[0], 1ull);
+    }
+    if constexpr (GAP) {
+      float* g2 = gap2_of(gt...)[q.split];
+      if (have && sub == 0 && certified && g2 != nullptr) {
+        auto low = [&](double dj) { return dj * (1.0 - rel) - aeps; };
+        double lo = lrest;
+        if (w != q.b) lo = fmin(lo, low(f0));
+        if (w != q.s) lo = fmin(lo, low(f1));
+        if (t_real && w != q.t) lo = fmin(lo, low(f2));
+        g2[q.row] = refine_gap2(lo, __builtin_inf(), whi);
+      }
     }
     const bool spill = have && sub == 0 && !certified;
     const unsigned long long m = __ballot(spill);
@@ -403,12 +431,19 @@
   if (tid < 2 && cnt[tid]) atomicAdd(sstats + 4 * shard + 1 + tid, cnt[tid]);
 }
 
-template <int NM>
+__device__ __forceinline__ void q3_second(double& second, int w, double dw, int j, double dj) {
+  if (dj < dw || (dj == dw && j < w)) second = fmin(second, dw);
+  else if (j != w) second = fmin(second, dj);
+}
+
+template <int NM, class... Gap>
 __global__ __launch_bounds__(256) void kmeans_refine_q3_kernel(
     const RefineTable tbl, int d, int ldx, const float* __restrict__ C32, int k,
     const int32_t* __restrict__ nbr_idx, const float* __restrict__ nbr_dist, int L,
     const uint32_t* __restrict__ q2count, const ExactQ2* __restrict__ q2, long cap2,
-    unsigned long long* __restrict__ sstats, int nstats) {
+    unsigned long long* __restrict__ sstats, int nstats, const Gap... gt) {
+  static_assert(sizeof...(Gap) <= 1, "nothing or one Gap2Table");
+  constexpr bool GAP = sizeof...(Gap) == 1;
   const int tid = threadIdx.x, lane = tid & 63;
   const int grp = lane / kRefineGroup, sub = lane % kRefineGroup;
   __shared__ unsigned long long cnt[3];
@@ -451,9 +486,12 @@
     const float* nd = nbr_dist + (size_t)w0 * L;
     const float* cw0 = C32 + (size_t)w0 * d;
     int evals = 0;
+    double second = __builtin_inf();
+    float snd = __builtin_inff();
     for (int jj = 0; jj < L; jj += kElkanStep) {
       const double lim = (r0 + sqrt(dw)) * (1.0 + 0x1p-40);
       if ((double)nd[jj] > lim) {
+        if constexpr (GAP) snd = fminf(snd, nd[jj]);
         done = true;
         break;
       }
@@ -462,6 +500,8 @@
 #pragma unroll
       for (int v = 0; v < kElkanStep; ++v) {
         const bool ok = jj + v < L && (double)nd[jj + v] <= lim;
+        if constexpr (GAP)
+          if (jj + v < L && !ok) snd = fminf(snd, nd[jj + v]);
         jv[v] = ok ? ni[jj + v] : -1;
         cp[v] = ok ? C32 + (size_t)jv[v] * d : cw0;
       }
@@ -469,8 +509,11 @@
       rows_dist2<NM, kElkanStep>(xv, cp, d, sub, dj);
       evals += kElkanStep;
 #pragma unroll
-      for (int v = 0; v < kElkanStep; ++v)
+      for (int v = 0; v < kElkanStep; ++v) {
+        if constexpr (GAP)
+          if (jv[v] >= 0) q3_second(second, w, dw, jv[v], dj[v]);
         if (jv[v] >= 0 && (dj[v] < dw || (dj[v] == dw && jv[v] < w))) { w = jv[v]; dw = dj[v]; }
+      }
     }
     const bool full = !done && L < k;
     if (full) {
@@ -481,8 +524,11 @@
         double dj[4];
         rows_dist2<NM, 4>(xv, cp, d, sub, dj);
 #pragma unroll
-        for (int v = 0; v < 4; ++v)
+        for (int v = 0; v < 4; ++v) {
+          if constexpr (GAP)
+            if (j + v < k) q3_second(second, w, dw, j + v, dj[v]);
           if (j + v < k && (dj[v] < dw || (dj[v] == dw && j + v < w))) { w = j + v; dw = dj[v]; }
+        }
       }
     }
     if (have && sub == 0) {
@@ -490,6 +536,11 @@
       if (full) atomicAdd(&cnt[2], 1ull);
       if (w != b0) atomicAdd(&cnt[0], 1ull);
       lab[q.row] = w;
+      if constexpr (GAP) {
+        float* g2 = gap2_of(gt...)[q.split];
+        const double rest = full ? __builtin_inf() : (double)snd - r0 * (1.0 + 0x1p-36);
+        if (g2 != nullptr) g2[q.row] = refine_gap2(second, rest, dw);
+      }
     }
   }
   __syncthreads();
```

Result: slower. 9173 (-14.5%).
